# GeoMop/MLMC

Measured on AMD Instinct MI355X. Metric: moment-evals/sec (samples x n_moments), higher is better.
Workload: dtype f64

## Files before the change

### include/mlmc_hip.h

```cpp
#ifndef MLMC_HIP_H
#define MLMC_HIP_H

#include <stdint.h>

#ifdef __cplusplus
extern "C" {
#endif

#define MLMC_ABI_VERSION 8

enum { MLMC_LEGENDRE = 0, MLMC_MONOMIAL = 1, MLMC_FOURIER = 2, MLMC_IDENTITY = 3, MLMC_SPLINE = 4 };
enum {
    MLMC_MODE_MOMENTS = 0,
    MLMC_MODE_COV = 1
};
enum { MLMC_HOST = 0, MLMC_DEVICE = 1 };

typedef struct mlmc_basis mlmc_basis;
typedef struct mlmc_accum mlmc_accum;

typedef struct {
    int32_t kind;
    int32_t size;
    double shift;
    double scale;
    double ref0, ref1;
    int32_t is_log;
    int32_t is_clip;
    int32_t out_size;
    int32_t reserved;
    const double *matrix;
    double x_lo, x_hi;
} mlmc_basis_desc;

int mlmc_init(int device, int flags);
void mlmc_shutdown(void);
int mlmc_set_stream(void *hip_stream);
int mlmc_wait_event(void *hip_event);
int mlmc_synchronize(void);
const char *mlmc_last_error(void);
int mlmc_abi_version(void);
int mlmc_device_info(char *name, int name_len, int *n_cu, int *wave_size, int64_t *hbm_bytes);

int mlmc_basis_create(const mlmc_basis_desc *desc, mlmc_basis **out);
void mlmc_basis_destroy(mlmc_basis *b);
int mlmc_basis_eval(const mlmc_basis *b, const double *x, int64_t n, int32_t size, double *out, int mem_kind);

#define MLMC_MODE_MEAN_ONLY 0x100
int mlmc_accum_create(const mlmc_basis *b, int32_t n_levels, int32_t mode, int32_t n_comp, mlmc_accum **out);
void mlmc_accum_destroy(mlmc_accum *a);
int mlmc_accum_reset(mlmc_accum *a);
int mlmc_accum_push(mlmc_accum *a, int32_t level, const double *fine, const double *coarse, int64_t n, int mem_kind);
int mlmc_accum_finalize(mlmc_accum *a, int64_t *n, int64_t *n_rm, double *s, double *sp, int mem_kind);
int mlmc_accum_estimate(mlmc_accum *a, int32_t n_chunks, const int32_t *levels, const double *const *fine,
                        const double *const *coarse, const int64_t *n_samples, int mem_kind, int64_t *n, int64_t *n_rm,
                        double *s, double *sp);
int mlmc_accum_estimate_packed(mlmc_accum *a, int32_t n_chunks, const int32_t *levels, const double *const *fine,
                               const double *const *coarse, const int64_t *n_samples, int mem_kind, double *packed,
                               int packed_kind);
int mlmc_accum_finalize_packed(mlmc_accum *a, double *packed, int mem_kind);
int mlmc_accum_kernel_time(mlmc_accum *a, double *ms, int64_t *launches, int64_t *alg_bytes);
int mlmc_accum_kernel_flops(mlmc_accum *a, int64_t *mfma_flops);
int mlmc_accum_aux_kernel_time(mlmc_accum *a, double *ms, int64_t *launches, int64_t *alg_bytes);
int mlmc_linearization_table(int32_t kind, int32_t R, int32_t squares, double *out, int64_t out_len);

int mlmc_accum_estimate_multi(int32_t M, const mlmc_basis *const *bases, int32_t K, int32_t n_levels, int32_t n_chunks,
                              const int32_t *levels, const double *const *fine, const double *const *coarse,
                              const int64_t *n_samples, int64_t *n, int64_t *n_rm, double *sums);
int mlmc_accum_estimate_multi_var(int32_t M, const mlmc_basis *const *bases, int32_t K, int32_t n_levels, int32_t n_chunks,
                                  const int32_t *levels, const double *const *fine, const double *const *coarse,
                                  const int64_t *n_samples, int64_t *n, int64_t *n_rm, double *sums, double *sums_sq);

#define MLMC_DIAG_NSTAT 9
int mlmc_level_diagnostics(int32_t M, int32_t n_levels, int32_t n_chunks, const int32_t *levels, const double *const *fine,
                           const double *const *coarse, const int64_t *n_samples, int64_t *n, int64_t *n_rm, double *stats);
int mlmc_diag_merge(const double *a, int64_t na, const double *b, int64_t nb, double *out);

int mlmc_xcov_create(int32_t M, int32_t n_levels, int32_t flags, mlmc_accum **out);
int mlmc_xcov_set_shift(mlmc_accum *a, const double *shift_host);

typedef struct {
    double tol;
    int32_t max_it;
    int32_t n_intervals;
    int32_t gauss_degree;
    int32_t reserved;
    double stab_penalty;
    double penalty_coef;
    int32_t decay_left, decay_right;
} mlmc_maxent_opts;

typedef struct {
    int32_t nit;
    int32_t success;
    double fun;
    double grad_norm;
    double moment0;
    int32_t n_quad;
    int32_t reserved;
} mlmc_maxent_info;

int mlmc_maxent_solve(const mlmc_basis *b, const double *mu, const double *sigma, int32_t R1, double a, double bnd_b,
                      const mlmc_maxent_opts *opts, const double *prev_lambda, int32_t n_prev, double *lambda_io,
                      double *grad_out, double *hess_out, mlmc_maxent_info *info);
int mlmc_density_eval(const mlmc_basis *b, const double *lambda, const double *sigma, int32_t R1, const double *x,
                      int64_t n, double *out, int mem_kind);
int mlmc_density_integrate(const mlmc_basis *b, const double *lambda, const double *sigma, int32_t R1, const double *lo,
                           const double *hi, int64_t n, int32_t degree, double *out);
int mlmc_maxent_solve_batch(int32_t B, const mlmc_basis *const *bases, const int32_t *R1, const double *a, const double *b,
                            const double *mu, const double *sigma, const mlmc_maxent_opts *opts, double *lambda_io,
                            double *grad_out, double *hess_out, mlmc_maxent_info *info);
int mlmc_density_eval_batch(int32_t B, const mlmc_basis *const *bases, const int32_t *R1, const double *lambda, const double *sigma,
                            const double *x, const int64_t *n, double *out);
int mlmc_density_integrate_batch(int32_t B, const mlmc_basis *const *bases, const int32_t *R1, const double *lambda,
                                 const double *sigma, const double *lo, const double *hi, const int64_t *n, int32_t degree,
                                 double *out);
int mlmc_density_cdf_batch(int32_t B, const mlmc_basis *const *bases, const int32_t *R1, const double *lambda, const double *sigma,
                           const double *a, const double *b, int32_t n_intervals, int32_t gauss_degree, const double *x,
                           const int64_t *n, double *out, double *mass_out, int mem_kind);
int mlmc_density_quantiles_batch(int32_t B, const mlmc_basis *const *bases, const int32_t *R1, const double *lambda,
                                 const double *sigma, const double *a, const double *b, int32_t n_intervals, int32_t gauss_degree,
                                 const double *p, const int64_t *n, double *out, double *mass_out, int mem_kind);
int mlmc_density_quantiles_kernel_time(double *ms, int64_t *launches);

int mlmc_percentiles(const double *x, int64_t n, const double *q_percent, int32_t nq, double *out, int64_t *n_valid,
                     int mem_kind);
int mlmc_percentiles_rows(const double *x, int64_t n_rows, int64_t n, int64_t ld, const double *q_percent, int32_t nq,
                          double *out , int64_t *n_valid , int mem_kind);

enum {
    MLMC_X_LOAD = 0,
    MLMC_X_CONST,
    MLMC_X_STORE,
    MLMC_X_SELECT,
    MLMC_X_ADD, MLMC_X_SUB, MLMC_X_MUL, MLMC_X_DIV,
    MLMC_X_MOD,
    MLMC_X_POW, MLMC_X_MAXIMUM, MLMC_X_MINIMUM, MLMC_X_FMAX, MLMC_X_FMIN, MLMC_X_ATAN2, MLMC_X_HYPOT, MLMC_X_FMOD,
    MLMC_X_NEG, MLMC_X_ABS, MLMC_X_SQRT, MLMC_X_SQUARE, MLMC_X_RECIP, MLMC_X_EXP, MLMC_X_EXP2, MLMC_X_EXPM1,
    MLMC_X_LOG, MLMC_X_LOG2, MLMC_X_LOG10, MLMC_X_LOG1P, MLMC_X_SIN, MLMC_X_COS, MLMC_X_TAN, MLMC_X_ASIN, MLMC_X_ACOS,
    MLMC_X_ATAN, MLMC_X_SINH, MLMC_X_COSH, MLMC_X_TANH, MLMC_X_FLOOR, MLMC_X_CEIL, MLMC_X_TRUNC, MLMC_X_RINT,
    MLMC_X_SIGN, MLMC_X_CBRT,
    MLMC_X_LT, MLMC_X_LE, MLMC_X_GT, MLMC_X_GE, MLMC_X_EQ, MLMC_X_NE,
    MLMC_X_AND, MLMC_X_OR, MLMC_X_NOT, MLMC_X_XOR,
    MLMC_X_N_OPS
};
#define MLMC_X_IMM_A 0x4000
#define MLMC_X_IMM_B 0x8000
#define MLMC_X_A_PREV 0x2000
#define MLMC_X_B_PREV 0x1000
#define MLMC_X_NO_WB 0x0800
#define MLMC_X_OP_MASK 0x07ff
typedef struct {
    uint16_t op, dst, a, b;
    double imm;
} mlmc_expr_instr;
#define MLMC_EXPR_MAX_REGS 16
#define MLMC_EXPR_MAX_INSTR 4096
typedef struct mlmc_expr mlmc_expr;
int mlmc_expr_create(const mlmc_expr_instr *prog, int32_t n_instr, int32_t n_regs, int32_t n_in_rows, int32_t n_out_rows,
                     mlmc_expr **out);
void mlmc_expr_destroy(mlmc_expr *e);
int mlmc_expr_eval(mlmc_expr *e, const double *const *rows_in, int32_t has_coarse, int64_t n, int64_t sample_stride,
                   int64_t side_stride, double *fine_out, double *coarse_out, int64_t *n_selected);
int mlmc_expr_state(mlmc_expr *e, int32_t *state, int64_t *compiled_launches);
int mlmc_expr_kernel_time(mlmc_expr *e, double *ms, int64_t *launches, int64_t *alg_bytes);

int mlmc_subsample_gather(const double *fine, const double *coarse, int32_t n_rows, int64_t n, int64_t k, uint64_t seed,
                          double *fine_out, double *coarse_out);

int mlmc_bootstrap_weights(int64_t n, int64_t b0, int64_t nb, const int64_t *sizes, uint64_t seed, uint32_t stream,
                           int32_t *w_out);
typedef struct mlmc_bootstrap mlmc_bootstrap;
int mlmc_bootstrap_create(const mlmc_basis *b, int32_t M, int32_t n_levels, int64_t B, mlmc_bootstrap **out);
void mlmc_bootstrap_destroy(mlmc_bootstrap *bs);
int mlmc_bootstrap_reset(mlmc_bootstrap *bs);
int mlmc_bootstrap_accum(mlmc_bootstrap *bs, int32_t level, const double *fine, const double *coarse, int64_t n,
                         const int64_t *sizes, uint64_t seed, uint32_t stream);
int mlmc_bootstrap_finalize(mlmc_bootstrap *bs, int64_t *n_out, double *s_out, double *sp_out);
int mlmc_bootstrap_kernel_time(mlmc_bootstrap *bs, double *ms_contract, double *ms_rng, int64_t *mfma_flops);

int mlmc_synth_generate(int32_t level_id, int64_t first_sample, int64_t n, double fine_step, double coarse_step,
                        double loc, double scale, int32_t n_rows, const int32_t *rows, double *const *out);
int mlmc_synth_seeds(int32_t level_id, int64_t first_sample, int64_t n, uint32_t *seeds_host);

#ifdef __cplusplus
}
#endif
#endif
```

### mlmc_amd/_lib.py

```python
import ctypes as C
import os
import threading

import numpy as np

_HERE = os.path.dirname(os.path.abspath(__file__))
LIB_PATH = os.environ.get("MLMC_HIP_LIB", os.path.join(_HERE, "libmlmc_hip.so"))

ABI_VERSION = 8
LEGENDRE, MONOMIAL, FOURIER, IDENTITY, SPLINE = 0, 1, 2, 3, 4
MODE_MOMENTS, MODE_COV = 0, 1
MODE_MEAN_ONLY = 0x100
HOST, DEVICE = 0, 1
FLAG_TIMING = 1


class MlmcHipError(RuntimeError):
    pass


class BasisDesc(C.Structure):
    _fields_ = [("kind", C.c_int32), ("size", C.c_int32), ("shift", C.c_double), ("scale", C.c_double),
                ("ref0", C.c_double), ("ref1", C.c_double), ("is_log", C.c_int32), ("is_clip", C.c_int32),
                ("out_size", C.c_int32), ("reserved", C.c_int32), ("matrix", C.POINTER(C.c_double)),
                ("x_lo", C.c_double), ("x_hi", C.c_double)]


class MaxentOpts(C.Structure):
    _fields_ = [("tol", C.c_double), ("max_it", C.c_int32), ("n_intervals", C.c_int32), ("gauss_degree", C.c_int32),
                ("reserved", C.c_int32), ("stab_penalty", C.c_double), ("penalty_coef", C.c_double),
                ("decay_left", C.c_int32), ("decay_right", C.c_int32)]


class MaxentInfo(C.Structure):
    _fields_ = [("nit", C.c_int32), ("success", C.c_int32), ("fun", C.c_double), ("grad_norm", C.c_double),
                ("moment0", C.c_double), ("n_quad", C.c_int32), ("reserved", C.c_int32)]


_dp = C.POINTER(C.c_double)
_ip = C.POINTER(C.c_int64)
_vp = C.c_void_p

SIGNATURES = {
    "mlmc_init": (C.c_int, [C.c_int, C.c_int]),
    "mlmc_shutdown": (None, []),
    "mlmc_set_stream": (C.c_int, [_vp]),
    "mlmc_synchronize": (C.c_int, []),
    "mlmc_wait_event": (C.c_int, [_vp]),
    "mlmc_last_error": (C.c_char_p, []),
    "mlmc_abi_version": (C.c_int, []),
    "mlmc_device_info": (C.c_int, [C.c_char_p, C.c_int, C.POINTER(C.c_int), C.POINTER(C.c_int), _ip]),
    "mlmc_basis_create": (C.c_int, [C.POINTER(BasisDesc), C.POINTER(_vp)]),
    "mlmc_basis_destroy": (None, [_vp]),
    "mlmc_basis_eval": (C.c_int, [_vp, _vp, C.c_int64, C.c_int32, _vp, C.c_int]),
    "mlmc_accum_create": (C.c_int, [_vp, C.c_int32, C.c_int32, C.c_int32, C.POINTER(_vp)]),
    "mlmc_accum_destroy": (None, [_vp]),
    "mlmc_accum_reset": (C.c_int, [_vp]),
    "mlmc_accum_push": (C.c_int, [_vp, C.c_int32, _vp, _vp, C.c_int64, C.c_int]),
    "mlmc_accum_finalize": (C.c_int, [_vp, _vp, _vp, _vp, _vp, C.c_int]),
    "mlmc_accum_finalize_packed": (C.c_int, [_vp, _vp, C.c_int]),
    "mlmc_accum_estimate": (C.c_int, [_vp, C.c_int32, _vp, _vp, _vp, _vp, C.c_int, _vp, _vp, _vp, _vp]),
    "mlmc_accum_estimate_packed": (C.c_int, [_vp, C.c_int32, _vp, _vp, _vp, _vp, C.c_int, _vp, C.c_int]),
    "mlmc_accum_kernel_time": (C.c_int, [_vp, _dp, _ip, _ip]),
    "mlmc_accum_kernel_flops": (C.c_int, [_vp, _ip]),
    "mlmc_accum_aux_kernel_time": (C.c_int, [_vp, _dp, _ip, _ip]),
    "mlmc_linearization_table": (C.c_int, [C.c_int32, C.c_int32, C.c_int32, _vp, C.c_int64]),
    "mlmc_percentiles": (C.c_int, [_vp, C.c_int64, _vp, C.c_int32, _vp, _ip, C.c_int]),
    "mlmc_percentiles_rows": (C.c_int, [_vp, C.c_int64, C.c_int64, C.c_int64, _vp, C.c_int32, _vp, _vp, C.c_int]),
    "mlmc_maxent_solve": (C.c_int, [_vp, _vp, _vp, C.c_int32, C.c_double, C.c_double, C.POINTER(MaxentOpts), _vp,
                                    C.c_int32, _vp, _vp, _vp, C.POINTER(MaxentInfo)]),
    "mlmc_density_eval": (C.c_int, [_vp, _vp, _vp, C.c_int32, _vp, C.c_int64, _vp, C.c_int]),
    "mlmc_density_integrate": (C.c_int, [_vp, _vp, _vp, C.c_int32, _vp, _vp, C.c_int64, C.c_int32, _vp]),
    "mlmc_xcov_create": (C.c_int, [C.c_int32, C.c_int32, C.c_int32, C.POINTER(_vp)]),
    "mlmc_xcov_set_shift": (C.c_int, [_vp, _vp]),
    "mlmc_accum_estimate_multi": (C.c_int, [C.c_int32, _vp, C.c_int32, C.c_int32, C.c_int32, _vp, _vp, _vp, _vp, _vp, _vp,
                                            _vp]),
    "mlmc_accum_estimate_multi_var": (C.c_int, [C.c_int32, _vp, C.c_int32, C.c_int32, C.c_int32, _vp, _vp, _vp, _vp, _vp, _vp,
                                                _vp, _vp]),
    "mlmc_level_diagnostics": (C.c_int, [C.c_int32, C.c_int32, C.c_int32, _vp, _vp, _vp, _vp, _vp, _vp, _vp]),
    "mlmc_diag_merge": (C.c_int, [_vp, C.c_int64, _vp, C.c_int64, _vp]),
    "mlmc_maxent_solve_batch": (C.c_int, [C.c_int32, _vp, _vp, _vp, _vp, _vp, _vp, C.POINTER(MaxentOpts), _vp, _vp, _vp, _vp]),
    "mlmc_density_eval_batch": (C.c_int, [C.c_int32, _vp, _vp, _vp, _vp, _vp, _vp, _vp]),
    "mlmc_density_integrate_batch": (C.c_int, [C.c_int32, _vp, _vp, _vp, _vp, _vp, _vp, _vp, C.c_int32, _vp]),
    "mlmc_density_cdf_batch": (C.c_int, [C.c_int32, _vp, _vp, _vp, _vp, _vp, _vp, C.c_int32, C.c_int32, _vp, _vp, _vp, _vp,
                                         C.c_int]),
    "mlmc_density_quantiles_batch": (C.c_int, [C.c_int32, _vp, _vp, _vp, _vp, _vp, _vp, C.c_int32, C.c_int32, _vp, _vp, _vp, _vp,
                                               C.c_int]),
    "mlmc_density_quantiles_kernel_time": (C.c_int, [_dp, _ip]),
    "mlmc_expr_create": (C.c_int, [_vp, C.c_int32, C.c_int32, C.c_int32, C.c_int32, C.POINTER(_vp)]),
    "mlmc_expr_destroy": (None, [_vp]),
    "mlmc_expr_eval": (C.c_int, [_vp, _vp, C.c_int32, C.c_int64, C.c_int64, C.c_int64, _vp, _vp, _ip]),
    "mlmc_expr_state": (C.c_int, [_vp, C.POINTER(C.c_int32), _ip]),
    "mlmc_expr_kernel_time": (C.c_int, [_vp, _dp, _ip, _ip]),
    "mlmc_synth_generate": (C.c_int, [C.c_int32, C.c_int64, C.c_int64, C.c_double, C.c_double, C.c_double, C.c_double,
                                      C.c_int32, _vp, _vp]),
    "mlmc_synth_seeds": (C.c_int, [C.c_int32, C.c_int64, C.c_int64, _vp]),
    "mlmc_subsample_gather": (C.c_int, [_vp, _vp, C.c_int32, C.c_int64, C.c_int64, C.c_uint64, _vp, _vp]),
    "mlmc_bootstrap_weights": (C.c_int, [C.c_int64, C.c_int64, C.c_int64, _vp, C.c_uint64, C.c_uint32, _vp]),
    "mlmc_bootstrap_create": (C.c_int, [_vp, C.c_int32, C.c_int32, C.c_int64, C.POINTER(_vp)]),
    "mlmc_bootstrap_destroy": (None, [_vp]),
    "mlmc_bootstrap_reset": (C.c_int, [_vp]),
    "mlmc_bootstrap_accum": (C.c_int, [_vp, C.c_int32, _vp, _vp, C.c_int64, _vp, C.c_uint64, C.c_uint32]),
    "mlmc_bootstrap_finalize": (C.c_int, [_vp, _vp, _vp, _vp]),
    "mlmc_bootstrap_kernel_time": (C.c_int, [_vp, _dp, _dp, _ip]),
}

_lock = threading.Lock()
_lib = None
_bound_device = None


def load():
    global _lib
    with _lock:
        if _lib is None:
            if not os.path.exists(LIB_PATH):
                raise MlmcHipError(
                    "libmlmc_hip.so not found at {} -- build it with `python -c 'import __graft_entry__ as g; g.build()'` "
                    "or `make -C mlmc_amd/csrc`; mlmc_amd has no CPU fallback".format(LIB_PATH))
            try:
                import torch
            except ImportError:
                pass
            lib = C.CDLL(LIB_PATH)
            for name, (res, args) in SIGNATURES.items():
                fn = getattr(lib, name)
                fn.restype = res
                fn.argtypes = args
            if lib.mlmc_abi_version() != ABI_VERSION:
                raise MlmcHipError("{} has ABI version {}, this package binds version {}: rebuild it "
                                   "(make -C mlmc_amd/csrc)".format(LIB_PATH, lib.mlmc_abi_version(), ABI_VERSION))
            _lib = lib
    return _lib


def check(rc):
    if rc != 0:
        raise MlmcHipError(load().mlmc_last_error().decode("utf-8", "replace"))


def init(device=None, flags=None):
    global _bound_device
    lib = load()
    if device is None:
        device = _bound_device if _bound_device is not None else int(os.environ.get("LOCAL_RANK", "0"))
    if flags is None:
        flags = FLAG_TIMING if os.environ.get("MLMC_HIP_TIMING") else 0
    check(lib.mlmc_init(int(device), int(flags)))
    _bound_device = int(device)
    return lib


def lib():
    if _bound_device is None:
        return init()
    return _lib


def use_torch_stream():
    import torch
    check(lib().mlmc_set_stream(C.c_void_p(torch.cuda.current_stream().cuda_stream)))


def device_info():
    l = lib()
    name = C.create_string_buffer(256)
    n_cu, wave = C.c_int(), C.c_int()
    hbm = C.c_int64()
    check(l.mlmc_device_info(name, 256, C.byref(n_cu), C.byref(wave), C.byref(hbm)))
    return dict(name=name.value.decode(), n_cu=n_cu.value, wave_size=wave.value, hbm_bytes=hbm.value, device=_bound_device)


def as_f64(a):
    return np.ascontiguousarray(a, dtype=np.float64)


def ptr(a):
    if a is None:
        return None
    if isinstance(a, np.ndarray):
        return a.ctypes.data_as(C.c_void_p)
    if hasattr(a, "data_ptr"):
        return C.c_void_p(a.data_ptr())
    raise TypeError(type(a))


def mem_kind(a):
    if isinstance(a, np.ndarray):
        return HOST
    if hasattr(a, "is_cuda"):
        return DEVICE if a.is_cuda else HOST
    raise TypeError(type(a))
```

### mlmc_amd/csrc/api.hip

```cpp
#include <cmath>
#include <chrono>
#include <cstring>
#include <new>

#include "common.hpp"
#include <algorithm>
#include <map>
#include <tuple>

namespace mlmc {

static thread_local std::string g_err;
void set_error(const std::string &msg) { g_err = msg; }
int fail(const std::string &msg) {
    g_err = msg;
    return 1;
}
Runtime &rt() {
    static Runtime r;
    return r;
}
std::recursive_mutex &api_mutex() {
    static std::recursive_mutex m;
    return m;
// ... 87 lines not shown
    *x_hi = as_double(last);
}

typedef long double ld;
static void legendre_products_ld(int R, std::vector<ld> &out) {
    const int K = 2 * R - 1;
    const size_t RR = (size_t)R * R;
    out.assign((size_t)K * RR, 0.0L);
    for (int i = 0; i < R; ++i)
        for (int j = 0; j < R; ++j) {
            const size_t ij = (size_t)i * R + j;
            const int hi = i > j ? i : j, lo = i > j ? j : i;
            const ld diff = (ld)(hi - lo);
            ld c = (2 * diff + 1) / (2 * (ld)hi + 1);
            for (int t = 1; t <= lo; ++t) {
                const ld tt = (ld)t;
                c = c * ((2 * tt - 1) / tt * (diff + tt) / (2 * (diff + tt) - 1));
            }
            for (int t = 0; t <= lo; ++t) {
                const int k = (hi - lo) + 2 * t;
                out[(size_t)k * RR + ij] = c;
                if (t == lo) break;
                const ld s = (ld)hi + t, kk = (ld)k;
                const ld si = s - hi, sj = s - lo, sk = s - kk;
                ld ratio = ((2 * kk + 5) / (2 * s + 3)) / ((2 * kk + 1) / (2 * s + 1));
                ratio = ratio * ((2 * si + 1) / (si + 1)) * ((2 * sj + 1) / (sj + 1));
                ratio = ratio * (sk / (2 * sk - 1));
                ratio = ratio * ((s + 1) / (2 * s + 1));
                c = c * ratio;
            }
        }
}

bool product_table(int kind, int R, std::vector<double> &out) {
    if (kind != MLMC_LEGENDRE && kind != MLMC_MONOMIAL) return false;
    const int K = 2 * R - 1;
    const size_t RR = (size_t)R * R;
    out.assign((size_t)K * RR, 0.0);
    if (kind == MLMC_MONOMIAL) {
        for (int i = 0; i < R; ++i)
            for (int j = 0; j < R; ++j) out[(size_t)(i + j) * RR + (size_t)i * R + j] = 1.0;
        return true;
    }
    std::vector<ld> c;
    legendre_products_ld(R, c);
    for (size_t q = 0; q < c.size(); ++q) out[q] = (double)c[q];
    return true;
}

static void legendre_square_products_ld(int R, std::vector<ld> &out) {
    const int K = 4 * R - 3;
    const size_t RR = (size_t)R * R;
    out.assign((size_t)K * RR, 0.0L);
    const int Q = 4 * R;
    const ld pi = 3.14159265358979323846264338327950288L;
    std::vector<ld> x(Q), w(Q), P((size_t)K * Q);
    for (int q = 0; q < Q; ++q) {
        ld t = std::cos(pi * ((ld)q + 0.75L) / ((ld)Q + 0.5L)), dp = 1.0L;
        for (int it = 0; it < 100; ++it) {
            ld p0 = 1.0L, p1 = t;
            for (int k = 2; k <= Q; ++k) {
                const ld p2 = ((2 * k - 1) * t * p1 - (k - 1) * p0) / k;
                p0 = p1;
                p1 = p2;
            }
            dp = Q * (t * p1 - p0) / (t * t - 1.0L);
            const ld dt = p1 / dp;
            t -= dt;
            if (std::fabs(dt) < 1e-20L) break;
        }
        {
            ld p0 = 1.0L, p1 = t;
            for (int k = 2; k <= Q; ++k) {
                const ld p2 = ((2 * k - 1) * t * p1 - (k - 1) * p0) / k;
                p0 = p1;
                p1 = p2;
            }
            dp = Q * (t * p1 - p0) / (t * t - 1.0L);
        }
        x[q] = t;
        w[q] = 2.0L / ((1.0L - t * t) * dp * dp);
        ld p0 = 1.0L, p1 = t;
        P[(size_t)0 * Q + q] = 1.0L;
        if (K > 1) P[(size_t)1 * Q + q] = t;
        for (int k = 2; k < K; ++k) {
            const ld p2 = ((2 * k - 1) * t * p1 - (k - 1) * p0) / k;
            p0 = p1;
            p1 = p2;
            P[(size_t)k * Q + q] = p2;
        }
    }
    std::vector<ld> sq(Q);
    for (int i = 0; i < R; ++i)
        for (int j = i; j < R; ++j) {
            for (int q = 0; q < Q; ++q) {
                const ld u = P[(size_t)i * Q + q] * P[(size_t)j * Q + q];
                sq[q] = w[q] * u * u;
            }
            for (int k = 0; k <= 2 * (i + j); k += 2) {
                ld acc = 0.0L;
                const ld *Pk = &P[(size_t)k * Q];
                for (int q = 0; q < Q; ++q) acc += sq[q] * Pk[q];
                const ld c = acc * (2 * k + 1) / 2;
                out[(size_t)k * RR + (size_t)i * R + j] = c;
                out[(size_t)k * RR + (size_t)j * R + i] = c;
            }
        }
    std::vector<ld> t1;
    legendre_products_ld(R, t1);
    for (int j = 0; j < R; ++j)
        for (int k = 0; k < K; ++k) {
            const ld c = k < 2 * R - 1 ? t1[(size_t)k * RR + (size_t)j * R + j] : 0.0L;
            out[(size_t)k * RR + (size_t)j] = c;
            out[(size_t)k * RR + (size_t)j * R] = c;
        }
}

bool square_product_table(int kind, int R, std::vector<double> &out) {
    if (kind != MLMC_LEGENDRE && kind != MLMC_MONOMIAL) return false;
    const int K = 4 * R - 3;
    const size_t RR = (size_t)R * R;
    out.assign((size_t)K * RR, 0.0);
    if (kind == MLMC_MONOMIAL) {
        for (int i = 0; i < R; ++i)
            for (int j = 0; j < R; ++j) out[(size_t)(2 * (i + j)) * RR + (size_t)i * R + j] = 1.0;
        return true;
    }
    std::vector<ld> c;
    legendre_square_products_ld(R, c);
    for (size_t q = 0; q < c.size(); ++q) out[q] = (double)c[q];
    return true;
}

static void chebyshev_compose(const std::vector<ld> &c, int K, int R, std::vector<double> &out) {
    const size_t RR = (size_t)R * R;
    std::vector<ld> g(K), at((size_t)K * K, 0.0L), col(K);
    g[0] = 1.0L;
    for (int j = 1; j < K; ++j) g[j] = g[j - 1] * (ld)(2 * j - 1) / (ld)(2 * j);
    for (int k = 0; k < K; ++k)
        for (int j = 0; j <= k; ++j) at[(size_t)(k - 2 * j < 0 ? 2 * j - k : k - 2 * j) * K + k] += g[j] * g[k - j];
    out.assign((size_t)K * RR, 0.0);
    for (int i = 0; i < R; ++i)
        for (int j = i; j < R; ++j) {
            const size_t ij = (size_t)i * R + j, ji = (size_t)j * R + i;
            for (int k = 0; k < K; ++k) col[k] = c[(size_t)k * RR + ij];
            for (int m = 0; m < K; ++m) {
                ld acc = 0.0L;
                for (int k = m; k < K; k += 2) acc += col[k] * at[(size_t)m * K + k];
                out[(size_t)m * RR + ij] = out[(size_t)m * RR + ji] = (double)acc;
            }
        }
}

bool product_table_chebyshev(int R, std::vector<double> &out) {
    std::vector<ld> c;
    legendre_products_ld(R, c);
    chebyshev_compose(c, 2 * R - 1, R, out);
    return true;
}

bool square_product_table_chebyshev(int R, std::vector<double> &out) {
    std::vector<ld> c;
    legendre_square_products_ld(R, c);
    const int K = 4 * R - 3;
    chebyshev_compose(c, K, R, out);
    std::vector<double> t1;
    product_table_chebyshev(R, t1);
    const size_t RR = (size_t)R * R;
    for (int j = 0; j < R; ++j)
        for (int m = 0; m < K; ++m) {
            const double v = m < 2 * R - 1 ? t1[(size_t)m * RR + (size_t)j * R + j] : 0.0;
            out[(size_t)m * RR + (size_t)j] = v;
            out[(size_t)m * RR + (size_t)j * R] = v;
        }
    return true;
}

static bool linearize_enabled() {
    const char *e = std::getenv("MLMC_HIP_LINEARIZE");
    return !(e && e[0] == '0');
}

static bool linearize_chebyshev_enabled() {
    const char *e = std::getenv("MLMC_HIP_LINEARIZE_CHEB");
    return !(e && e[0] == '0');
}

static int lin_min_size() {
    const char *e = std::getenv("MLMC_HIP_LINEARIZE_MIN");
    return e ? std::atoi(e) : 16;
}

static int need_runtime() {
    if (!rt().ready) return fail("mlmc_init has not been called (no HIP device bound)");
    return 0;
}

}

using namespace mlmc;

extern "C" {

int mlmc_abi_version(void) { return MLMC_ABI_VERSION; }
const char *mlmc_last_error(void) { return g_err.c_str(); }

int mlmc_init(int device, int flags) {
    MLMC_API_GUARD;
    Runtime &r = rt();
    int count = 0;
    hipError_t e = hipGetDeviceCount(&count);
    if (e != hipSuccess || count <= 0) return fail("no HIP device available: libmlmc_hip has no CPU fallback");
    if (device < 0 || device >= count) return fail("mlmc_init: device index out of range");
    if (r.ready && r.device == device) {
        r.flags = flags;
        return 0;
    }
    if (r.ready) return fail("mlmc_init: this process is already bound to another device (one process per GPU)");
    MLMC_HIP_CHECK(hipSetDevice(device));
    MLMC_HIP_CHECK(hipGetDeviceProperties(&r.prop, device));
    if (std::strncmp(r.prop.gcnArchName, "gfx950", 6) != 0)
        return fail(std::string("mlmc_init: kernels are built for gfx950 only, device is ") + r.prop.gcnArchName);
    MLMC_HIP_CHECK(hipStreamCreateWithFlags(&r.stream, hipStreamNonBlocking));
    r.own_stream = true;
    r.device = device;
    r.flags = flags;
    r.n_cu = r.prop.multiProcessorCount;
    r.ready = true;
    return 0;
}

}

namespace mlmc {
hipError_t wait_stream(hipStream_t st) {
    const auto t0 = std::chrono::steady_clock::now();
    for (int spins = 0;; ++spins) {
        const hipError_t e = hipStreamQuery(st);
        if (e != hipErrorNotReady) return e;
        if ((spins & 63) == 63 && std::chrono::steady_clock::now() - t0 > std::chrono::milliseconds(4)) break;
    }
    return hipStreamSynchronize(st);
}
}

extern "C" {

int mlmc_set_stream(void *stream) {
    MLMC_API_GUARD;
    Runtime &r = rt();
    if (!r.ready) return fail("mlmc_init has not been called (no HIP device bound)");
    MLMC_HIP_CHECK(wait_stream(r.stream));
    if (r.own_stream) (void)hipStreamDestroy(r.stream);
    r.stream = (hipStream_t)stream;
    r.own_stream = false;
    return 0;
}

int mlmc_wait_event(void *hip_event) {
    MLMC_API_GUARD;
    Runtime &r = rt();
    if (!r.ready) return fail("mlmc_init has not been called (no HIP device bound)");
    if (!hip_event) return fail("mlmc_wait_event: null event");
    MLMC_HIP_CHECK(hipStreamWaitEvent(r.stream, (hipEvent_t)hip_event, 0));
    return 0;
}

int mlmc_synchronize(void) {
    MLMC_API_GUARD;
    Runtime &r = rt();
    if (!r.ready) return fail("mlmc_init has not been called (no HIP device bound)");
    MLMC_HIP_CHECK(wait_stream(r.stream));
    return 0;
}

void mlmc_shutdown(void) {
    MLMC_API_GUARD;
    Runtime &r = rt();
    if (!r.ready) return;
    (void)wait_stream(r.stream);
    if (r.own_stream) (void)hipStreamDestroy(r.stream);
    r.stream = nullptr;
    r.ready = false;
    r.device = -1;
}

int mlmc_device_info(char *name, int name_len, int *n_cu, int *wave_size, int64_t *hbm_bytes) {
    MLMC_API_GUARD;
    if (need_runtime()) return 1;
    if (name && name_len > 0) {
        std::strncpy(name, rt().prop.name, (size_t)name_len - 1);
        name[name_len - 1] = 0;
    }
    if (n_cu) *n_cu = rt().prop.multiProcessorCount;
    if (wave_size) *wave_size = rt().prop.warpSize;
    if (hbm_bytes) *hbm_bytes = (int64_t)rt().prop.totalGlobalMem;
    return 0;
}

int mlmc_basis_create(const mlmc_basis_desc *d, mlmc_basis **out) {
    MLMC_API_GUARD;
    if (need_runtime()) return 1;
    if (!d || !out) return fail("mlmc_basis_create: null argument");
    if (d->size <= 0) return fail("mlmc_basis_create: size must be > 0");
    if (d->kind < MLMC_LEGENDRE || d->kind > MLMC_SPLINE) return fail("mlmc_basis_create: unknown kind");
    if (d->kind == MLMC_SPLINE && d->size < 4) return fail("mlmc_basis_create: cubic spline moments need size >= 4");
    if (d->kind == MLMC_IDENTITY && d->size != 1) return fail("mlmc_basis_create: IDENTITY has size 1");
    if (d->out_size < 0 || (d->out_size > 0 && !d->matrix)) return fail("mlmc_basis_create: matrix missing");
    if (d->kind == MLMC_LEGENDRE && d->size > 512) return fail("mlmc_basis_create: at most 512 Legendre moments");
    mlmc_basis *b = new (std::nothrow) mlmc_basis();
    if (!b) return fail("out of memory");
    b->p.kind = d->kind;
    b->p.size = d->size;
    b->p.shift = d->shift;
    b->p.scale = d->scale;
    b->p.ref0 = d->ref0;
    b->p.ref1 = d->ref1;
    b->p.is_log = d->is_log;
    b->p.is_clip = d->is_clip;
    b->p.x_lo = d->x_lo;
    b->p.x_hi = d->x_hi;
    if (d->is_log && d->is_clip && d->x_lo == 0.0 && d->x_hi == 0.0) log_keep_interval(b->p, &b->p.x_lo, &b->p.x_hi);
    b->out_size = d->out_size;
    const int R = d->size;
    b->scale_c.assign(R, 1.0);
    if (d->kind == MLMC_LEGENDRE) {
        long double c = 1.0L;
        for (int i = 0; i < R; ++i) {
            if (i >= 1) c = c * (long double)(2 * i - 1) / (long double)(2 * i);
            b->scale_c[i] = (double)c;
        }
    }
    hipError_t e = hipMalloc(&b->d_scale, sizeof(double) * R);
    if (e == hipSuccess) e = hipMemcpy(b->d_scale, b->scale_c.data(), sizeof(double) * R, hipMemcpyHostToDevice);
    if (e == hipSuccess && d->out_size > 0) {
        b->matrix.assign(d->matrix, d->matrix + (size_t)d->out_size * R);
        e = hipMalloc(&b->d_matrix, sizeof(double) * b->matrix.size());
        if (e == hipSuccess)
            e = hipMemcpy(b->d_matrix, b->matrix.data(), sizeof(double) * b->matrix.size(), hipMemcpyHostToDevice);
    }
    if (e != hipSuccess) {
        mlmc_basis_destroy(b);
        return fail(std::string("mlmc_basis_create: ") + hipGetErrorString(e));
    }
    *out = b;
    return 0;
}

void mlmc_basis_destroy(mlmc_basis *b) {
    MLMC_API_GUARD;
    if (!b) return;
    if (b->d_scale) (void)hipFree(b->d_scale);
    if (b->d_matrix) (void)hipFree(b->d_matrix);
    delete b;
}

int mlmc_basis_eval(const mlmc_basis *b, const double *x, int64_t n, int32_t size, double *out, int mem_kind) {
    MLMC_API_GUARD;
    if (need_runtime()) return 1;
    if (!b || (n > 0 && (!x || !out))) return fail("mlmc_basis_eval: null argument");
    const int max_size = b->out_size > 0 ? b->out_size : b->p.size;
    if (size <= 0 || size > max_size) return fail("mlmc_basis_eval: size out of range");
    if (n == 0) return 0;
    hipStream_t st = rt().stream;
    if (mem_kind == MLMC_DEVICE) {
        if (int rc = launch_eval(b, x, n, size, out)) return rc;
        MLMC_HIP_CHECK(wait_stream(st));
        return 0;
    }
    double *d_x = nullptr, *d_o = nullptr;
    hipError_t e0 = hipMalloc(&d_x, sizeof(double) * (size_t)n);
    if (e0 == hipSuccess) e0 = hipMalloc(&d_o, sizeof(double) * (size_t)n * size);
    if (e0 == hipSuccess) e0 = hipMemcpyAsync(d_x, x, sizeof(double) * (size_t)n, hipMemcpyHostToDevice, st);
    int rc = e0 == hipSuccess ? launch_eval(b, d_x, n, size, d_o) : fail(std::string("mlmc_basis_eval: ") + hipGetErrorString(e0));
    if (!rc) {
        hipError_t e = hipMemcpyAsync(out, d_o, sizeof(double) * (size_t)n * size, hipMemcpyDeviceToHost, st);
        if (e == hipSuccess) e = wait_stream(st);
        if (e != hipSuccess) rc = fail(std::string("mlmc_basis_eval copy back: ") + hipGetErrorString(e));
    }
    (void)hipFree(d_x);
    (void)hipFree(d_o);
    return rc;
}

struct LinTables {
    double *d_prod = nullptr, *d_prod2 = nullptr;
};
static int lin_tables(int kind, int R, bool cheb, bool squares, LinTables **out) {
    static std::map<std::tuple<int, int, int>, LinTables> cache;
    LinTables &t = cache[std::make_tuple(cheb ? 1 : 0, kind, R)];
    if (!t.d_prod) {
        std::vector<double> h;
        if (cheb) product_table_chebyshev(R, h);
        else product_table(kind, R, h);
        MLMC_HIP_CHECK(hipMalloc(&t.d_prod, sizeof(double) * h.size()));
        MLMC_HIP_CHECK(hipMemcpy(t.d_prod, h.data(), sizeof(double) * h.size(), hipMemcpyHostToDevice));
    }
    if (squares && !t.d_prod2) {
        std::vector<double> h;
        if (cheb) square_product_table_chebyshev(R, h);
        else square_product_table(kind, R, h);
        MLMC_HIP_CHECK(hipMalloc(&t.d_prod2, sizeof(double) * h.size()));
        MLMC_HIP_CHECK(hipMemcpy(t.d_prod2, h.data(), sizeof(double) * h.size(), hipMemcpyHostToDevice));
    }
    *out = &t;
    return 0;
}

static int inner_basis_create(const mlmc_basis *b, int size, bool cheb, mlmc_basis **out) {
    mlmc_basis_desc d;
    std::memset(&d, 0, sizeof(d));
    d.kind = cheb ? (int)MLMC_MONOMIAL : b->p.kind;
    d.size = size;
    d.shift = b->p.shift; d.scale = b->p.scale; d.ref0 = b->p.ref0; d.ref1 = b->p.ref1;
    d.is_log = b->p.is_log; d.is_clip = b->p.is_clip;
    d.x_lo = b->p.x_lo; d.x_hi = b->p.x_hi;
    if (int rc = mlmc_basis_create(&d, out)) return rc;
    (*out)->p.x_lo = b->p.x_lo;
    (*out)->p.x_hi = b->p.x_hi;
    if (cheb) (*out)->p.kind = KIND_CHEBYSHEV;
    return 0;
}

static int ensure_lin(mlmc_accum *a) {
    if (a->lin) return 0;
    const mlmc_basis *b = a->basis;
    const int K1 = 2 * a->R - 1, K2 = 4 * a->R - 3;
    const bool cheb1 = a->lin_cheb && K1 > 64, cheb2 = a->lin_cheb && K2 > 64;
    LinTables *t1 = nullptr, *t2 = nullptr;
    if (int rc = lin_tables(b->p.kind, a->R, cheb1, false, &t1)) return rc;
    if (a->lin0_eligible)
        if (int rc = lin_tables(b->p.kind, a->R, cheb2, true, &t2)) return rc;
    int rc = inner_basis_create(b, K1, cheb1, &a->lin_basis);
    if (!rc) rc = mlmc_accum_create(a->lin_basis, a->n_levels, MLMC_MODE_MOMENTS | MLMC_MODE_MEAN_ONLY, a->n_comp, &a->lin);
    if (!rc) {
        a->lin->host_outputs = false;
        a->lin_K = K1;
        a->d_lin_prod = t1->d_prod;
    }
    if (!rc && a->lin0_eligible) {
        rc = inner_basis_create(b, K2, cheb2, &a->lin0_basis);
        if (!rc) rc = mlmc_accum_create(a->lin0_basis, a->n_levels, MLMC_MODE_MOMENTS | MLMC_MODE_MEAN_ONLY, a->n_comp, &a->lin0);
        if (!rc) {
            a->lin0->host_outputs = false;
            a->lin0_K = K2;
            a->d_lin0_prod1 = t2->d_prod;
            a->d_lin0_prod = t2->d_prod2;
        }
    }
    if (rc) {
        if (a->lin) mlmc_accum_destroy(a->lin);
        if (a->lin_basis) mlmc_basis_destroy(a->lin_basis);
        if (a->lin0) mlmc_accum_destroy(a->lin0);
        if (a->lin0_basis) mlmc_basis_destroy(a->lin0_basis);
        a->lin = a->lin0 = nullptr;
        a->lin_basis = a->lin0_basis = nullptr;
        a->lin_eligible = a->lin0_eligible = false;
    }
    return rc;
}

int mlmc_accum_create(const mlmc_basis *b, int32_t n_levels, int32_t mode, int32_t n_comp, mlmc_accum **out) {
    MLMC_API_GUARD;
    if (need_runtime()) return 1;
    if (!b || !out) return fail("mlmc_accum_create: null argument");
    if (n_levels <= 0 || n_comp <= 0) return fail("mlmc_accum_create: n_levels and n_comp must be > 0");
    const bool mean_only = (mode & MLMC_MODE_MEAN_ONLY) != 0;
    mode &= ~MLMC_MODE_MEAN_ONLY;
    if (mode != MLMC_MODE_MOMENTS && mode != MLMC_MODE_COV) return fail("mlmc_accum_create: unknown mode");
    mlmc_accum *a = new (std::nothrow) mlmc_accum();
    if (!a) return fail("out of memory");
    a->basis = b;
    a->n_levels = n_levels;
    a->mode = mode;
    const bool spline_band = mode == MLMC_MODE_COV && mean_only && b->out_size == 0 && b->p.kind == MLMC_SPLINE && b->p.size <= SPLINE_BAND_MAX_R;
    a->cov_from_values = mode == MLMC_MODE_COV && (b->out_size > 0 || (b->p.size > 128 && !spline_band));
    a->mean_only = mean_only && ((mode == MLMC_MODE_COV && !a->cov_from_values) || (mode == MLMC_MODE_MOMENTS && b->out_size > 0));
    a->mean_only_plain = mean_only && mode == MLMC_MODE_MOMENTS && b->out_size == 0 &&
                         (b->p.kind == MLMC_LEGENDRE || b->p.kind == MLMC_MONOMIAL || b->p.kind == KIND_CHEBYSHEV) && b->p.size > 64 &&
                         b->p.size <= 256;
    a->n_comp = n_comp;
    a->R = b->p.size;
    a->Rout = b->out_size > 0 ? b->out_size : b->p.size;
    a->RP = (((mode == MLMC_MODE_COV && b->out_size > 0 ? a->Rout : a->R) + 15) / 16) * 16;
    if (mode == MLMC_MODE_MOMENTS) {
        a->K = (int64_t)n_comp * a->Rout;
        a->int_width = 2 * (int64_t)a->R + (b->out_size > 0 ? (int64_t)a->RP * a->RP : 0);
    } else {
        a->K = (int64_t)n_comp * a->Rout * a->Rout;
        a->int_width = 3 * (int64_t)a->RP * a->RP;
    }
    const size_t tot = (size_t)n_levels * n_comp * a->int_width;
    a->state_bytes = sizeof(double) * tot + sizeof(int64_t) * 2 * n_levels;
    a->out_bytes = (sizeof(int64_t) + sizeof(double)) * 2 * n_levels + 2 * sizeof(double) * (size_t)n_levels * a->K;
    if (hipMalloc(&a->d_state, a->state_bytes) != hipSuccess || hipMalloc(&a->d_out, a->out_bytes) != hipSuccess ||
        hipHostMalloc(&a->h_out, a->out_bytes, hipHostMallocDefault) != hipSuccess) {
        mlmc_accum_destroy(a);
        return fail("mlmc_accum_create: device / pinned allocation failed");
    }
    a->d_totals = (double *)a->d_state;
    a->d_counts = (int64_t *)(a->d_totals + tot);
    a->level_flushed.assign(n_levels, 0);
    if (mode == MLMC_MODE_MOMENTS && n_comp == 1 && b->out_size == 0) {
        void *dev_view = nullptr;
        if (hipHostGetDevicePointer(&dev_view, a->h_out, 0) == hipSuccess && dev_view) {
            a->host_outputs = true;
            a->h_out_n = (int64_t *)dev_view;
            a->h_out_s = (double *)(a->h_out_n + 2 * (size_t)n_levels) + 2 * (size_t)n_levels;
            a->h_out_sp = a->h_out_s + (size_t)n_levels * a->K;
        }
    }
    a->d_out_n = (int64_t *)a->d_out;
    a->d_out_nd = (double *)(a->d_out_n + 2 * (size_t)n_levels);
    a->d_out_s = a->d_out_nd + 2 * (size_t)n_levels;
    a->d_out_sp = a->d_out_s + (size_t)n_levels * a->K;
    if (mode == MLMC_MODE_COV && !mean_only && !a->cov_from_values && b->out_size == 0 && b->p.size > lin_min_size() && b->p.size <= 128 &&
        (b->p.kind == MLMC_LEGENDRE || b->p.kind == MLMC_MONOMIAL) && b->p.is_clip &&
        std::fabs(b->p.ref0) <= 1.0 && std::fabs(b->p.ref1) <= 1.0 &&
        linearize_enabled()) {
        a->lin_eligible = true;
        const char *min_n = std::getenv("MLMC_HIP_LINEARIZE_MIN_N");
        a->lin_min_n = min_n ? std::atoll(min_n) : (a->R > 32 ? 100000 : 1500000);
        const char *lin0_env = std::getenv("MLMC_HIP_LINEARIZE_LEVEL0");
        a->lin0_eligible = a->R <= 64 && !(lin0_env && lin0_env[0] == '0');
        a->lin_cheb = b->p.kind == MLMC_LEGENDRE && linearize_chebyshev_enabled() && std::getenv("MLMC_HIP_NO_SPLIT") == nullptr;
    }
    *out = a;
    return mlmc_accum_reset(a);
}

int mlmc_accum_reset(mlmc_accum *a) {
    MLMC_API_GUARD;
    if (need_runtime()) return 1;
    if (!a) return fail("mlmc_accum_reset: null argument");
    hipStream_t st = rt().stream;
    a->pending.clear();
    std::fill(a->level_flushed.begin(), a->level_flushed.end(), 0);
    MLMC_HIP_CHECK(hipMemsetAsync(a->d_state, 0, a->state_bytes, st));
    if (a->xcov) {
        MLMC_HIP_CHECK(hipMemcpyAsync(a->d_shift, a->shift_host.data(), sizeof(double) * a->shift_host.size(), hipMemcpyHostToDevice, st));
        a->xcov_pushes = 0;
    }
    a->lin_used = a->lin0_used = false;
    a->lin_levels.assign(a->n_levels, 0);
    a->lin0_levels.assign(a->n_levels, 0);
    if (a->lin0)
        if (int rc = mlmc_accum_reset(a->lin0)) return rc;
    if (a->lin) return mlmc_accum_reset(a->lin);
    return 0;
}

void mlmc_accum_destroy(mlmc_accum *a) {
    MLMC_API_GUARD;
    if (!a) return;
    if (rt().ready) (void)wait_stream(rt().stream);
    if (a->lin) mlmc_accum_destroy(a->lin);
    if (a->lin_basis) mlmc_basis_destroy(a->lin_basis);
    if (a->lin0) mlmc_accum_destroy(a->lin0);
    if (a->lin0_basis) mlmc_basis_destroy(a->lin0_basis);
    void *ptrs[] = {a->d_state, a->d_partials, a->d_pcounts, a->d_stage_f, a->d_stage_c, a->d_mask, a->d_out, a->d_vals_f, a->d_vals_c, a->d_vals_tmp,
                    a->d_shift};
    for (void *p : ptrs)
        if (p) (void)hipFree(p);
    if (a->h_out) (void)hipHostFree(a->h_out);
    for (hipEvent_t e : a->ev) (void)hipEventDestroy(e);
    delete a;
}

int mlmc_accum_push(mlmc_accum *a, int32_t level, const double *fine, const double *coarse, int64_t n, int mem_kind) {
    MLMC_API_GUARD;
    if (need_runtime()) return 1;
    if (!a) return fail("mlmc_accum_push: null argument");
    if (level < 0 || level >= a->n_levels) return fail("mlmc_accum_push: level out of range");
    if (n < 0) return fail("mlmc_accum_push: negative n");
    if (n == 0) return 0;
    if (!fine) return fail("mlmc_accum_push: fine is NULL");
    if (n > ((int64_t)1 << 40)) return fail("mlmc_accum_push: chunk too large, split it");
    hipStream_t st = rt().stream;
    const size_t bytes = sizeof(double) * (size_t)n * a->n_comp;
    const double *d_f = fine, *d_c = coarse;
    if (mem_kind == MLMC_HOST) {
        if (bytes > a->stage_cap) {
            MLMC_HIP_CHECK(wait_stream(st));
            if (a->d_stage_f) (void)hipFree(a->d_stage_f);
            if (a->d_stage_c) (void)hipFree(a->d_stage_c);
            a->d_stage_f = a->d_stage_c = nullptr;
            a->stage_cap = 0;
            MLMC_HIP_CHECK(hipMalloc(&a->d_stage_f, bytes));
            MLMC_HIP_CHECK(hipMalloc(&a->d_stage_c, bytes));
            a->stage_cap = bytes;
        } else {
            MLMC_HIP_CHECK(wait_stream(st));
        }
        MLMC_HIP_CHECK(hipMemcpyAsync(a->d_stage_f, fine, bytes, hipMemcpyHostToDevice, st));
        d_f = a->d_stage_f;
        if (coarse) {
            MLMC_HIP_CHECK(hipMemcpyAsync(a->d_stage_c, coarse, bytes, hipMemcpyHostToDevice, st));
            d_c = a->d_stage_c;
        }
        MLMC_HIP_CHECK(wait_stream(st));
    } else if (mem_kind != MLMC_DEVICE) {
        return fail("mlmc_accum_push: bad mem_kind");
    }
    if (a->xcov) {
        ++a->xcov_pushes;
        return launch_xcov_push(a, level, d_f, d_c, n);
    }
    const uint8_t *d_mask = nullptr;
    bool count_in_kernel = true;
    if (a->n_comp > 1) {
        if (int rc = ensure((void **)&a->d_mask, &a->mask_cap, (size_t)n)) return rc;
        if (int rc = launch_mask(a, d_f, d_c, n, a->d_mask, a->d_counts + 2 * (int64_t)level)) return rc;
        d_mask = a->d_mask;
        count_in_kernel = false;
    }
    for (int m = 0; m < a->n_comp; ++m) {
        const double *f_m = d_f + (int64_t)m * n;
        const double *c_m = d_c ? d_c + (int64_t)m * n : nullptr;
        const bool count = count_in_kernel && m == 0;
        int rc;
        if (a->mode == MLMC_MODE_MOMENTS) {
            const bool defer = mem_kind == MLMC_DEVICE || a->n_comp > 1;
            rc = launch_moments_accum(a, level, m, f_m, c_m, d_mask, n, count, defer);
            if (!rc && a->basis->out_size > 0 && !a->mean_only) {
                if (a->R <= 128) {
                    rc = launch_cov_accum(a, level, m, f_m, c_m, d_mask, n, false, 1);
                } else {
                    int64_t chunk = 1 << 22;
                    while (chunk > 4096 && chunk * a->R > ((int64_t)1 << 28)) chunk >>= 1;
                    const size_t need = sizeof(double) * (size_t)(n < chunk ? n : chunk) * a->R;
                    if (need > a->vals_cap) {
                        MLMC_HIP_CHECK(wait_stream(st));
                        if (a->d_vals_f) (void)hipFree(a->d_vals_f);
                        if (a->d_vals_c) (void)hipFree(a->d_vals_c);
                        a->d_vals_f = a->d_vals_c = nullptr;
                        a->vals_cap = 0;
                        MLMC_HIP_CHECK(hipMalloc(&a->d_vals_f, need));
                        MLMC_HIP_CHECK(hipMalloc(&a->d_vals_c, need));
                        a->vals_cap = need;
                    }
                    for (int64_t off = 0; off < n && !rc; off += chunk) {
                        const int64_t m_n = (n - off < chunk) ? n - off : chunk;
                        rc = launch_eval_scaled_base(a->basis, f_m + off, m_n, a->d_vals_f);
                        if (!rc && c_m) rc = launch_eval_scaled_base(a->basis, c_m + off, m_n, a->d_vals_c);
                        if (!rc) rc = launch_cov_from_values(a, level, m, a->d_vals_f, c_m ? a->d_vals_c : nullptr,
                                                             d_mask ? d_mask + off : nullptr, m_n, false, 1);
                    }
                }
            }
        } else if (a->cov_from_values) {
            const int R1 = a->Rout;
            int64_t chunk = 1 << 22;
            while (chunk > 4096 && chunk * R1 > ((int64_t)1 << 28)) chunk >>= 1;
            const size_t need = sizeof(double) * (size_t)(n < chunk ? n : chunk) * R1;
            if (need > a->vals_cap) {
                MLMC_HIP_CHECK(wait_stream(st));
                if (a->d_vals_f) (void)hipFree(a->d_vals_f);
                if (a->d_vals_c) (void)hipFree(a->d_vals_c);
                a->d_vals_f = a->d_vals_c = nullptr;
                a->vals_cap = 0;
                MLMC_HIP_CHECK(hipMalloc(&a->d_vals_f, need));
                MLMC_HIP_CHECK(hipMalloc(&a->d_vals_c, need));
                a->vals_cap = need;
            }
            if (a->basis->out_size > 0) {
                const size_t need_tmp = sizeof(double) * (size_t)(n < chunk ? n : chunk) * a->R;
                if (need_tmp > a->vals_tmp_cap) {
                    MLMC_HIP_CHECK(wait_stream(st));
                    if (a->d_vals_tmp) (void)hipFree(a->d_vals_tmp);
                    a->d_vals_tmp = nullptr;
                    a->vals_tmp_cap = 0;
                    MLMC_HIP_CHECK(hipMalloc(&a->d_vals_tmp, need_tmp));
                    a->vals_tmp_cap = need_tmp;
                }
            }
            rc = 0;
            for (int64_t off = 0; off < n && !rc; off += chunk) {
                const int64_t m_n = (n - off < chunk) ? n - off : chunk;
                rc = launch_eval(a->basis, f_m + off, m_n, R1, a->d_vals_f, a->d_vals_tmp);
                if (!rc && c_m) rc = launch_eval(a->basis, c_m + off, m_n, R1, a->d_vals_c, a->d_vals_tmp);
                if (!rc) rc = launch_cov_from_values(a, level, m, a->d_vals_f, c_m ? a->d_vals_c : nullptr,
                                                     d_mask ? d_mask + off : nullptr, m_n, count);
            }
        } else {
            if (a->lin_eligible && !a->lin && n >= a->lin_min_n)
                if (int rcl = ensure_lin(a)) return rcl;
            const bool use_lin0 = a->lin0 && !d_c && n >= a->lin_min_n;
            if (use_lin0) {
                a->lin0_used = true;
                a->lin0_levels[level] = 1;
                rc = launch_moments_accum(a->lin0, level, m, f_m, nullptr, d_mask, n, count_in_kernel && m == 0,
                                          mem_kind == MLMC_DEVICE || a->n_comp > 1);
                if (rc) return rc;
                continue;
            }
            const bool use_lin = a->lin && n >= a->lin_min_n;
            rc = m == 0 ? launch_cov_accum(a, level, 0, d_f, d_c, d_mask, n, count_in_kernel, a->mean_only ? 2 : (use_lin ? 3 : 0), a->n_comp) : 0;
            if (!rc && use_lin) { a->lin_used = true; a->lin_levels[level] = 1; }
            if (!rc && use_lin)
                rc = launch_moments_accum(a->lin, level, m, f_m, c_m, d_mask, n, false, mem_kind == MLMC_DEVICE || a->n_comp > 1);
        }
        if (rc) return rc;
    }
    if (a->mode == MLMC_MODE_MOMENTS && (mem_kind == MLMC_HOST || a->n_comp > 1))
        if (int rc = flush_moments(a)) return rc;
    if (a->lin && (mem_kind == MLMC_HOST || a->n_comp > 1))
        if (int rc = flush_moments(a->lin)) return rc;
    if (a->lin0 && (mem_kind == MLMC_HOST || a->n_comp > 1))
        if (int rc = flush_moments(a->lin0)) return rc;
    return 0;
}

int mlmc_accum_finalize(mlmc_accum *a, int64_t *n, int64_t *n_rm, double *s, double *sp, int mem_kind) {
    MLMC_API_GUARD;
    if (need_runtime()) return 1;
    if (!a || !n || !n_rm || !s || !sp) return fail("mlmc_accum_finalize: null argument");
    hipStream_t st = rt().stream;
    if (a->mode == MLMC_MODE_MOMENTS)
        if (int rcf = flush_moments(a)) return rcf;
    const int L = a->n_levels;
    const size_t nk = (size_t)L * a->K;
    if (a->host_outputs && mem_kind == MLMC_HOST) {
        MLMC_HIP_CHECK(wait_stream(st));
        const int64_t *hn = (const int64_t *)a->h_out;
        const double *hs = (const double *)(hn + 2 * (size_t)L) + 2 * (size_t)L;
        const size_t K = (size_t)a->K;
        for (int l = 0; l < L; ++l) {
            if (a->level_flushed[l]) {
                n[l] = hn[l];
                n_rm[l] = hn[L + l];
                std::memcpy(s + l * K, hs + l * K, sizeof(double) * K);
                std::memcpy(sp + l * K, hs + nk + l * K, sizeof(double) * K);
            } else {
                n[l] = n_rm[l] = 0;
                std::fill(s + l * K, s + (l + 1) * K, 0.0);
                std::fill(sp + l * K, sp + (l + 1) * K, 0.0);
            }
        }
        return 0;
    }
    int rc = a->xcov ? launch_xcov_finalize(a) : (a->mode == MLMC_MODE_MOMENTS) ? launch_moments_finalize(a) : launch_cov_finalize(a);
    if (rc) return rc;
    if (mem_kind == MLMC_DEVICE) {
        MLMC_HIP_CHECK(hipMemcpyAsync(n, a->d_out_n, sizeof(int64_t) * L, hipMemcpyDeviceToDevice, st));
        MLMC_HIP_CHECK(hipMemcpyAsync(n_rm, a->d_out_n + L, sizeof(int64_t) * L, hipMemcpyDeviceToDevice, st));
        MLMC_HIP_CHECK(hipMemcpyAsync(s, a->d_out_s, sizeof(double) * nk, hipMemcpyDeviceToDevice, st));
        MLMC_HIP_CHECK(hipMemcpyAsync(sp, a->d_out_sp, sizeof(double) * nk, hipMemcpyDeviceToDevice, st));
        MLMC_HIP_CHECK(wait_stream(st));
    } else {
        MLMC_HIP_CHECK(hipMemcpyAsync(a->h_out, a->d_out, a->out_bytes, hipMemcpyDeviceToHost, st));
        MLMC_HIP_CHECK(wait_stream(st));
        const int64_t *hn = (const int64_t *)a->h_out;
        const double *hs = (const double *)(hn + 2 * (size_t)L) + 2 * (size_t)L;
        std::memcpy(n, hn, sizeof(int64_t) * L);
        std::memcpy(n_rm, hn + L, sizeof(int64_t) * L);
        std::memcpy(s, hs, sizeof(double) * nk);
        std::memcpy(sp, hs + nk, sizeof(double) * nk);
    }
    return 0;
}

int mlmc_accum_estimate(mlmc_accum *a, int32_t n_chunks, const int32_t *levels, const double *const *fine,
                        const double *const *coarse, const int64_t *n_samples, int mem_kind, int64_t *n, int64_t *n_rm,
                        double *s, double *sp) {
    MLMC_API_GUARD;
    if (!a || n_chunks < 0 || (n_chunks > 0 && (!levels || !fine || !n_samples))) return fail("mlmc_accum_estimate: null argument");
    if (int rc = mlmc_accum_reset(a)) return rc;
    for (int k = 0; k < n_chunks; ++k)
        if (int rc = mlmc_accum_push(a, levels[k], fine[k], coarse ? coarse[k] : nullptr, n_samples[k], mem_kind)) return rc;
    return mlmc_accum_finalize(a, n, n_rm, s, sp, MLMC_HOST);
}

int mlmc_accum_finalize_packed(mlmc_accum *a, double *packed, int mem_kind) {
    MLMC_API_GUARD;
    if (need_runtime()) return 1;
    if (!a || !packed) return fail("mlmc_accum_finalize_packed: null argument");
    hipStream_t st = rt().stream;
    if (a->mode == MLMC_MODE_MOMENTS && a->host_outputs && mem_kind == MLMC_DEVICE && a->R <= MAX_TERMS_PER_PASS &&
        (int)a->pending.size() == a->n_levels &&
        std::none_of(a->level_flushed.begin(), a->level_flushed.end(), [](char f) { return f != 0; })) {
        a->packed_target = packed;
        const int rcf = flush_moments(a);
        a->packed_target = nullptr;
        return rcf;
    }
    if (a->mode == MLMC_MODE_MOMENTS)
        if (int rcf = flush_moments(a)) return rcf;
    int rc = a->xcov ? launch_xcov_finalize(a) : (a->mode == MLMC_MODE_MOMENTS) ? launch_moments_finalize(a) : launch_cov_finalize(a);
    if (rc) return rc;
    const size_t bytes = sizeof(double) * (2 * (size_t)a->n_levels + 2 * (size_t)a->n_levels * a->K);
    MLMC_HIP_CHECK(hipMemcpyAsync(packed, a->d_out_nd, bytes, mem_kind == MLMC_DEVICE ? hipMemcpyDeviceToDevice : hipMemcpyDeviceToHost, st));
    if (mem_kind == MLMC_DEVICE) return 0;
    MLMC_HIP_CHECK(wait_stream(st));
    return 0;
}

int mlmc_accum_estimate_packed(mlmc_accum *a, int32_t n_chunks, const int32_t *levels, const double *const *fine,
                               const double *const *coarse, const int64_t *n_samples, int mem_kind, double *packed,
                               int packed_kind) {
    MLMC_API_GUARD;
    if (!a || n_chunks < 0 || (n_chunks > 0 && (!levels || !fine || !n_samples))) return fail("mlmc_accum_estimate_packed: null argument");
    if (int rc = mlmc_accum_reset(a)) return rc;
    for (int k = 0; k < n_chunks; ++k)
        if (int rc = mlmc_accum_push(a, levels[k], fine[k], coarse ? coarse[k] : nullptr, n_samples[k], mem_kind)) return rc;
    return mlmc_accum_finalize_packed(a, packed, packed_kind);
}

int mlmc_accum_kernel_time(mlmc_accum *a, double *ms, int64_t *launches, int64_t *alg_bytes) {
    MLMC_API_GUARD;
    if (!a) return fail("mlmc_accum_kernel_time: null argument");
    if (a->ev_used) {
        MLMC_HIP_CHECK(hipEventSynchronize(a->ev[a->ev_used - 1]));
        if (int rc = timing_collect(a)) return rc;
    }
    if (ms) *ms = a->ms_total;
    if (launches) *launches = a->launches;
    if (alg_bytes) *alg_bytes = a->alg_bytes;
    a->ms_total = 0;
    a->launches = 0;
    a->alg_bytes = 0;
    return 0;
}

int mlmc_accum_aux_kernel_time(mlmc_accum *a, double *ms, int64_t *launches, int64_t *alg_bytes) {
    MLMC_API_GUARD;
    if (!a) return fail("mlmc_accum_aux_kernel_time: null argument");
    double t = 0.0, t0 = 0.0;
    int64_t l = 0, l0 = 0, b = 0, b0 = 0;
    if (a->lin)
        if (int rc = mlmc_accum_kernel_time(a->lin, &t, &l, &b)) return rc;
    if (a->lin0)
        if (int rc = mlmc_accum_kernel_time(a->lin0, &t0, &l0, &b0)) return rc;
    if (ms) *ms = t + t0;
    if (launches) *launches = l + l0;
    if (alg_bytes) *alg_bytes = b + b0;
    return 0;
}

int mlmc_linearization_table(int32_t kind, int32_t R, int32_t squares, double *out, int64_t out_len) {
    if (!out) return fail("mlmc_linearization_table: null argument");
    if (kind != MLMC_LEGENDRE && kind != MLMC_MONOMIAL) return fail("mlmc_linearization_table: Legendre or monomial moments");
    if (squares < 0 || squares > 3) return fail("mlmc_linearization_table: squares is 0 .. 3");
    const bool cheb = squares >= 2, sq = squares == 1 || squares == 3;
    if (cheb && kind != MLMC_LEGENDRE) return fail("mlmc_linearization_table: the tables for Chebyshev sums belong to Legendre moments");
    if (R < 1 || R > (sq ? 64 : 128)) return fail("mlmc_linearization_table: size out of range");
    const int64_t K = sq ? 4 * (int64_t)R - 3 : 2 * (int64_t)R - 1;
    if (out_len < K * R * R) return fail("mlmc_linearization_table: output too small");
    std::vector<double> t;
    if (cheb) {
        if (sq) square_product_table_chebyshev(R, t);
        else product_table_chebyshev(R, t);
    } else if (sq) {
        square_product_table(kind, R, t);
    } else {
        product_table(kind, R, t);
    }
    std::memcpy(out, t.data(), sizeof(double) * t.size());
    return 0;
}

int mlmc_xcov_create(int32_t M, int32_t n_levels, int32_t flags, mlmc_accum **out) {
    MLMC_API_GUARD;
    if (need_runtime()) return 1;
    if (!out) return fail("mlmc_xcov_create: null argument");
    if (M < 1 || M > XCOV_MAX_M)
        return fail("mlmc_xcov_create: M = " + std::to_string(M) + " components, supported are 1 .. " + std::to_string(XCOV_MAX_M));
    if (n_levels <= 0) return fail("mlmc_xcov_create: n_levels must be > 0");
    if (flags & ~MLMC_MODE_MEAN_ONLY) return fail("mlmc_xcov_create: unknown flags (only MLMC_MODE_MEAN_ONLY)");
    mlmc_accum *a = new (std::nothrow) mlmc_accum();
    if (!a) return fail("out of memory");
    a->xcov = true;
    a->mode = MODE_XCOV;
    a->n_levels = n_levels;
    a->n_comp = M;
    a->mean_only = (flags & MLMC_MODE_MEAN_ONLY) != 0;
    a->K = (int64_t)M * M;
    a->int_width = 2 * a->K;
    const size_t tot = (size_t)n_levels * a->int_width;
    a->state_bytes = sizeof(double) * tot + sizeof(int64_t) * 2 * n_levels;
    a->out_bytes = (sizeof(int64_t) + sizeof(double)) * 2 * n_levels + 2 * sizeof(double) * (size_t)n_levels * a->K;
    a->shift_host.assign(M, 0.0);
    if (hipMalloc(&a->d_state, a->state_bytes) != hipSuccess || hipMalloc(&a->d_out, a->out_bytes) != hipSuccess ||
        hipMalloc(&a->d_shift, sizeof(double) * M) != hipSuccess ||
        hipHostMalloc(&a->h_out, a->out_bytes, hipHostMallocDefault) != hipSuccess) {
        mlmc_accum_destroy(a);
        return fail("mlmc_xcov_create: device / pinned allocation failed");
    }
    a->d_totals = (double *)a->d_state;
    a->d_counts = (int64_t *)(a->d_totals + tot);
    a->level_flushed.assign(n_levels, 0);
    a->d_out_n = (int64_t *)a->d_out;
    a->d_out_nd = (double *)(a->d_out_n + 2 * (size_t)n_levels);
    a->d_out_s = a->d_out_nd + 2 * (size_t)n_levels;
    a->d_out_sp = a->d_out_s + (size_t)n_levels * a->K;
    *out = a;
    return mlmc_accum_reset(a);
}

int mlmc_xcov_set_shift(mlmc_accum *a, const double *shift_host) {
    MLMC_API_GUARD;
    if (need_runtime()) return 1;
    if (!a) return fail("mlmc_xcov_set_shift: null argument");
    if (!a->xcov) return fail("mlmc_xcov_set_shift: not a component-covariance accumulator (mlmc_xcov_create)");
    if (a->xcov_pushes > 0) return fail("mlmc_xcov_set_shift: pushes are pending; reset the accumulator first");
    const int M = a->n_comp;
    if (shift_host)
        for (int m = 0; m < M; ++m)
            if (!std::isfinite(shift_host[m])) return fail("mlmc_xcov_set_shift: shift[" + std::to_string(m) + "] is not finite");
    MLMC_HIP_CHECK(wait_stream(rt().stream));
    if (shift_host) std::memcpy(a->shift_host.data(), shift_host, sizeof(double) * M);
    else std::fill(a->shift_host.begin(), a->shift_host.end(), 0.0);
    return 0;
}

int mlmc_accum_kernel_flops(mlmc_accum *a, int64_t *mfma_flops) {
    MLMC_API_GUARD;
    if (!a) return fail("mlmc_accum_kernel_flops: null argument");
    if (mfma_flops) *mfma_flops = a->mfma_flops;
    a->mfma_flops = 0;
    return 0;
}

}
```

### mlmc_amd/csrc/common.hpp

```cpp
#pragma once
#include <hip/hip_runtime.h>
#include <stdint.h>
#include <mutex>
#include <string>
#include <vector>

#include "../../include/mlmc_hip.h"

namespace mlmc {

constexpr int WAVE = 64;
constexpr int ACC_THREADS = 256;
#ifndef MLMC_TERMS_PER_PASS
#define MLMC_TERMS_PER_PASS 64
#endif
constexpr int MAX_TERMS_PER_PASS = MLMC_TERMS_PER_PASS;
constexpr int KIND_CHEBYSHEV = 16;
static_assert(KIND_CHEBYSHEV > MLMC_SPLINE && KIND_CHEBYSHEV > MLMC_IDENTITY && KIND_CHEBYSHEV > MLMC_FOURIER && KIND_CHEBYSHEV > MLMC_MONOMIAL &&
                  KIND_CHEBYSHEV > MLMC_LEGENDRE && KIND_CHEBYSHEV > 7,
              "KIND_CHEBYSHEV must not collide with a public basis kind of mlmc_hip.h");
constexpr int SPLINE_BAND_MAX_R = 256;

void set_error(const std::string &msg);
int fail(const std::string &msg);
#define MLMC_HIP_CHECK(expr)                                                                   \
    do {                                                                                       \
        hipError_t _e = (expr);                                                                \
        if (_e != hipSuccess)                                                                  \
            return ::mlmc::fail(std::string(#expr) + ": " + hipGetErrorString(_e));            \
    } while (0)

std::recursive_mutex &api_mutex();
void bind_thread_to_device();
struct ApiGuard {
    std::lock_guard<std::recursive_mutex> lock;
    ApiGuard() : lock(api_mutex()) { bind_thread_to_device(); }
};
#define MLMC_API_GUARD ::mlmc::ApiGuard mlmc_api_guard_

struct Runtime {
    bool ready = false;
    int device = -1;
    int flags = 0;
    int n_cu = 0;
    hipStream_t stream = nullptr;
    bool own_stream = false;
    hipDeviceProp_t prop;
};
Runtime &rt();
hipError_t wait_stream(hipStream_t st);

struct MultiWorkspace {
    char *dev = nullptr;
    size_t cap = 0;
    int reserve(size_t bytes) {
        if (bytes <= cap) return 0;
        MLMC_HIP_CHECK(wait_stream(rt().stream));
        if (dev) (void)hipFree(dev);
        dev = nullptr;
        cap = 0;
        MLMC_HIP_CHECK(hipMalloc((void **)&dev, bytes));
        cap = bytes;
        return 0;
    }
};

inline size_t mm_align(size_t bytes) { return (bytes + 255) / 256 * 256; }

__device__ __forceinline__ unsigned long long order_key(double x) {
    unsigned long long u = (unsigned long long)__double_as_longlong(x);
    return (u >> 63) ? ~u : (u | 0x8000000000000000ull);
}

__device__ __forceinline__ void philox_round(uint32_t (&c)[4], uint32_t k0, uint32_t k1) {
    const uint64_t p0 = (uint64_t)0xD2511F53u * c[0], p1 = (uint64_t)0xCD9E8D57u * c[2];
    const uint32_t n0 = (uint32_t)(p1 >> 32) ^ c[1] ^ k0, n1 = (uint32_t)p1;
    const uint32_t n2 = (uint32_t)(p0 >> 32) ^ c[3] ^ k1, n3 = (uint32_t)p0;
    c[0] = n0; c[1] = n1; c[2] = n2; c[3] = n3;
}

struct BasisParams {
    int kind;
    int size;
    double shift, scale, ref0, ref1;
    int is_log, is_clip;
    double x_lo, x_hi;
};

}

struct mlmc_basis {
    mlmc::BasisParams p;
    int out_size = 0;
    std::vector<double> matrix;
    std::vector<double> scale_c;
    double *d_scale = nullptr;
    double *d_matrix = nullptr;
};

struct PendingSeg {
    const double *fine, *coarse;
    const uint8_t *mask;
    int64_t n;
    int level, comp;
    bool count;
};

struct mlmc_accum {
    const mlmc_basis *basis = nullptr;
    int n_levels = 0, mode = 0, n_comp = 1;
    bool mean_only = false;
    bool cov_from_values = false;
    bool mean_only_plain = false;
    int R = 0;
    int Rout = 0;
    int64_t K = 0;
    int64_t int_width = 0;
    void *d_state = nullptr;
    size_t state_bytes = 0;
    double *d_totals = nullptr;
    int64_t *d_counts = nullptr;
    double *d_partials = nullptr; size_t partials_cap = 0;
    int64_t *d_pcounts = nullptr; size_t pcounts_cap = 0;
    double *d_stage_f = nullptr, *d_stage_c = nullptr; size_t stage_cap = 0;
    uint8_t *d_mask = nullptr; size_t mask_cap = 0;
    double *d_vals_f = nullptr, *d_vals_c = nullptr; size_t vals_cap = 0;
    double *d_vals_tmp = nullptr; size_t vals_tmp_cap = 0;
    void *d_out = nullptr;
    size_t out_bytes = 0;
    void *h_out = nullptr;
    bool host_outputs = false;
    double *packed_target = nullptr;
    double *h_out_s = nullptr, *h_out_sp = nullptr; int64_t *h_out_n = nullptr;
    std::vector<char> level_flushed;
    double *d_out_s = nullptr, *d_out_sp = nullptr, *d_out_nd = nullptr; int64_t *d_out_n = nullptr;
    std::vector<hipEvent_t> ev;
    size_t ev_used = 0;
    double ms_total = 0;
    int64_t launches = 0, alg_bytes = 0;
    int64_t mfma_flops = 0;
    int RP = 0;
    bool lin_eligible = false, lin0_eligible = false;
    mlmc_accum *lin = nullptr;
    mlmc_basis *lin_basis = nullptr;
    double *d_lin_prod = nullptr;
    int lin_K = 0;
    mlmc_accum *lin0 = nullptr;
    mlmc_basis *lin0_basis = nullptr;
    double *d_lin0_prod = nullptr;
    double *d_lin0_prod1 = nullptr;
    bool lin_cheb = false;
    std::vector<char> lin_levels, lin0_levels;
    int lin0_K = 0;
    bool lin0_used = false;
    int64_t lin_min_n = 0;
    bool lin_used = false;
    std::vector<PendingSeg> pending;
    bool xcov = false;
    double *d_shift = nullptr;
    std::vector<double> shift_host;
    int64_t xcov_pushes = 0;
};

namespace mlmc {
int launch_eval(const mlmc_basis *b, const double *d_x, int64_t n, int size, double *d_out, double *scratch = nullptr);
int launch_eval_scaled_base(const mlmc_basis *b, const double *d_x, int64_t n, double *d_out);
int launch_mask(const mlmc_accum *a, const double *d_f, const double *d_c, int64_t n, uint8_t *d_mask, int64_t *d_counts_level);
int launch_moments_accum(mlmc_accum *a, int level, int comp, const double *d_f, const double *d_c, const uint8_t *d_mask,
                         int64_t n, bool count, bool defer);
int flush_moments(mlmc_accum *a);
int launch_moments_finalize(mlmc_accum *a);
int launch_cov_accum(mlmc_accum *a, int level, int comp, const double *d_f, const double *d_c, const uint8_t *d_mask,
                     int64_t n, bool count, int gram_mode, int ncomp = 1);
int launch_cov_finalize(mlmc_accum *a);
constexpr int XCOV_MAX_M = 1024;
constexpr int MODE_XCOV = 2;
int launch_xcov_push(mlmc_accum *a, int level, const double *d_f, const double *d_c, int64_t n);
int launch_xcov_finalize(mlmc_accum *a);
bool product_table(int kind, int R, std::vector<double> &out);
bool square_product_table(int kind, int R, std::vector<double> &out);
bool product_table_chebyshev(int R, std::vector<double> &out);
bool square_product_table_chebyshev(int R, std::vector<double> &out);
int launch_cov_from_values(mlmc_accum *a, int level, int comp, const double *d_vf, const double *d_vc, const uint8_t *d_mask,
                           int64_t n, bool count, int gram_mode = 0);
int ensure(void **p, size_t *cap, size_t bytes);
void gauss_legendre(int n, std::vector<double> &x, std::vector<double> &w);
std::vector<double> effective_coeffs(const mlmc_basis *b, const double *lambda, const double *sigma, int R1);
int timing_begin(mlmc_accum *a);
int timing_end(mlmc_accum *a);
}
```

### mlmc_amd/csrc/cov.hip

```cpp
#include <cstring>

#include "device_basis.hpp"

namespace mlmc {

typedef double v4f64 __attribute__((ext_vector_type(4)));
#ifdef MLMC_PROF_COV
__device__ unsigned long long *g_prof_cov;
#define MLMC_COV_STAMP(slot)                                      \
    {                                                             \
        const unsigned long long now_ = __builtin_amdgcn_s_memtime(); \
        prof_acc[slot] += now_ - prof_t;                          \
        prof_t = now_;                                            \
    }
#else
#define MLMC_COV_STAMP(slot)
#endif
#ifndef MLMC_COV_PRIO_MFMA
#define MLMC_COV_PRIO_MFMA 0
#define MLMC_COV_PRIO_EVAL 2
#endif
#ifndef MLMC_COV_SLICE_BITS
#define MLMC_COV_SLICE_BITS 17
#endif
// ... 212 lines not shown
            const int rowl = lane & 15;
#pragma unroll
            for (int kk = 0; kk < BATCH / 16; ++kk) {
                const int col = 4 * (wave + 4 * kk) + (lane >> 4);
                double d[T], sv[T], dd[T], ss[T], ds[T];
#pragma unroll
                for (int i = 0; i < T; ++i) {
                    const double f = lds_f[(16 * i + rowl) * STRIDE + col];
                    d[i] = sv[i] = f;
                    if (PAIR) {
                        const double c = lds_c[(16 * i + rowl) * STRIDE + col];
                        d[i] = f - c;
                        sv[i] = f + c;
                    }
                    if (M0) {
                        dd[i] = d[i] * d[i];
                        ss[i] = sv[i] * sv[i];
                        ds[i] = d[i] * sv[i];
                    }
                }
#pragma unroll
                for (int i = 0; i < T; ++i)
#pragma unroll
                    for (int j = 0; j < T; ++j) {
                        const bool upper = j >= i;
                        if (M0) {
                            if (DO_G0 && (PAIR || upper)) acc[0][i][j] = __builtin_amdgcn_mfma_f64_16x16x4f64(d[i], sv[j], acc[0][i][j], 0, 0, 0);
                            if (PAIR || upper) acc[1][i][j] = __builtin_amdgcn_mfma_f64_16x16x4f64(dd[i], ss[j], acc[1][i][j], 0, 0, 0);
                            if (PAIR && upper) acc[NG - 1][i][j] = __builtin_amdgcn_mfma_f64_16x16x4f64(ds[i], ds[j], acc[NG - 1][i][j], 0, 0, 0);
                        } else if (MODE == 1 || !PAIR) {
                            if (upper) acc[0][i][j] = __builtin_amdgcn_mfma_f64_16x16x4f64(d[i], d[j], acc[0][i][j], 0, 0, 0);
                        } else {
                            acc[0][i][j] = __builtin_amdgcn_mfma_f64_16x16x4f64(d[i], sv[j], acc[0][i][j], 0, 0, 0);
                        }
                    }
            }
            __builtin_amdgcn_s_setprio(MLMC_COV_PRIO_EVAL);
            MLMC_COV_STAMP(2)
            __syncthreads();
            MLMC_COV_STAMP(3)
            continue;
        }
        const int arow = 16 * I + (lane & 15);
#pragma unroll
        for (int kk = 0; kk < BATCH / 4 / NSL; ++kk) {
            const int ks = kslice + kk * NSL;
            const int col = 4 * ks + (lane >> 4);
            double fa = lds_f[arow * STRIDE + col];
            double da = fa, sa = fa;
            if (PAIR) {
                double ca = lds_c[arow * STRIDE + col];
                da = fa - ca;
                sa = fa + ca;
            }
            const double a1 = da * da, a2 = da * sa;
#pragma unroll
            for (int J = 0; J < T; ++J) {
                const int brow = 16 * J + (lane & 15);
                double fb = (WIDE ? lds_fb : lds_f)[brow * STRIDE + col];
                double db = fb, sb = fb;
                if (PAIR) {
                    double cb = (WIDE ? lds_cb : lds_c)[brow * STRIDE + col];
                    db = fb - cb;
                    sb = fb + cb;
                }
                if (M0) {
                    if (DO_G0) acc[0][0][J] = __builtin_amdgcn_mfma_f64_16x16x4f64(da, sb, acc[0][0][J], 0, 0, 0);
                    if (PAIR) {
                        acc[1][0][J] = __builtin_amdgcn_mfma_f64_16x16x4f64(a1, sb * sb, acc[1][0][J], 0, 0, 0);
                        acc[2][0][J] = __builtin_amdgcn_mfma_f64_16x16x4f64(a2, db * sb, acc[2][0][J], 0, 0, 0);
                    } else {
                        acc[1][0][J] = __builtin_amdgcn_mfma_f64_16x16x4f64(a1, fb * fb, acc[1][0][J], 0, 0, 0);
                    }
                } else {
                    acc[0][0][J] = __builtin_amdgcn_mfma_f64_16x16x4f64(da, MODE == 2 ? sb : db, acc[0][0][J], 0, 0, 0);
                }
            }
        }
        __builtin_amdgcn_s_setprio(MLMC_COV_PRIO_EVAL);
        __syncthreads();
    }

#ifdef MLMC_PROF_COV
    if (lane == 0 && blockIdx.y == 0) {
        unsigned long long *q = g_prof_cov + ((size_t)blockIdx.x * 4 + wave) * 6;
        q[0] = prof_acc[0]; q[1] = prof_acc[1]; q[2] = prof_acc[2]; q[3] = prof_acc[3];
        q[4] = __builtin_amdgcn_s_memtime() - prof_t0;
        q[5] = ((unsigned long long)__builtin_amdgcn_s_getreg((4 << 0) | (0 << 6) | (31 << 11)) & 0xffffu) |
               ((unsigned long long)__builtin_amdgcn_s_getreg((20 << 0) | (0 << 6) | (3 << 11)) << 16) |
               ((__builtin_amdgcn_s_memrealtime() - prof_r0) << 24);
    }
#endif
    constexpr int NGOUT = M0 ? 3 : 1;
    double *__restrict__ prow = partials + (SLICED ? ((int64_t)blockIdx.x * 4 + wave) : ((int64_t)blockIdx.x * NSL + kslice)) * (NGOUT * NT * NT);
#pragma unroll
    for (int Iw = 0; Iw < TI; ++Iw) {
        const int It = SLICED ? Iw : I;
#pragma unroll
        for (int J = 0; J < T; ++J) {
#pragma unroll
            for (int r = 0; r < 4; ++r) {
                const int row = 16 * It + (lane >> 4) + 4 * r;
                const int col = 16 * J + (lane & 15);
                const bool low = SLICED && J < It;
                const int mirror = (16 * It + (lane & 15)) * NT + (16 * J + (lane >> 4) + 4 * r);
                if (M0) {
                    if (PAIR) {
                        prow[0 * NT * NT + row * NT + col] = acc[0][Iw][J][r];
                        prow[1 * NT * NT + row * NT + col] = acc[1][Iw][J][r];
                        if (!low) prow[2 * NT * NT + row * NT + col] = acc[NG - 1][Iw][J][r];
                        else prow[2 * NT * NT + mirror] = acc[NG - 1][SLICED ? J : 0][It][r];
                    } else if (!low) {
                        prow[0 * NT * NT + row * NT + col] = acc[0][Iw][J][r];
                        prow[1 * NT * NT + row * NT + col] = acc[1][Iw][J][r];
                        prow[2 * NT * NT + row * NT + col] = acc[1][Iw][J][r];
                    } else {
                        prow[0 * NT * NT + mirror] = acc[0][SLICED ? J : 0][It][r];
                        prow[1 * NT * NT + mirror] = acc[1][SLICED ? J : 0][It][r];
                        prow[2 * NT * NT + mirror] = acc[1][SLICED ? J : 0][It][r];
                    }
                } else if (low && (MODE == 1 || !PAIR)) {
                    prow[mirror] = acc[0][SLICED ? J : 0][It][r];
                } else {
                    prow[row * NT + col] = acc[0][Iw][J][r];
                }
            }
        }
    }
    if (pcounts) {
        n_keep = wave_sum_i(n_keep);
        n_rm = wave_sum_i(n_rm);
        if (lane == 0) { ldc[wave][0] = n_keep; ldc[wave][1] = n_rm; }
        __syncthreads();
        if (threadIdx.x < 2) {
            const int v = ldc[0][threadIdx.x] + ldc[1][threadIdx.x] + ldc[2][threadIdx.x] + ldc[3][threadIdx.x];
            pcounts[(int64_t)blockIdx.x * 2 + threadIdx.x] = v;
        }
    }
}

__host__ __device__ constexpr int sym_n(int w) { return w < 2 ? 2 : 3; }
__host__ __device__ constexpr int sym_i(int w, int t) { return t == 0 ? w : (w < 2 ? w : (w == 2 ? (t == 1 ? 2 : 0) : (t == 1 ? 0 : 1))); }
__host__ __device__ constexpr int sym_j(int w, int t) { return t == 0 ? w : (w < 2 ? w + 1 : (w == 2 ? (t == 1 ? 3 : 2) : 3)); }
__host__ __device__ constexpr int psym_n(int w) { return w == 0 ? 1 : 3; }
__host__ __device__ constexpr int psym_i(int w, int t) { return t == 0 ? w : (w == 1 ? (t == 1 ? 1 : 0) : (w == 2 ? (t == 1 ? 2 : 0) : (t == 1 ? 0 : 1))); }
__host__ __device__ constexpr int psym_j(int w, int t) { return t == 0 ? w : (w == 1 ? (t == 1 ? 2 : 1) : (w == 2 ? (t == 1 ? 3 : 2) : 3)); }
__host__ __device__ constexpr int bsym_n(int w) { return (w == 0 || w == 3) ? 3 : 2; }
__host__ __device__ constexpr int bsym_i(int w, int t) { return w == 0 ? (t == 2 ? 1 : 0) : (w == 1 ? 0 : (w == 2 ? 1 : (t == 2 ? 3 : 2))); }
__host__ __device__ constexpr int bsym_j(int w, int t) { return w == 0 ? (t == 0 ? 0 : 1) : (w == 1 ? 2 + t : (w == 2 ? 2 + t : (t == 0 ? 2 : 3))); }
__host__ __device__ constexpr int xsym_n(int kind, int w) { return kind == 2 ? bsym_n(w) : (kind == 1 ? psym_n(w) : sym_n(w)); }
__host__ __device__ constexpr int xsym_i(int kind, int w, int t) { return kind == 2 ? bsym_i(w, t) : (kind == 1 ? psym_i(w, t) : sym_i(w, t)); }
__host__ __device__ constexpr int xsym_j(int kind, int w, int t) { return kind == 2 ? bsym_j(w, t) : (kind == 1 ? psym_j(w, t) : sym_j(w, t)); }

template <int KIND, bool PAIR, int MODE, int BD, int W>
__device__ __forceinline__ void cov_t4_body(const BasisParams &bp, 
                                            const double *__restrict__ fine, const double *__restrict__ coarse,
                                            const uint8_t *__restrict__ mask, int64_t n, double *__restrict__ partials,
                                            int64_t *__restrict__ pcounts, double *__restrict__ lds_f,
                                            double *__restrict__ lds_c, int (*ldc)[2]) {
    constexpr int NT = 64;
    constexpr int TA = 64 * BD;
    constexpr int N_EVAL = TA + NT;
    constexpr bool BLK = PAIR && (MODE == 0 || MODE == 3) && MLMC_COV_BLK22 && COV_T4_BATCH == 32;
    constexpr bool BLK2 = PAIR && MODE == 2 && MLMC_COV_BLK22 && COV_T4_BATCH == 32;
    constexpr int ONE = BLK ? 2 : ((PAIR && MLMC_COV_T4_ONE_LIST && COV_T4_BATCH == 32) ? 1 : 0);
    constexpr int NS = xsym_n(ONE, W);
    constexpr int W1 = (MODE == 0 && !PAIR) ? (W + 2) % 4 : W;
    constexpr int NS1 = sym_n(W1);
    constexpr int NFULL = (MODE == 0 && PAIR) ? 2 : (((MODE == 2 || MODE == 3) && PAIR) ? 1 : 0);
    constexpr int GV = MODE == 3 ? 0 : 1;
    constexpr int NSYMM = (MODE == 0 && !PAIR) ? 2 : 1;
    const int lane = threadIdx.x & 63;

    v4f64 accf[NFULL > 0 ? NFULL : 1][4];
    v4f64 accs[NSYMM][3];
#pragma unroll
    for (int g = 0; g < (NFULL > 0 ? NFULL : 1); ++g)
#pragma unroll
        for (int j = 0; j < 4; ++j) accf[g][j] = (v4f64){0.0, 0.0, 0.0, 0.0};
#pragma unroll
    for (int g = 0; g < NSYMM; ++g)
#pragma unroll
        for (int t = 0; t < 3; ++t) accs[g][t] = (v4f64){0.0, 0.0, 0.0, 0.0};

    constexpr int BATCH = PAIR ? COV_T4_BATCH : 2 * COV_T4_BATCH;
    constexpr int STRIDE = BATCH + MLMC_COV_B128_PAD;
    constexpr bool evaluator = BLK ? (W == 1) : (W < COV_T4_BATCH / 32);
    constexpr int EW = BLK ? 0 : W;
    const int samp = PAIR ? (EW * 32 + (lane & 31)) : (EW * 64 + lane);
    const int psamp = cov_t4_pos(samp);
    const bool is_coarse = PAIR && (lane >> 5);
    const double *__restrict__ src = is_coarse ? coarse : fine;
    double *__restrict__ dst = is_coarse ? lds_c : lds_f;
    int n_keep = 0, n_rm = 0;

    const int64_t n_batches = (n + BATCH - 1) / BATCH;
    int64_t batch = blockIdx.x;
    double xv = 0.0;
    uint8_t mv = 1;
    if (evaluator && batch < n_batches) {
        int64_t idx = batch * BATCH + samp;
        if (idx < n) { xv = src[idx]; if (mask) mv = mask[idx]; }
    }
#ifdef MLMC_PROF_COV
    unsigned long long prof_acc[4] = {0, 0, 0, 0}, prof_t = __builtin_amdgcn_s_memtime();
    const unsigned long long prof_t0 = prof_t, prof_r0 = __builtin_amdgcn_s_memrealtime();
#endif
    constexpr bool RANKS = (MODE == 0 || (MODE == 3 && MLMC_COV_VAR_RANKS)) && PAIR;
    const unsigned per_round = gridDim.x >= (unsigned)COV_T4_WGS ? gridDim.x / (unsigned)COV_T4_WGS : 1u;
    const unsigned prio_slot = (blockIdx.x / per_round) % (unsigned)COV_T4_WGS;
    MLMC_COV_EVAL_PRIO(RANKS);
    for (; batch < n_batches; batch += gridDim.x) {
        if (evaluator) {
            const int64_t idx = batch * BATCH + samp;
            const bool valid = idx < n;
            bool keep;
            double t = transform_value(bp, xv, keep);
            keep = keep && valid && (mv != 0);
            if (PAIR) {
                const int other = __shfl_xor((int)keep, 32, 64);
                keep = keep && (other != 0);
            }
            if (!is_coarse) { n_keep += (int)keep; n_rm += (int)(valid && !keep); }
            const int64_t nidx = (batch + gridDim.x) * BATCH + samp;
            if (nidx < n) { xv = src[nidx]; if (mask) mv = mask[nidx]; }
            TermGen<KIND> g;
            g.init(keep ? t : 0.0, keep ? 1.0 : 0.0, bp);
            if constexpr (KIND == MLMC_SPLINE) {
                cov_spline_store<NT, STRIDE, TA>(g, dst, psamp);
            } else {
#pragma unroll
                for (int i = 0; i < N_EVAL; ++i) {
                    const double q = g.next(i);
                    if (i >= TA) dst[(i - TA) * STRIDE + psamp] = q;
                }
            }
        }
        MLMC_COV_STAMP(0)
        const unsigned long long prio_clock = __builtin_amdgcn_s_memtime();
        __syncthreads();
        MLMC_COV_STAMP(1)
        MLMC_COV_MFMA_PRIO(RANKS, prio_slot, (unsigned)COV_T4_WGS, prio_clock);
        typedef double v2f64 __attribute__((ext_vector_type(2)));
        v2f64 f2[4], c2[4];
#pragma unroll
        for (int ks = 0; ks < BATCH / 4; ++ks) {
            const int col = 4 * ks + (lane >> 4);
            double d[4], sm[4];
#pragma unroll
            for (int J = 0; J < 4; ++J) {
                const int row = 16 * J + (lane & 15);
                double f, c = 0.0;
                if (MLMC_COV_B128) {
                    if ((ks & 1) == 0) {
                        const int base = row * STRIDE + 8 * (ks >> 1) + 2 * (lane >> 4);
                        f2[J] = *reinterpret_cast<const v2f64 *>(lds_f + base);
                        if (PAIR) c2[J] = *reinterpret_cast<const v2f64 *>(lds_c + base);
                    }
                    f = (ks & 1) ? f2[J].y : f2[J].x;
                    if (PAIR) c = (ks & 1) ? c2[J].y : c2[J].x;
                } else {
                    f = lds_f[row * STRIDE + col];
                    if (PAIR) c = lds_c[row * STRIDE + col];
                }
                d[J] = f;
                sm[J] = f;
                if (PAIR) {
                    d[J] = f - c;
                    sm[J] = f + c;
                }
            }
            if (BLK) {
                constexpr int RA = 2 * (W >> 1), CA = 2 * (W & 1);
                double ds[4];
#pragma unroll
                for (int J = 0; J < 4; ++J) ds[J] = d[J] * sm[J];
#pragma unroll
                for (int r = 0; r < 2; ++r) {
                    const double dr2 = d[RA + r] * d[RA + r];
#pragma unroll
                    for (int c = 0; c < 2; ++c) {
                        if (MODE == 0)
                            accf[0][2 * r + c] = __builtin_amdgcn_mfma_f64_16x16x4f64(d[RA + r], sm[CA + c], accf[0][2 * r + c], 0, 0, 0);
                        accf[GV][2 * r + c] = __builtin_amdgcn_mfma_f64_16x16x4f64(dr2, sm[CA + c] * sm[CA + c], accf[GV][2 * r + c], 0, 0, 0);
                    }
                }
#pragma unroll
                for (int t = 0; t < NS; ++t)
                    accs[0][t] = __builtin_amdgcn_mfma_f64_16x16x4f64(ds[xsym_i(ONE, W, t)], ds[xsym_j(ONE, W, t)], accs[0][t], 0, 0, 0);
            } else if ((MODE == 0 || MODE == 3) && PAIR) {
                const double dw2 = d[W] * d[W];
                double ds[4];
#pragma unroll
                for (int J = 0; J < 4; ++J) {
                    if (MODE == 0) accf[0][J] = __builtin_amdgcn_mfma_f64_16x16x4f64(d[W], sm[J], accf[0][J], 0, 0, 0);
                    accf[GV][J] = __builtin_amdgcn_mfma_f64_16x16x4f64(dw2, sm[J] * sm[J], accf[GV][J], 0, 0, 0);
                    ds[J] = d[J] * sm[J];
                }
#pragma unroll
                for (int t = 0; t < NS; ++t)
                    accs[0][t] = __builtin_amdgcn_mfma_f64_16x16x4f64(ds[xsym_i(ONE, W, t)], ds[xsym_j(ONE, W, t)], accs[0][t], 0, 0, 0);
            } else if (MODE == 0) {
                double f2[4];
#pragma unroll
                for (int J = 0; J < 4; ++J) f2[J] = d[J] * d[J];
#pragma unroll
                for (int t = 0; t < NS; ++t)
                    accs[0][t] = __builtin_amdgcn_mfma_f64_16x16x4f64(d[xsym_i(ONE, W, t)], d[xsym_j(ONE, W, t)], accs[0][t], 0, 0, 0);
#pragma unroll
                for (int t = 0; t < NS1; ++t)
                    accs[1][t] = __builtin_amdgcn_mfma_f64_16x16x4f64(f2[sym_i(W1, t)], f2[sym_j(W1, t)], accs[1][t], 0, 0, 0);
            } else if (MODE == 3) {
                double f2[4];
#pragma unroll
                for (int J = 0; J < 4; ++J) f2[J] = d[J] * d[J];
#pragma unroll
                for (int t = 0; t < NS; ++t)
                    accs[0][t] = __builtin_amdgcn_mfma_f64_16x16x4f64(f2[xsym_i(ONE, W, t)], f2[xsym_j(ONE, W, t)], accs[0][t], 0, 0, 0);
            } else if (MODE == 2 && PAIR && BLK2) {
                constexpr int RA = 2 * (W >> 1), CA = 2 * (W & 1);
#pragma unroll
                for (int r = 0; r < 2; ++r)
#pragma unroll
                    for (int c = 0; c < 2; ++c)
                        accf[0][2 * r + c] = __builtin_amdgcn_mfma_f64_16x16x4f64(d[RA + r], sm[CA + c], accf[0][2 * r + c], 0, 0, 0);
            } else if (MODE == 2 && PAIR) {
#pragma unroll
                for (int J = 0; J < 4; ++J)
                    accf[0][J] = __builtin_amdgcn_mfma_f64_16x16x4f64(d[W], sm[J], accf[0][J], 0, 0, 0);
            } else {
#pragma unroll
                for (int t = 0; t < NS; ++t)
                    accs[0][t] = __builtin_amdgcn_mfma_f64_16x16x4f64(d[xsym_i(ONE, W, t)], d[xsym_j(ONE, W, t)], accs[0][t], 0, 0, 0);
            }
        }
        MLMC_COV_EVAL_PRIO(RANKS);
        MLMC_COV_STAMP(2)
        __syncthreads();
        MLMC_COV_STAMP(3)
    }
#ifdef MLMC_PROF_COV
    if (lane == 0 && blockIdx.y == 0) {
        unsigned long long *q = g_prof_cov + ((size_t)blockIdx.x * 4 + W) * 6;
        q[0] = prof_acc[0]; q[1] = prof_acc[1]; q[2] = prof_acc[2]; q[3] = prof_acc[3];
        q[4] = __builtin_amdgcn_s_memtime() - prof_t0;
        q[5] = ((unsigned long long)__builtin_amdgcn_s_getreg((4 << 0) | (0 << 6) | (31 << 11)) & 0xffffu) |
               ((unsigned long long)__builtin_amdgcn_s_getreg((20 << 0) | (0 << 6) | (3 << 11)) << 16) |
               ((__builtin_amdgcn_s_memrealtime() - prof_r0) << 24);
    }
#endif

    constexpr int NGOUT = cov_ng(MODE);
    double *__restrict__ prow = partials + (int64_t)blockIdx.x * (NGOUT * NT * NT);
    const int r0 = lane >> 4, c0 = lane & 15;
    if (MODE == 3 && PAIR) {
#pragma unroll
        for (int J = 0; J < 4; ++J)
#pragma unroll
            for (int r = 0; r < 4; ++r) {
                const int tr = BLK ? 2 * (W >> 1) + (J >> 1) : W, tc = BLK ? 2 * (W & 1) + (J & 1) : J;
                prow[(16 * tr + r0 + 4 * r) * NT + 16 * tc + c0] = accf[0][J][r];
            }
    }
    if (MODE == 0 && PAIR) {
#pragma unroll
        for (int J = 0; J < 4; ++J)
#pragma unroll
            for (int r = 0; r < 4; ++r) {
                const int tr = BLK ? 2 * (W >> 1) + (J >> 1) : W, tc = BLK ? 2 * (W & 1) + (J & 1) : J;
                const int row = 16 * tr + r0 + 4 * r, col = 16 * tc + c0;
                prow[0 * NT * NT + row * NT + col] = accf[0][J][r];
                prow[1 * NT * NT + row * NT + col] = accf[1][J][r];
            }
    }
    if (MODE == 2 && PAIR) {
#pragma unroll
        for (int J = 0; J < 4; ++J)
#pragma unroll
            for (int r = 0; r < 4; ++r) {
                const int tr = BLK2 ? 2 * (W >> 1) + (J >> 1) : W, tc = BLK2 ? 2 * (W & 1) + (J & 1) : J;
                prow[(16 * tr + r0 + 4 * r) * NT + 16 * tc + c0] = accf[0][J][r];
            }
    }
#pragma unroll
    for (int t = 0; t < ((MODE == 2 && PAIR) ? 0 : NS); ++t)
#pragma unroll
        for (int r = 0; r < 4; ++r) {
            const int row = 16 * xsym_i(ONE, W, t) + r0 + 4 * r, col = 16 * xsym_j(ONE, W, t) + c0;
            if (MODE == 0 && PAIR) {
                prow[2 * NT * NT + row * NT + col] = accs[0][t][r];
                if (xsym_i(ONE, W, t) != xsym_j(ONE, W, t)) prow[2 * NT * NT + col * NT + row] = accs[0][t][r];
            } else if (MODE == 3) {
                const bool off = xsym_i(ONE, W, t) != xsym_j(ONE, W, t);
                prow[NT * NT + row * NT + col] = accs[0][t][r];
                if (off) prow[NT * NT + col * NT + row] = accs[0][t][r];
                if (!PAIR) {
                    prow[row * NT + col] = accs[0][t][r];
                    if (off) prow[col * NT + row] = accs[0][t][r];
                }
            } else if (MODE == 0) {
                prow[0 * NT * NT + row * NT + col] = accs[0][t][r];
                if (xsym_i(ONE, W, t) != xsym_j(ONE, W, t)) prow[0 * NT * NT + col * NT + row] = accs[0][t][r];
            } else {
                prow[row * NT + col] = accs[0][t][r];
                if (xsym_i(ONE, W, t) != xsym_j(ONE, W, t)) prow[col * NT + row] = accs[0][t][r];
            }
        }
    if (MODE == 0 && !PAIR) {
#pragma unroll
        for (int t = 0; t < NS1; ++t)
#pragma unroll
            for (int r = 0; r < 4; ++r) {
                const int row = 16 * sym_i(W1, t) + r0 + 4 * r, col = 16 * sym_j(W1, t) + c0;
                prow[1 * NT * NT + row * NT + col] = accs[1][t][r];
                prow[2 * NT * NT + row * NT + col] = accs[1][t][r];
                if (sym_i(W1, t) != sym_j(W1, t)) {
                    prow[1 * NT * NT + col * NT + row] = accs[1][t][r];
                    prow[2 * NT * NT + col * NT + row] = accs[1][t][r];
                }
            }
    }
    if (pcounts) {
        n_keep = wave_sum_i(n_keep);
        n_rm = wave_sum_i(n_rm);
        if (lane == 0 && W < 2) { ldc[W][0] = n_keep; ldc[W][1] = n_rm; }
        __syncthreads();
        if (threadIdx.x < 2) pcounts[(int64_t)blockIdx.x * 2 + threadIdx.x] = ldc[0][threadIdx.x] + ldc[1][threadIdx.x];
    }
}

template <int KIND, bool PAIR, int MODE, int BD>
__global__ __launch_bounds__(256, COV_T4_WGS) void k_cov_accum_t4(BasisParams bp, 
                                                         const double *__restrict__ fine, const double *__restrict__ coarse,
                                                         const uint8_t *__restrict__ mask, int64_t n, int R,
                                                         double *__restrict__ partials, int64_t *__restrict__ pcounts) {
    __shared__ __attribute__((aligned(16))) double lds_f[64 * ((PAIR ? COV_T4_BATCH : 2 * COV_T4_BATCH) + MLMC_COV_B128_PAD)];
    __shared__ __attribute__((aligned(16))) double lds_c[PAIR ? 64 * (COV_T4_BATCH + MLMC_COV_B128_PAD) : 1];
    __shared__ int ldc[2][2];
    (void)R;
    fine += (int64_t)blockIdx.y * n;
    if (PAIR) coarse += (int64_t)blockIdx.y * n;
    partials += (int64_t)blockIdx.y * gridDim.x * (cov_ng(MODE) * 64 * 64);
    if (blockIdx.y) pcounts = nullptr;
    switch (__builtin_amdgcn_readfirstlane((int)(threadIdx.x >> 6))) {
        case 0: cov_t4_body<KIND, PAIR, MODE, BD, 0>(bp, fine, coarse, mask, n, partials, pcounts, lds_f, lds_c, ldc); break;
        case 1: cov_t4_body<KIND, PAIR, MODE, BD, 1>(bp, fine, coarse, mask, n, partials, pcounts, lds_f, lds_c, ldc); break;
        case 2: cov_t4_body<KIND, PAIR, MODE, BD, 2>(bp, fine, coarse, mask, n, partials, pcounts, lds_f, lds_c, ldc); break;
        default: cov_t4_body<KIND, PAIR, MODE, BD, 3>(bp, fine, coarse, mask, n, partials, pcounts, lds_f, lds_c, ldc); break;
    }
}

__global__ __launch_bounds__(1024) void k_reduce_cov(const double *__restrict__ partials, int nrows, int NT, int NG, int RP,
                                                    int roff, int coff, double *__restrict__ totals, int64_t comp_stride,
                                                    int mirror, const int64_t *__restrict__ pcounts, int nblocks,
                                                    int64_t *__restrict__ counts) {
    __shared__ double lds[64][17];
    const int c = threadIdx.x & 15, g = threadIdx.x >> 4;
    const int width = NG * NT * NT;
    if (pcounts && blockIdx.x == gridDim.x - 1) {
        if (blockIdx.y == 0 && threadIdx.x < 64) {
            int64_t a = 0, b = 0;
            for (int i = threadIdx.x; i < nblocks; i += 64) { a += pcounts[2 * i]; b += pcounts[2 * i + 1]; }
            for (int off = 32; off >= 1; off >>= 1) { a += __shfl_xor(a, off, 64); b += __shfl_xor(b, off, 64); }
            if (threadIdx.x == 0) { counts[0] += a; counts[1] += b; }
        }
        return;
    }
    partials += (int64_t)blockIdx.y * nrows * width;
    totals += (int64_t)blockIdx.y * comp_stride;
    const int col = blockIdx.x * 16 + c;
    double acc = 0.0;
    if (col < width)
        for (int b = g; b < nrows; b += 64) acc += partials[(int64_t)b * width + col];
    lds[g][c] = acc;
    __syncthreads();
    if (g == 0 && col < width) {
        double v = 0.0;
#pragma unroll
        for (int k = 0; k < 64; ++k) v += lds[k][c];
        const int gi = col / (NT * NT), rem = col % (NT * NT);
        const int row = roff + rem / NT, cc = coff + rem % NT;
        if (row < RP && cc < RP) {
            totals[(int64_t)gi * RP * RP + (int64_t)row * RP + cc] += v;
            if (mirror) totals[(int64_t)gi * RP * RP + (int64_t)cc * RP + row] += v;
        }
    }
}

template <int KIND, int T, int MODE, int BI, int BJ>
static int launch_cov_t(const BasisParams &bp, bool pair, int blocks, int ncomp, const double *d_f, const double *d_c,
                        const uint8_t *d_mask, int64_t n, int R, double *partials, int64_t *pcounts) {
    hipStream_t st = rt().stream;
    if constexpr (T == 4 && BI == BJ) {
        if (pair)
            hipLaunchKernelGGL((k_cov_accum_t4<KIND, true, MODE, BI>), dim3(blocks, ncomp), dim3(256), 0, st, bp, d_f, d_c, d_mask, n, R, partials, pcounts);
        else
            hipLaunchKernelGGL((k_cov_accum_t4<KIND, false, MODE, BI>), dim3(blocks, ncomp), dim3(256), 0, st, bp, d_f, d_c, d_mask, n, R, partials, pcounts);
    } else {
        if (pair)
            hipLaunchKernelGGL((k_cov_accum<KIND, T, true, MODE, BI, BJ>), dim3(blocks, ncomp), dim3(256), 0, st, bp, d_f, d_c, d_mask, n, R, partials, pcounts, 0, 0);
        else
            hipLaunchKernelGGL((k_cov_accum<KIND, T, false, MODE, BI, BJ>), dim3(blocks, ncomp), dim3(256), 0, st, bp, d_f, d_c, d_mask, n, R, partials, pcounts, 0, 0);
    }
    MLMC_HIP_CHECK(hipGetLastError());
    return 0;
}

template <int KIND, int MODE>
static int launch_cov_kind(const BasisParams &bp, int T, int bi, int bj, bool pair, int blocks, int ncomp, const double *d_f,
                           const double *d_c, const uint8_t *d_mask, int64_t n, int R, double *partials, int64_t *pcounts) {
#define MLMC_COV_ARGS bp, pair, blocks, ncomp, d_f, d_c, d_mask, n, R, partials, pcounts
    if (T == 1) return launch_cov_t<KIND, 1, MODE, 0, 0>(MLMC_COV_ARGS);
    if (T == 2) return launch_cov_t<KIND, 2, MODE, 0, 0>(MLMC_COV_ARGS);
    if (bi == 0 && bj == 0) return launch_cov_t<KIND, 4, MODE, 0, 0>(MLMC_COV_ARGS);
    if (bi == 0 && bj == 1) return launch_cov_t<KIND, 4, MODE, 0, 1>(MLMC_COV_ARGS);
    if (bi == 1 && bj == 0) return launch_cov_t<KIND, 4, MODE, 1, 0>(MLMC_COV_ARGS);
    if (bi == 1 && bj == 1) return launch_cov_t<KIND, 4, MODE, 1, 1>(MLMC_COV_ARGS);
#undef MLMC_COV_ARGS
    return fail("covariance: at most 128 moments");
}

int launch_cov_from_values(mlmc_accum *a, int level, int comp, const double *d_vf, const double *d_vc, const uint8_t *d_mask,
                           int64_t n, bool count, int gram_mode) {
    if (n == 0) return 0;
    const bool diff_gram = gram_mode == 1;
    const int R = diff_gram ? a->R : a->Rout;
    hipStream_t st = rt().stream;
    const int T = (R <= 16) ? 1 : (R <= 32 ? 2 : 4);
    const int NT = 16 * T, NSL = 4 / T;
    const bool pair = d_vc != nullptr;
    const int NB = (R + 63) / 64;
    const int64_t n_batches = (n + COV_BATCH - 1) / COV_BATCH;
    const int NG = diff_gram ? 1 : 3;
    const size_t width = (size_t)NG * NT * NT;
    const BasisParams &bp = a->basis->p;
    double *totals = a->d_totals + ((int64_t)level * a->n_comp + comp) * a->int_width + (diff_gram ? 2 * (int64_t)R : 0);
    const bool symmetric = !pair || diff_gram;
    for (int bi = 0; bi < NB; ++bi)
        for (int bj = 0; bj < NB; ++bj) {
            if (symmetric && bj < bi) continue;
            const bool wide = bi != bj;
            int blocks = rt().n_cu * (wide ? 1 : 2);
            if (n_batches < blocks) blocks = (int)n_batches;
            const int n_slices = T <= 2 ? 4 : NSL;
            if (int rc = ensure((void **)&a->d_partials, &a->partials_cap, sizeof(double) * (size_t)blocks * n_slices * width)) return rc;
            if (int rc = ensure((void **)&a->d_pcounts, &a->pcounts_cap, sizeof(int64_t) * (size_t)blocks * 2)) return rc;
            const bool do_count = count && bi == 0 && bj == 0 && !diff_gram;
            int64_t *pc = do_count ? a->d_pcounts : nullptr;
            if (int rc = timing_begin(a)) return rc;
#define MLMC_COV_VALS1(TT, BJJ, MODE)                                                                                           \
    do {                                                                                                                        \
        if (pair)                                                                                                               \
            hipLaunchKernelGGL((k_cov_accum<MLMC_IDENTITY, TT, true, MODE, 0, BJJ, true>), dim3(blocks), dim3(256), 0, st, bp,      \
                               d_vf, d_vc, d_mask, n, R, a->d_partials, pc, 64 * bi, 64 * bj);                                  \
        else                                                                                                                    \
            hipLaunchKernelGGL((k_cov_accum<MLMC_IDENTITY, TT, false, MODE, 0, BJJ, true>), dim3(blocks), dim3(256), 0, st, bp,     \
                               d_vf, d_vc, d_mask, n, R, a->d_partials, pc, 64 * bi, 64 * bj);                                  \
    } while (0)
#define MLMC_COV_VALS(TT, BJJ)                                                                                                  \
    do {                                                                                                                        \
        if (diff_gram) MLMC_COV_VALS1(TT, BJJ, 1); else MLMC_COV_VALS1(TT, BJJ, 0);                                             \
    } while (0)
            if (T == 1) MLMC_COV_VALS(1, 0);
            else if (T == 2) MLMC_COV_VALS(2, 0);
            else if (!wide) MLMC_COV_VALS(4, 0);
            else MLMC_COV_VALS(4, 1);
#undef MLMC_COV_VALS
#undef MLMC_COV_VALS1
            MLMC_HIP_CHECK(hipGetLastError());
            if (int rc = timing_end(a)) return rc;
            if (!diff_gram) {
                a->launches += 1;
                a->alg_bytes += (int64_t)n * (pair ? 16 : 8);
                a->mfma_flops += (int64_t)512 * n * (T <= 2 ? (pair ? 2 * T * T + T * (T + 1) / 2 : T * (T + 1)) : (pair ? 3 : 2) * 16);
            }
            hipLaunchKernelGGL(k_reduce_cov, dim3((unsigned)((width + 15) / 16) + (do_count ? 1u : 0u)), dim3(1024), 0, st, a->d_partials,
                               blocks * n_slices, NT, NG, a->RP, 64 * bi, 64 * bj, totals, (int64_t)0, (symmetric && wide) ? 1 : 0,
                               do_count ? a->d_pcounts : (const int64_t *)nullptr, blocks, a->d_counts + 2 * (int64_t)level);
            MLMC_HIP_CHECK(hipGetLastError());
        }
    return 0;
}

constexpr int BAND_W = 5;
template <bool PAIR>
__global__ __launch_bounds__(256) void k_spline_band_accum(BasisParams bp, const double *__restrict__ fine,
                                                          const double *__restrict__ coarse, const uint8_t *__restrict__ mask,
                                                          int64_t n, int R, double *__restrict__ partials,
                                                          int64_t *__restrict__ pcounts) {
    extern __shared__ double band_tab[];
    __shared__ int ldc[4][2];
    const int RP8 = R + 8;
    fine += (int64_t)blockIdx.y * n;
    if (PAIR) coarse += (int64_t)blockIdx.y * n;
    partials += (int64_t)blockIdx.y * gridDim.x * (BAND_W * R);
    if (blockIdx.y) pcounts = nullptr;
    const int lane = threadIdx.x & 63, wave = threadIdx.x >> 6;
    for (int i = threadIdx.x; i < 4 * RP8 * BAND_W; i += 256) band_tab[i] = 0.0;
    __syncthreads();
    double *__restrict__ tab = band_tab + (size_t)wave * RP8 * BAND_W;
    int n_keep = 0, n_rm = 0;
    const int64_t T = (int64_t)gridDim.x * 256;
    for (int64_t i = (int64_t)blockIdx.x * 256 + threadIdx.x; i < n; i += T) {
        bool kf, kc = true;
        const double tf = transform_value(bp, fine[i], kf);
        double tc = 0.0;
        if (PAIR) tc = transform_value(bp, coarse[i], kc);
        const bool keep = kf && kc && (!mask || mask[i] != 0);
        n_keep += (int)keep;
        n_rm += (int)!keep;
        if (!keep) continue;
        TermGen<MLMC_SPLINE> gf, gc;
        gf.init(tf, 1.0, bp);
        const double nf[4] = {gf.n0, gf.n1, gf.n2, gf.n3};
        double nc[4] = {0.0, 0.0, 0.0, 0.0};
        bool same = false;
        if (PAIR) {
            gc.init(tc, 1.0, bp);
            nc[0] = gc.n0; nc[1] = gc.n1; nc[2] = gc.n2; nc[3] = gc.n3;
            same = gc.k == gf.k;
        }
#pragma unroll
        for (int j = 0; j < 4; ++j) {
            const int r = gf.k + j;
            if (r < 1) continue;
            double *__restrict__ row = tab + (size_t)r * BAND_W;
            atomicAdd(&row[4], same ? nf[j] - nc[j] : nf[j]);
#pragma unroll
            for (int j2 = j; j2 < 4; ++j2)
                atomicAdd(&row[j2 - j], same ? __builtin_fma(nf[j], nf[j2], -(nc[j] * nc[j2])) : nf[j] * nf[j2]);
        }
        if (PAIR && !same) {
#pragma unroll
            for (int j = 0; j < 4; ++j) {
                const int r = gc.k + j;
                if (r < 1) continue;
                double *__restrict__ row = tab + (size_t)r * BAND_W;
                atomicAdd(&row[4], -nc[j]);
#pragma unroll
                for (int j2 = j; j2 < 4; ++j2) atomicAdd(&row[j2 - j], -(nc[j] * nc[j2]));
            }
        }
    }
    n_keep = wave_sum_i(n_keep);
    n_rm = wave_sum_i(n_rm);
    if (lane == 0) { ldc[wave][0] = n_keep; ldc[wave][1] = n_rm; }
    __syncthreads();
    for (int j = threadIdx.x; j < BAND_W * R; j += 256) {
        const int o = j;
        partials[(int64_t)blockIdx.x * (BAND_W * R) + j] =
            ((band_tab[o] + band_tab[(size_t)RP8 * BAND_W + o]) + band_tab[(size_t)2 * RP8 * BAND_W + o]) + band_tab[(size_t)3 * RP8 * BAND_W + o];
    }
    if (pcounts && threadIdx.x < 2)
        pcounts[(int64_t)blockIdx.x * 2 + threadIdx.x] = ldc[0][threadIdx.x] + ldc[1][threadIdx.x] + ldc[2][threadIdx.x] + ldc[3][threadIdx.x];
}

__global__ __launch_bounds__(1024) void k_reduce_band(const double *__restrict__ partials, const int64_t *__restrict__ pcounts, int nblocks,
                                                     int R, int RP, double *__restrict__ totals, int64_t comp_stride,
                                                     int64_t *__restrict__ counts, int corner) {
    __shared__ double lds[64][17];
    __shared__ long long lc[16][2];
    const int width = BAND_W * R;
    const int n_col_groups = (width + 15) / 16;
    totals += (int64_t)blockIdx.y * comp_stride;
    if ((int)blockIdx.x == n_col_groups) {
        long long a = 0, b = 0;
        for (int i = threadIdx.x; i < nblocks; i += 1024) { a += pcounts[2 * i]; b += pcounts[2 * i + 1]; }
        for (int off = 32; off >= 1; off >>= 1) { a += __shfl_xor(a, off, 64); b += __shfl_xor(b, off, 64); }
        if ((threadIdx.x & 63) == 0) { lc[threadIdx.x >> 6][0] = a; lc[threadIdx.x >> 6][1] = b; }
        __syncthreads();
        if (threadIdx.x == 0) {
            a = 0; b = 0;
            for (int w = 0; w < 16; ++w) { a += lc[w][0]; b += lc[w][1]; }
            if (counts && blockIdx.y == 0) { counts[0] += a; counts[1] += b; }
            if (corner) totals[0] += (double)a;
        }
        return;
    }
    partials += (int64_t)blockIdx.y * nblocks * width;
    const int c = threadIdx.x & 15, g = threadIdx.x >> 4;
    const int col = blockIdx.x * 16 + c;
    double acc = 0.0;
    if (col < width)
        for (int b = g; b < nblocks; b += 64) acc += partials[(int64_t)b * width + col];
    lds[g][c] = acc;
    __syncthreads();
    if (g == 0 && col < width) {
        double v = 0.0;
#pragma unroll
        for (int k = 0; k < 64; ++k) v += lds[k][c];
        const int r = col / BAND_W, w = col % BAND_W;
        if (r >= 1) {
            if (w == 4) {
                totals[r] += v;
                totals[(int64_t)r * RP] += v;
            } else if (r + w < R) {
                totals[(int64_t)r * RP + r + w] += v;
                if (w) totals[(int64_t)(r + w) * RP + r] += v;
            }
        }
    }
}

static int launch_spline_band(mlmc_accum *a, int level, int comp, const double *d_f, const double *d_c, const uint8_t *d_mask, int64_t n,
                              bool count, int ncomp) {
    hipStream_t st = rt().stream;
    const int R = a->R;
    const bool pair = d_c != nullptr;
    int blocks = rt().n_cu * 4;
    const int64_t want = (n + 255) / 256;
    if (want < blocks) blocks = (int)want;
    if (int rc = ensure((void **)&a->d_partials, &a->partials_cap, sizeof(double) * (size_t)blocks * BAND_W * R * ncomp)) return rc;
    if (int rc = ensure((void **)&a->d_pcounts, &a->pcounts_cap, sizeof(int64_t) * (size_t)blocks * 2)) return rc;
    const size_t lds = sizeof(double) * 4 * (size_t)(R + 8) * BAND_W;
    const BasisParams &bp = a->basis->p;
    double *totals = a->d_totals + ((int64_t)level * a->n_comp + comp) * a->int_width;
    if (int rc = timing_begin(a)) return rc;
    if (pair)
        hipLaunchKernelGGL(k_spline_band_accum<true>, dim3(blocks, ncomp), dim3(256), lds, st, bp, d_f, d_c, d_mask, n, R, a->d_partials, a->d_pcounts);
    else
        hipLaunchKernelGGL(k_spline_band_accum<false>, dim3(blocks, ncomp), dim3(256), lds, st, bp, d_f, d_c, d_mask, n, R, a->d_partials, a->d_pcounts);
    MLMC_HIP_CHECK(hipGetLastError());
    if (int rc = timing_end(a)) return rc;
    a->launches += 1;
    a->alg_bytes += (int64_t)n * (pair ? 16 : 8) * ncomp;
    hipLaunchKernelGGL(k_reduce_band, dim3((BAND_W * R + 15) / 16 + 1, ncomp), dim3(1024), 0, st, a->d_partials, a->d_pcounts, blocks, R, a->RP,
                       totals, a->int_width, count ? a->d_counts + 2 * (int64_t)level : (int64_t *)nullptr, pair ? 0 : 1);
    MLMC_HIP_CHECK(hipGetLastError());
    return 0;
}

static int cov_tiles_per_sample(int T, bool diagonal, bool pair, int gram_mode) {
    const int full = T * T, upper = T * (T + 1) / 2;
    if (!diagonal) return (gram_mode == 0 ? (pair ? 3 : 2) : (gram_mode == 3 ? (pair ? 2 : 1) : 1)) * full;
    if (gram_mode == 0) return pair ? 2 * full + upper : 2 * upper;
    if (gram_mode == 3) return pair ? full + upper : upper;
    if (gram_mode == 1 || !pair) return upper;
    return full;
}

int launch_cov_accum(mlmc_accum *a, int level, int comp, const double *d_f, const double *d_c, const uint8_t *d_mask,
                     int64_t n, bool count, int gram_mode, int ncomp) {
    const bool diff_gram_only = gram_mode == 1;
    if (n == 0) return 0;
    const int R = a->R;
    if (a->basis->p.kind == MLMC_SPLINE && gram_mode == 2 && R <= SPLINE_BAND_MAX_R)
        return launch_spline_band(a, level, comp, d_f, d_c, d_mask, n, count, ncomp);
    if (R > 128) return fail("covariance accumulation in registers covers 128 moments; larger bases go through launch_cov_from_values");
    hipStream_t st = rt().stream;
    const int T = (R <= 16) ? 1 : (R <= 32 ? 2 : 4);
    const int NT = 16 * T, NSL = 4 / T;
    const int NB = (R + 63) / 64;
    const bool pair = d_c != nullptr;
    const int64_t bsz = T == 4 ? (pair ? COV_T4_BATCH : 2 * COV_T4_BATCH) : cov_batch(T, false, false, pair);
    const int64_t n_batches = (n + bsz - 1) / bsz;
    const BasisParams &bp = a->basis->p;
    double *totals0 = a->d_totals + ((int64_t)level * a->n_comp + comp) * a->int_width + (diff_gram_only ? 2 * (int64_t)R : 0);
    for (int bi = 0; bi < NB; ++bi)
        for (int bj = 0; bj < NB; ++bj) {
            if (!pair && bj < bi) continue;
            const bool two_slots = gram_mode == 3 && T == 4 && bi == bj;
            const int NG = gram_mode == 3 ? (two_slots ? 2 : 3) : cov_ng(gram_mode);
            const size_t width = (size_t)NG * NT * NT;
            double *totals = totals0 + (two_slots ? (int64_t)a->RP * a->RP : 0);
            int blocks = rt().n_cu * ((bi != bj) ? ((pair && MLMC_COV_WIDE_BATCH < 64) ? 2 : 1) : (T == 1 ? 4 : (T == 4 ? COV_T4_WGS : 2)));
            if ((n_batches + 3) / 4 < blocks) blocks = (int)((n_batches + 3) / 4);
            const int n_slices = T <= 2 ? 4 : NSL;
            if (int rc = ensure((void **)&a->d_partials, &a->partials_cap, sizeof(double) * (size_t)blocks * n_slices * width * ncomp)) return rc;
            if (int rc = ensure((void **)&a->d_pcounts, &a->pcounts_cap, sizeof(int64_t) * (size_t)blocks * 2)) return rc;
            const bool do_count = count && bi == 0 && bj == 0;
            int64_t *pc = do_count ? a->d_pcounts : nullptr;
            const bool timed = !diff_gram_only;
            if (timed) if (int rc = timing_begin(a)) return rc;
            int rc;
#define MLMC_COV_DISPATCH(KIND)                                                                                               \
    rc = gram_mode == 3 ? launch_cov_kind<KIND, 3>(bp, T, bi, bj, pair, blocks, ncomp, d_f, d_c, d_mask, n, R, a->d_partials, pc) \
       : gram_mode == 2 ? launch_cov_kind<KIND, 2>(bp, T, bi, bj, pair, blocks, ncomp, d_f, d_c, d_mask, n, R, a->d_partials, pc) \
       : diff_gram_only ? launch_cov_kind<KIND, 1>(bp, T, bi, bj, pair, blocks, ncomp, d_f, d_c, d_mask, n, R, a->d_partials, pc) \
                        : launch_cov_kind<KIND, 0>(bp, T, bi, bj, pair, blocks, ncomp, d_f, d_c, d_mask, n, R, a->d_partials, pc)
#define MLMC_COV_DISPATCH012(KIND)                                                                                            \
    rc = gram_mode == 2 ? launch_cov_kind<KIND, 2>(bp, T, bi, bj, pair, blocks, ncomp, d_f, d_c, d_mask, n, R, a->d_partials, pc) \
       : diff_gram_only ? launch_cov_kind<KIND, 1>(bp, T, bi, bj, pair, blocks, ncomp, d_f, d_c, d_mask, n, R, a->d_partials, pc) \
                        : launch_cov_kind<KIND, 0>(bp, T, bi, bj, pair, blocks, ncomp, d_f, d_c, d_mask, n, R, a->d_partials, pc)
            if (gram_mode == 3 && bp.kind != MLMC_LEGENDRE && bp.kind != MLMC_MONOMIAL)
                return fail("covariance: the variance-only pass exists for the polynomial families");
            switch (bp.kind) {
                case MLMC_LEGENDRE: MLMC_COV_DISPATCH(MLMC_LEGENDRE); break;
                case MLMC_MONOMIAL: MLMC_COV_DISPATCH(MLMC_MONOMIAL); break;
                case MLMC_FOURIER: MLMC_COV_DISPATCH012(MLMC_FOURIER); break;
                case MLMC_SPLINE: MLMC_COV_DISPATCH012(MLMC_SPLINE); break;
                default: return fail("covariance: unsupported basis kind");
            }
#undef MLMC_COV_DISPATCH
#undef MLMC_COV_DISPATCH012
            if (rc) return rc;
            if (timed) {
                if (int rc2 = timing_end(a)) return rc2;
                a->launches += 1;
                a->alg_bytes += (int64_t)n * (pair ? 16 : 8) * ncomp;
                a->mfma_flops += (int64_t)512 * cov_tiles_per_sample(T, bi == bj, pair, gram_mode) * n * ncomp;
            }
            hipLaunchKernelGGL(k_reduce_cov, dim3((unsigned)((width + 15) / 16) + (do_count ? 1u : 0u), ncomp), dim3(1024), 0, st, a->d_partials,
                               blocks * n_slices, NT, NG, a->RP, 64 * bi, 64 * bj, totals, a->int_width, (!pair && bi != bj) ? 1 : 0,
                               do_count ? a->d_pcounts : (const int64_t *)nullptr, blocks, a->d_counts + 2 * (int64_t)level);
            MLMC_HIP_CHECK(hipGetLastError());
        }
    return 0;
}

__global__ void k_cov_finalize(const double *__restrict__ totals, const double *__restrict__ scale_c, int R, int RP,
                               int64_t int_width, double *__restrict__ out_s, double *__restrict__ out_sp,
                               const int64_t *__restrict__ counts, int n_levels, int64_t *__restrict__ out_n,
                               double *__restrict__ out_nd, int mean_only, const int64_t *__restrict__ counts2) {
    const int lc = blockIdx.y;
    if (lc == 0 && blockIdx.x == 0)
        for (int l = threadIdx.x; l < n_levels; l += blockDim.x) {
            const int64_t kept = counts[2 * l] + (counts2 ? counts2[2 * l] : 0), removed = counts[2 * l + 1] + (counts2 ? counts2[2 * l + 1] : 0);
            out_n[l] = kept;
            out_n[n_levels + l] = removed;
            out_nd[l] = (double)kept;
            out_nd[n_levels + l] = (double)removed;
        }
    const double *G0 = totals + (int64_t)lc * int_width;
    const double *G1 = G0 + (int64_t)RP * RP;
    const double *G2 = G1 + (int64_t)RP * RP;
    const int idx = blockIdx.x * blockDim.x + threadIdx.x;
    if (idx >= R * R) return;
    const int i = idx / R, j = idx % R;
    const double ci = scale_c ? scale_c[i] : 1.0, cj = scale_c ? scale_c[j] : 1.0;
    const double cc = ci * cj;
    out_s[(int64_t)lc * R * R + idx] = 0.5 * cc * (G0[i * RP + j] + G0[j * RP + i]);
    out_sp[(int64_t)lc * R * R + idx] = mean_only ? __builtin_nan("")
                                                  : 0.25 * (cc * cc) * ((G1[i * RP + j] + G1[j * RP + i]) + 2.0 * G2[i * RP + j]);
}

constexpr int LIN_LC = 8;
constexpr int LIN_MAX_JOBS = 12;
struct LinSrc {
    const double *prod;
    const double *totals;
    const double *scale;
    int64_t width;
    int K, squares;
};
struct LinJob {
    double *out;
    int n_rows;
    int row[LIN_LC];
    LinSrc src[2];
};
struct LinJobs {
    LinJob job[LIN_MAX_JOBS];
};
__global__ void k_cov_lin_mean(LinJobs jobs, int R, int parity_step) {
    extern __shared__ double m_s[];
    const LinJob &jb = jobs.job[blockIdx.y];
    const int idx = blockIdx.x * blockDim.x + threadIdx.x;
    const int RR = R * R;
    for (int e = 0; e < 2; ++e) {
        const LinSrc &sr = jb.src[e];
        if (!sr.prod) continue;
        const int K = sr.K;
        __syncthreads();
        for (int q = threadIdx.x; q < LIN_LC * K; q += blockDim.x) {
            const int l = q / K, k = q % K;
            m_s[q] = l < jb.n_rows ? sr.scale[k] * sr.totals[(int64_t)jb.row[l] * sr.width + k] : 0.0;
        }
        __syncthreads();
        if (idx < RR) {
            double acc[LIN_LC];
#pragma unroll
            for (int l = 0; l < LIN_LC; ++l) acc[l] = 0.0;
            const int k0 = (parity_step == 2 && !sr.squares) ? ((idx / R + idx % R) & 1) : 0;
            for (int k = k0; k < K; k += parity_step) {
                const double c = sr.prod[(int64_t)k * RR + idx];
#pragma unroll
                for (int l = 0; l < LIN_LC; ++l) acc[l] = __builtin_fma(c, m_s[l * K + k], acc[l]);
            }
#pragma unroll
            for (int l = 0; l < LIN_LC; ++l)
                if (l < jb.n_rows) jb.out[(int64_t)jb.row[l] * RR + idx] += acc[l];
        }
    }
}

int launch_cov_finalize(mlmc_accum *a) {
    if (a->lin && a->lin_used) {
        if (int rc = flush_moments(a->lin)) return rc;
    }
    const bool lin0 = a->lin0 && a->lin0_used;
    if (lin0) {
        if (int rc = flush_moments(a->lin0)) return rc;
    }
    const int pstep = a->basis->p.kind == MLMC_LEGENDRE ? 2 : 1;
    const int n_lc = a->n_levels * a->n_comp;
    const bool vals = a->cov_from_values;
    const int R = vals ? a->Rout : a->R;
    hipLaunchKernelGGL(k_cov_finalize, dim3((R * R + 255) / 256, n_lc), dim3(256), 0, rt().stream, a->d_totals,
                       vals ? (const double *)nullptr : a->basis->d_scale, R,
                       a->RP, a->int_width, a->d_out_s, a->d_out_sp, a->d_counts, a->n_levels, a->d_out_n, a->d_out_nd,
                       a->mean_only ? 1 : 0, lin0 ? a->lin0->d_counts : (const int64_t *)nullptr);
    MLMC_HIP_CHECK(hipGetLastError());
    const bool lin = a->lin && a->lin_used;
    if (!lin && !lin0) return 0;
    LinSrc src0, src02, src1;
    std::memset(&src0, 0, sizeof(src0));
    std::memset(&src02, 0, sizeof(src02));
    std::memset(&src1, 0, sizeof(src1));
    int max_K = 0;
    if (lin0) {
        src0.prod = a->d_lin0_prod1; src0.totals = a->lin0->d_totals; src0.scale = a->lin0_basis->d_scale;
        src0.width = a->lin0->int_width; src0.K = a->lin_K; src0.squares = 0;
        src02 = src0;
        src02.prod = a->d_lin0_prod; src02.K = a->lin0_K; src02.squares = 1;
        max_K = a->lin0_K;
    }
    if (lin) {
        src1.prod = a->d_lin_prod; src1.totals = a->lin->d_totals; src1.scale = a->lin_basis->d_scale;
        src1.width = a->lin->int_width; src1.K = a->lin_K; src1.squares = 0;
        if (a->lin_K > max_K) max_K = a->lin_K;
    }
    LinJobs jobs;
    std::memset(&jobs, 0, sizeof(jobs));
    int n_jobs = 0;
    const dim3 block(256);
    auto launch = [&]() -> int {
        if (n_jobs == 0) return 0;
        hipLaunchKernelGGL(k_cov_lin_mean, dim3((R * R + 255) / 256, n_jobs), block, sizeof(double) * LIN_LC * max_K, rt().stream, jobs, R, pstep);
        MLMC_HIP_CHECK(hipGetLastError());
        std::memset(&jobs, 0, sizeof(jobs));
        n_jobs = 0;
        return 0;
    };
    for (int cls = 1; cls <= 4; ++cls) {
        LinJob *jb = nullptr;
        for (int lc = 0; lc < n_lc; ++lc) {
            const int level = lc / a->n_comp;
            const int fed = ((lin0 && a->lin0_levels[level]) ? 1 : 0) | ((lin && a->lin_levels[level]) ? 2 : 0);
            if (cls <= 3 ? fed != cls : !(fed & 1)) continue;
            if (!jb || jb->n_rows == LIN_LC) {
                if (n_jobs == LIN_MAX_JOBS)
                    if (int rc = launch()) return rc;
                jb = &jobs.job[n_jobs++];
                jb->out = cls == 4 ? a->d_out_sp : a->d_out_s;
                jb->src[0] = cls == 4 ? src02 : (cls == 2 ? src1 : src0);
                if (cls == 3) jb->src[1] = src1;
            }
            jb->row[jb->n_rows++] = lc;
        }
    }
    return launch();
}

}
```

### mlmc_amd/csrc/device_basis.hpp

```cpp
#pragma once
#include "common.hpp"

namespace mlmc {

__device__ __forceinline__ double transform_value(const BasisParams &bp, double x, bool &keep) {
    if (bp.kind == MLMC_IDENTITY) {
        keep = !(x != x);
        return x;
    }
    if (bp.is_log) {
        const double tl = (log(x) - bp.shift) * bp.scale + bp.ref0;
        if (bp.is_clip)
            keep = (x >= bp.x_lo) && (x <= bp.x_hi);
        else
            keep = (x > 0.0) && (x < __builtin_inf()) && !(tl != tl) && !(fabs(tl) == __builtin_inf());
        return tl;
    }
    double t = (x - bp.shift) * bp.scale + bp.ref0;
    if (bp.is_clip)
        keep = (t >= bp.ref0) && (t <= bp.ref1);
    else
        keep = !(t != t) && !(fabs(t) == __builtin_inf());
    return t;
}

__device__ __forceinline__ double transform_plain(const BasisParams &bp, double x, bool &keep) {
    const double t = (x - bp.shift) * bp.scale + bp.ref0;
    keep = (t >= bp.ref0) && (t <= bp.ref1);
    return t;
}

constexpr int LEGENDRE_MAX_TERMS = 512;
struct LegendreG {
    double v[LEGENDRE_MAX_TERMS];
    constexpr LegendreG() : v() {
        for (int i = 0; i < LEGENDRE_MAX_TERMS; ++i)
            v[i] = i < 2 ? 0.0 : 4.0 * ((double)((long long)(i - 1) * (i - 1)) / (double)((long long)(2 * i - 1) * (2 * i - 3)));
    }
};
__device__ constexpr LegendreG kLegendreG = LegendreG();

template <int KIND>
struct TermGen {
    double x, p1, p2, c1, s1;
    __device__ __forceinline__ void init(double x_, double w, const BasisParams &) {
        x = (KIND == MLMC_LEGENDRE || KIND == KIND_CHEBYSHEV) ? 2.0 * x_ : x_;
        p1 = w;
        p2 = 0.0;
        if (KIND == MLMC_FOURIER) {
            sincos(x_, &s1, &c1);
            p1 = w;
            p2 = 0.0;
        }
    }
    __device__ __forceinline__ double skip(int j, double g) {
        if (KIND == MLMC_LEGENDRE) {
            const double q = __builtin_fma(x, p1, -(g * p2));
            p2 = p1;
            p1 = q;
            return q;
        } else if (KIND == KIND_CHEBYSHEV) {
            const double q = __builtin_fma(x, p1, -p2);
            p2 = p1;
            p1 = q;
            return q;
        } else {
            return next(2 + (j & 1));
        }
    }
    __device__ __forceinline__ void jump128() {
        const double w = p1, t = 0.5 * x;
        double a = t, b = __builtin_fma(x, t, -1.0);
#pragma unroll
        for (int k = 0; k < 7; ++k) {
            const double a2 = 2.0 * a;
            b = __builtin_fma(a2, b, -t);
            a = __builtin_fma(a2, a, -1.0);
        }
        const double c = __builtin_fma(x, a, -b);
        p2 = __builtin_fma(x, c, -a) * w;
        p1 = c * w;
    }
    __device__ __forceinline__ double next(int i) {
        if (i == 0) return p1;
        if (KIND == MLMC_LEGENDRE) {
            double q;
            if (i == 1) q = x * p1;
            else q = __builtin_fma(x, p1, -(kLegendreG.v[i] * p2));
            p2 = p1;
            p1 = q;
            return q;
        } else if (KIND == KIND_CHEBYSHEV) {
            double q;
            if (i == 1) q = (0.5 * x) * p1;
            else q = __builtin_fma(x, p1, -p2);
            p2 = p1;
            p1 = q;
            return q;
        } else if (KIND == MLMC_MONOMIAL) {
            p1 = p1 * x;
            return p1;
        } else if (KIND == MLMC_FOURIER) {
            if (i & 1) {
                double c = __builtin_fma(p1, c1, -(p2 * s1));
                double s = __builtin_fma(p2, c1, p1 * s1);
                p1 = c;
                p2 = s;
                return c;
            }
            return p2;
        } else {
            return 0.0;
        }
    }
};

template <>
struct TermGen<MLMC_IDENTITY> {
    double v;
    __device__ __forceinline__ void init(double x_, double w, const BasisParams &) { v = x_ * w; }
    __device__ __forceinline__ double next(int) { return v; }
};

template <>
struct TermGen<MLMC_SPLINE> {
    double n0, n1, n2, n3, w;
    int k;
    static __device__ __forceinline__ double knot(int j, int ns, double inv_ns) {
        int c = j - 3;
        c = c < 0 ? 0 : (c > ns ? ns : c);
        return (double)c * inv_ns;
    }
    __device__ __forceinline__ void init(double t, double w_, const BasisParams &bp) {
        w = w_;
        const int ns = bp.size - 3;
        const double inv_ns = 1.0 / (double)ns;
        const double u = (t - bp.ref0) / (bp.ref1 - bp.ref0);
        int s = (int)(u * (double)ns);
        s = s < 0 ? 0 : (s > ns - 1 ? ns - 1 : s);
        k = s;
        if (s >= 2 && s <= ns - 3) {
            const double v = u * (double)ns - (double)s;
            const double v2 = v * v, v3 = v2 * v, om = 1.0 - v;
            constexpr double sixth = 1.0 / 6.0;
            n0 = (om * om * om * sixth) * w;
            n1 = (__builtin_fma(3.0, v3, __builtin_fma(-6.0, v2, 4.0)) * sixth) * w;
            n2 = (__builtin_fma(-3.0, v3, __builtin_fma(3.0, v2, __builtin_fma(3.0, v, 1.0))) * sixth) * w;
            n3 = (v3 * sixth) * w;
            return;
        }
        const int mu = s + 3;
        double N[4], left[4], right[4];
        N[0] = 1.0;
#pragma unroll
        for (int j = 1; j <= 3; ++j) {
            left[j] = u - knot(mu + 1 - j, ns, inv_ns);
            right[j] = knot(mu + j, ns, inv_ns) - u;
            double saved = 0.0;
#pragma unroll
            for (int r = 0; r < j; ++r) {
                const double temp = N[r] / (right[r + 1] + left[j - r]);
                N[r] = saved + right[r + 1] * temp;
                saved = left[j - r] * temp;
            }
            N[j] = saved;
        }
        n0 = N[0] * w; n1 = N[1] * w; n2 = N[2] * w; n3 = N[3] * w;
    }
    __device__ __forceinline__ double next(int i) {
        if (i == 0) return w;
        const int j = i - k;
        return j == 0 ? n0 : (j == 1 ? n1 : (j == 2 ? n2 : (j == 3 ? n3 : 0.0)));
    }
};

__device__ __forceinline__ double wave_sum(double v) {
#pragma unroll
    for (int off = 32; off >= 1; off >>= 1) v += __shfl_xor(v, off, 64);
    return v;
}
__device__ __forceinline__ int wave_sum_i(int v) {
#pragma unroll
    for (int off = 32; off >= 1; off >>= 1) v += __shfl_xor(v, off, 64);
    return v;
}

}
```

### mlmc_amd/csrc/moments.hip

```cpp
#include <cstdlib>
#include <cstring>

#include "device_basis.hpp"

namespace mlmc {

template <int KIND>
__global__ void k_eval(BasisParams bp, const double *__restrict__ scale_c,
                       const double *__restrict__ x, int64_t n, int size, double *__restrict__ out) {
    int64_t i = (int64_t)blockIdx.x * blockDim.x + threadIdx.x;
    if (i >= n) return;
    bool keep;
    double t = transform_value(bp, x[i], keep);
    TermGen<KIND> g;
    g.init(keep ? t : 0.0, 1.0, bp);
    const double nan = __builtin_nan("");
    for (int r = 0; r < size; ++r) {
        double q = g.next(r);
        if (KIND == MLMC_LEGENDRE && scale_c) q *= scale_c[r];
        out[i * size + r] = keep ? q : nan;
    }
}

__global__ void k_apply_matrix(const double *__restrict__ phi, const double *__restrict__ T, int64_t n, int R0, int size,
// ... 345 lines not shown

    double s[RT], sp[RT];
#pragma unroll
    for (int i = 0; i < RT; ++i) { s[i] = 0.0; sp[i] = 0.0; }
    int n_keep = 0, n_rm = 0;
    const unsigned prio_mod = tab.prio_mod > 0 ? (unsigned)tab.prio_mod : 1u;
    constexpr bool WIDE = RT <= 16 && T0C == 0;
    if (PLAIN && WIDE) {
        if (sg.coarse) accum_samples_wide<KIND, RT, true>(bp, sg.fine, sg.coarse, sg.n, bid, sg.nblocks, s, sp, n_keep, n_rm);
        else accum_samples_wide<KIND, RT, false>(bp, sg.fine, sg.coarse, sg.n, bid, sg.nblocks, s, sp, n_keep, n_rm);
    } else if (sg.coarse) {
        accum_samples<KIND, RT, true, T0C, PLAIN>(bp, sg.fine, sg.coarse, sg.mask, sg.n, t0, bid, sg.nblocks, prio_mod, s, sp, n_keep, n_rm);
    } else {
        accum_samples<KIND, RT, false, T0C, PLAIN>(bp, sg.fine, sg.coarse, sg.mask, sg.n, t0, bid, sg.nblocks, prio_mod, s, sp, n_keep, n_rm);
    }
#ifdef MLMC_PROF
    const unsigned long long prof_r1 = __builtin_amdgcn_s_memrealtime(), prof_c1 = __builtin_amdgcn_s_memtime();
#endif
    __shared__ double red[2 * RT][WAVE + 1];
    __shared__ int ldc[4][2];
    const int lane = threadIdx.x & 63, wave = threadIdx.x >> 6;
    for (int w = 0; w < 4; ++w) {
        if (wave == w) {
            if (w == 0) {
#pragma unroll
                for (int i = 0; i < RT; ++i) { red[i][lane] = s[i]; red[RT + i][lane] = sp[i]; }
            } else {
#pragma unroll
                for (int i = 0; i < RT; ++i) { red[i][lane] += s[i]; red[RT + i][lane] += sp[i]; }
            }
        }
        __syncthreads();
    }
    n_keep = wave_sum_i(n_keep);
    n_rm = wave_sum_i(n_rm);
    if (lane == 0) { ldc[wave][0] = n_keep; ldc[wave][1] = n_rm; }
    __syncthreads();
    for (int j = threadIdx.x; j < 2 * RT; j += ACC_THREADS) {
        double v = 0.0;
#pragma unroll 8
        for (int l = 0; l < WAVE; ++l) v += red[j][l];
        partials[(int64_t)blockIdx.x * (2 * RT) + j] = v;
    }
    if (threadIdx.x < 2) {
        int v = ldc[0][threadIdx.x] + ldc[1][threadIdx.x] + ldc[2][threadIdx.x] + ldc[3][threadIdx.x];
        pcounts[(int64_t)blockIdx.x * 2 + threadIdx.x] = v;
    }
#ifdef MLMC_PROF
    if ((threadIdx.x & 63) == 0) {
        unsigned long long *p = g_prof + ((size_t)blockIdx.x * 4 + (threadIdx.x >> 6)) * 5;
        p[0] = prof_r0; p[1] = prof_r1; p[2] = __builtin_amdgcn_s_memrealtime(); p[3] = prof_c1 - prof_c0;
        p[4] = (unsigned long long)__builtin_amdgcn_s_getreg((4 << 0) | (0 << 6) | (31 << 11)) |
               ((unsigned long long)__builtin_amdgcn_s_getreg((20 << 0) | (0 << 6) | (31 << 11)) << 32);
    }
#endif
}

constexpr int SPLIT_LANES = 128;
#ifndef MLMC_SPLIT_HEAD
#define MLMC_SPLIT_HEAD 30
#endif
constexpr int SPLIT_HEAD = MLMC_SPLIT_HEAD;
__host__ __device__ constexpr int split_max(int ht, int tt) { return ht > tt ? ht : tt; }
#ifndef MLMC_SPLIT_WPS
#define MLMC_SPLIT_WPS 2
#endif
#ifdef MLMC_SPLIT_NO_PRIO
#define MLMC_SPLIT_PRIO_INIT
#define MLMC_SPLIT_PRIO_TRIP
#else
#ifndef MLMC_SPLIT_PRIO_BITS
#define MLMC_SPLIT_PRIO_BITS 16
#endif
#define MLMC_SPLIT_PRIO_INIT                                                                                              \
    const unsigned prio_phase = (__builtin_amdgcn_s_getreg((3 << 11) | (0 << 6) | 4) & 15u) % MLMC_SPLIT_WPS;  \
    unsigned long long prio_clock = __builtin_amdgcn_s_memtime();
#define MLMC_SPLIT_PRIO_TRIP                                                                                              \
    if ((((unsigned)(prio_clock >> MLMC_SPLIT_PRIO_BITS)) % MLMC_SPLIT_WPS) == prio_phase) __builtin_amdgcn_s_setprio(2); \
    else __builtin_amdgcn_s_setprio(0);                                                                                   \
    prio_clock = __builtin_amdgcn_s_memtime();
#endif

template <int KIND>
__device__ __forceinline__ void split_export(const TermGen<KIND> &g, double *__restrict__ slot) {
    slot[0 * SPLIT_LANES] = g.x;
    slot[1 * SPLIT_LANES] = g.p1;
    if (KIND == MLMC_LEGENDRE || KIND == KIND_CHEBYSHEV) slot[2 * SPLIT_LANES] = g.p2;
}
template <int KIND>
__device__ __forceinline__ void split_import(TermGen<KIND> &g, const double *__restrict__ slot) {
    g.x = slot[0 * SPLIT_LANES];
    g.p1 = slot[1 * SPLIT_LANES];
    g.p2 = (KIND == MLMC_LEGENDRE || KIND == KIND_CHEBYSHEV) ? slot[2 * SPLIT_LANES] : 0.0;
    g.c1 = g.s1 = 0.0;
}

#ifndef MLMC_SPLIT_NS
#define MLMC_SPLIT_NS 2
#endif
template <int KIND, bool PAIR, bool PLAIN, int HT, int TT, bool SQ, int NS, int T0 = 0>
__device__ __forceinline__ void split_head(const BasisParams &bp, const double *__restrict__ fine, const double *__restrict__ coarse,
                                           const uint8_t *__restrict__ mask, int64_t n, int bid, int nb, int n_trips,
                                           double *__restrict__ hand, double (&s)[split_max(HT, TT)], double (&sp)[split_max(HT, TT)],
                                           int &n_keep, int &n_rm) {
    const int64_t T = (int64_t)nb * SPLIT_LANES;
    const int l128 = threadIdx.x & (SPLIT_LANES - 1);
    int64_t idx[NS];
    double f[NS], c[NS];
    uint8_t m[NS];
#pragma unroll
    for (int q = 0; q < NS; ++q) {
        idx[q] = (int64_t)bid * SPLIT_LANES + l128 + q * T;
        const int64_t j = idx[q] < n ? idx[q] : n - 1;
        f[q] = fine[j];
        c[q] = PAIR ? coarse[j] : 0.0;
        m[q] = (!PLAIN && mask) ? mask[j] : (uint8_t)1;
    }
    MLMC_SPLIT_PRIO_INIT
    for (int k = 0; k < n_trips; ++k) {
        MLMC_SPLIT_PRIO_TRIP
        bool valid[NS];
        double xf[NS], xc[NS];
        uint8_t mm[NS];
#pragma unroll
        for (int q = 0; q < NS; ++q) {
            valid[q] = idx[q] < n;
            xf[q] = f[q]; xc[q] = c[q]; mm[q] = m[q];
            idx[q] += (int64_t)NS * T;
            const int64_t j = idx[q] < n ? idx[q] : n - 1;
            f[q] = fine[j];
            if (PAIR) c[q] = coarse[j];
            if (!PLAIN && mask) m[q] = mask[j];
        }
        TermGen<KIND> gf[NS], gc[NS];
#pragma unroll
        for (int q = 0; q < NS; ++q) {
            bool kf, kc = true;
            const double tf = PLAIN ? transform_plain(bp, xf[q], kf) : transform_value(bp, xf[q], kf);
            double tc = 0;
            if (PAIR) tc = PLAIN ? transform_plain(bp, xc[q], kc) : transform_value(bp, xc[q], kc);
            const bool keep = valid[q] && kf && kc && (PLAIN || mm[q] != 0);
            n_keep += (int)keep;
            n_rm += (int)(valid[q] && !keep);
            const double w = keep ? 1.0 : 0.0;
            gf[q].init(keep ? tf : 0.0, w, bp);
            if (PAIR) gc[q].init(keep ? tc : 0.0, w, bp);
        }
        if constexpr (KIND == KIND_CHEBYSHEV && T0 == 128) {
#pragma unroll
            for (int q = 0; q < NS; ++q) {
                gf[q].jump128();
                if (PAIR) gc[q].jump128();
            }
        } else if (T0 > 0) {
#pragma unroll
            for (int i = 0; i < T0; ++i) {
#pragma unroll
                for (int q = 0; q < NS; ++q) {
                    gf[q].next(i);
                    if (PAIR) gc[q].next(i);
                }
            }
        }
#pragma unroll
        for (int i = 0; i < HT; ++i) {
#pragma unroll
            for (int q = 0; q < NS; ++q) {
                double d = gf[q].next(T0 + i);
                if (PAIR) d -= gc[q].next(T0 + i);
                s[i] += d;
                if (SQ) sp[i] = __builtin_fma(d, d, sp[i]);
            }
        }
        double *__restrict__ slot = hand + (size_t)(k & 1) * (6 * NS * SPLIT_LANES) + l128;
#pragma unroll
        for (int q = 0; q < NS; ++q) {
            split_export<KIND>(gf[q], slot + (3 * q) * SPLIT_LANES);
            if (PAIR) split_export<KIND>(gc[q], slot + (3 * (NS + q)) * SPLIT_LANES);
        }
        __syncthreads();
    }
    __syncthreads();
}

template <int KIND, bool PAIR, int HT, int TT, bool SQ, int NS, int T0 = 0>
__device__ __forceinline__ void split_tail(const BasisParams &bp, int n_trips, const double *__restrict__ hand,
                                           double (&s)[split_max(HT, TT)], double (&sp)[split_max(HT, TT)]) {
    const int l128 = threadIdx.x & (SPLIT_LANES - 1);
    __syncthreads();
    MLMC_SPLIT_PRIO_INIT
    for (int k = 0; k < n_trips; ++k) {
        MLMC_SPLIT_PRIO_TRIP
        const double *__restrict__ slot = hand + (size_t)(k & 1) * (6 * NS * SPLIT_LANES) + l128;
        TermGen<KIND> gf[NS], gc[NS];
#pragma unroll
        for (int q = 0; q < NS; ++q) {
            split_import<KIND>(gf[q], slot + (3 * q) * SPLIT_LANES);
            if (PAIR) split_import<KIND>(gc[q], slot + (3 * (NS + q)) * SPLIT_LANES);
        }
#pragma unroll
        for (int i = 0; i < TT; ++i) {
#pragma unroll
            for (int q = 0; q < NS; ++q) {
                double d = gf[q].next(T0 + HT + i);
                if (PAIR) d -= gc[q].next(T0 + HT + i);
                s[i] += d;
                if (SQ) sp[i] = __builtin_fma(d, d, sp[i]);
            }
        }
        __syncthreads();
    }
}

template <int KIND, bool PLAIN, int HT, int TT, int WPS, bool SQ = true, int NS = MLMC_SPLIT_NS, int T0 = 0>
__global__ __launch_bounds__(ACC_THREADS, WPS) void k_moments_accum_split(BasisParams bp, SegTable tab,
                                                                        double *__restrict__ partials,
                                                                        int64_t *__restrict__ pcounts) {
    __shared__ double hand[2 * 6 * NS * SPLIT_LANES];
    constexpr int MAXT = split_max(HT, TT), NTOT = HT + TT;
    __shared__ double wsum[4][2 * MAXT];
    __shared__ int ldc[2][2];
    Seg sg = tab.seg[0];
#pragma unroll
    for (int k = 1; k < MAX_SEG; ++k)
        if (k < tab.nseg && (int)blockIdx.x >= tab.seg[k].block0) sg = tab.seg[k];
    const int bid = (int)blockIdx.x - sg.block0;
    const int lane = threadIdx.x & 63;
    const int wave = __builtin_amdgcn_readfirstlane((int)(threadIdx.x >> 6));
    const int64_t T2 = NS * (int64_t)sg.nblocks * SPLIT_LANES;
    const int64_t first = (int64_t)bid * SPLIT_LANES;
    const int n_trips = first < sg.n ? (int)((sg.n - first + T2 - 1) / T2) : 0;

    double s[MAXT], sp[MAXT];
#pragma unroll
    for (int i = 0; i < MAXT; ++i) { s[i] = 0.0; sp[i] = 0.0; }
    int n_keep = 0, n_rm = 0;
    if (wave < 2) {
        if (sg.coarse) split_head<KIND, true, PLAIN, HT, TT, SQ, NS, T0>(bp, sg.fine, sg.coarse, sg.mask, sg.n, bid, sg.nblocks, n_trips, hand, s, sp, n_keep, n_rm);
        else split_head<KIND, false, PLAIN, HT, TT, SQ, NS, T0>(bp, sg.fine, sg.coarse, sg.mask, sg.n, bid, sg.nblocks, n_trips, hand, s, sp, n_keep, n_rm);
    } else {
        if (sg.coarse) split_tail<KIND, true, HT, TT, SQ, NS, T0>(bp, n_trips, hand, s, sp);
        else split_tail<KIND, false, HT, TT, SQ, NS, T0>(bp, n_trips, hand, s, sp);
    }
#pragma unroll
    for (int i = 0; i < MAXT; ++i) {
        const double a = wave_sum(s[i]), b = SQ ? wave_sum(sp[i]) : __builtin_nan("");
        if (lane == 0) { wsum[wave][i] = a; wsum[wave][MAXT + i] = b; }
    }
    n_keep = wave_sum_i(n_keep);
    n_rm = wave_sum_i(n_rm);
    if (lane == 0 && wave < 2) { ldc[wave][0] = n_keep; ldc[wave][1] = n_rm; }
    __syncthreads();
    if (threadIdx.x < 2 * NTOT) {
        const int which = threadIdx.x / NTOT, term = threadIdx.x % NTOT;
        const int half = term < HT ? 0 : 1, i = half ? term - HT : term;
        partials[(int64_t)blockIdx.x * (2 * NTOT) + threadIdx.x] = wsum[2 * half][which * MAXT + i] + wsum[2 * half + 1][which * MAXT + i];
    }
    if (threadIdx.x < 2) pcounts[(int64_t)blockIdx.x * 2 + threadIdx.x] = ldc[0][threadIdx.x] + ldc[1][threadIdx.x];
}

__global__ __launch_bounds__(1024) void k_reduce_partials(const double *__restrict__ partials,
                                                         const int64_t *__restrict__ pcounts, SegTable tab, ReduceTable rtab,
                                                         int width, int RT, int t0, int int_R) {
    __shared__ double lds[16][64];
    Seg sg = tab.seg[0];
    ReduceTarget tg = rtab.t[0];
#pragma unroll
    for (int k = 1; k < MAX_SEG; ++k)
        if ((int)blockIdx.x == k) { sg = tab.seg[k]; tg = rtab.t[k]; }
    const int row0 = sg.block0, nblocks = sg.nblocks;
    const int c = threadIdx.x & 63, g = threadIdx.x >> 6;
    for (int c0 = 0; c0 < width; c0 += 64) {
        const int col = c0 + c;
        double acc = 0.0;
        if (col < width) {
            const double *__restrict__ pc = partials + (int64_t)row0 * width + col;
#pragma unroll 8
            for (int b = g; b < nblocks; b += 16) acc += pc[(int64_t)b * width];
        }
        __syncthreads();
        lds[g][c] = acc;
        __syncthreads();
        if (g == 0 && col < width) {
            double v = 0.0;
#pragma unroll
            for (int k = 0; k < 16; ++k) v += lds[k][c];
            const int which = col / RT, term = t0 + col % RT;
            if (term < int_R) {
                const double t = tg.totals[(int64_t)which * int_R + term] + v;
                tg.totals[(int64_t)which * int_R + term] = t;
                if (tg.h_s) {
                    const double c = tg.scale[term];
                    if (which == 0) tg.h_s[term] = c * t;
                    else tg.h_sp[term] = (c * c) * t;
                    if (tg.p_s) {
                        if (which == 0) tg.p_s[term] = c * t;
                        else tg.p_sp[term] = (c * c) * t;
                    }
                }
            }
        }
    }
    if (tg.counts && g == 15) {
        int64_t a = 0, b = 0;
        for (int i = c; i < nblocks; i += 64) { a += pcounts[2 * (int64_t)(row0 + i)]; b += pcounts[2 * (int64_t)(row0 + i) + 1]; }
        for (int off = 32; off >= 1; off >>= 1) { a += __shfl_xor(a, off, 64); b += __shfl_xor(b, off, 64); }
// ... 43 lines not shown
        const double nf[4] = {gf.n0, gf.n1, gf.n2, gf.n3};
        if (!pair) {
#pragma unroll
            for (int j = 0; j < 4; ++j) {
                const int r = gf.k + j;
                if (r > 0) { atomicAdd(&ws[r], nf[j]); if (NEED_SQ) atomicAdd(&wsp[r], nf[j] * nf[j]); }
            }
            continue;
        }
        gc.init(tc, 1.0, bp);
        const double nc[4] = {gc.n0, gc.n1, gc.n2, gc.n3};
        const int delta = gc.k - gf.k;
        if (delta == 0) {
#pragma unroll
            for (int j = 0; j < 4; ++j) {
                const int r = gf.k + j;
                const double d = nf[j] - nc[j];
                if (r > 0) { atomicAdd(&ws[r], d); if (NEED_SQ) atomicAdd(&wsp[r], d * d); }
            }
        } else {
#pragma unroll
            for (int j = 0; j < 4; ++j) {
                const int r = gf.k + j, jc = j - delta;
                const double c = jc == 0 ? nc[0] : (jc == 1 ? nc[1] : (jc == 2 ? nc[2] : (jc == 3 ? nc[3] : 0.0)));
                const double d = nf[j] - c;
                if (r > 0) { atomicAdd(&ws[r], d); if (NEED_SQ) atomicAdd(&wsp[r], d * d); }
            }
#pragma unroll
            for (int j = 0; j < 4; ++j) {
                const int r = gc.k + j, jf = j + delta;
                if ((jf < 0 || jf > 3) && r > 0) { atomicAdd(&ws[r], -nc[j]); if (NEED_SQ) atomicAdd(&wsp[r], nc[j] * nc[j]); }
            }
        }
    }
    n_keep = wave_sum_i(n_keep);
    n_rm = wave_sum_i(n_rm);
    if (lane == 0) { ldc[wave][0] = n_keep; ldc[wave][1] = n_rm; }
    __syncthreads();
    const int keep_block = ldc[0][0] + ldc[1][0] + ldc[2][0] + ldc[3][0];
    for (int j = threadIdx.x; j < 2 * R; j += ACC_THREADS) {
        const int which = j / R, r = j % R;
        const int o = which * RP + r;
        double v = ((sacc[o] + sacc[2 * RP + o]) + sacc[4 * RP + o]) + sacc[6 * RP + o];
        if (r == 0) v = pair ? 0.0 : (double)keep_block;
        partials[(int64_t)blockIdx.x * (2 * R) + j] = v;
    }
    if (threadIdx.x < 2) {
        int v = ldc[0][threadIdx.x] + ldc[1][threadIdx.x] + ldc[2][threadIdx.x] + ldc[3][threadIdx.x];
        pcounts[(int64_t)blockIdx.x * 2 + threadIdx.x] = v;
    }
}

template <int KIND, int RT, int T0C, bool PLAIN>
static int launch_accum_rt(const BasisParams &bp, const SegTable &tab, int total_blocks, int t0,
                           double *partials, int64_t *pcounts) {
    hipLaunchKernelGGL((k_moments_accum<KIND, RT, T0C, PLAIN>), dim3(total_blocks), dim3(ACC_THREADS), 0, rt().stream, bp, tab, t0, partials,
                       pcounts);
    MLMC_HIP_CHECK(hipGetLastError());
    return 0;
}

template <int KIND, int RT, int T0C, bool PLAIN>
static int occupancy_rt(int *per_cu) {
    MLMC_HIP_CHECK(hipOccupancyMaxActiveBlocksPerMultiprocessor(per_cu, (const void *)k_moments_accum<KIND, RT, T0C, PLAIN>, ACC_THREADS, 0));
    return 0;
}

static int pick_rt(int kind, int n_terms, int t0) {
    if (kind == MLMC_IDENTITY) return 4;
    if (t0 == 32) return n_terms <= 16 ? 16 : 32;
    if (t0 == 64) return n_terms <= 16 ? 16 : (n_terms <= 32 ? 32 : (n_terms <= 48 ? 48 : 64));
    if (t0 > 0) return 64;
    if (kind == MLMC_LEGENDRE) {
        const int opts[] = {4, 6, 8, 10, 12, 16, 20, 24, 28, 32, 40, 48, 56, 64};
        for (int o : opts)
            if (n_terms <= o) return o;
        return 64;
    }
    const int opts[] = {8, 16, 24, 32, 48, 64};
    for (int o : opts)
        if (n_terms <= o) return o;
    return 64;
}

static int accum_dispatch(int op, bool plain, const BasisParams &bp, int rt_sel, const SegTable *tab, int total_blocks,
                          int t0, double *partials, int64_t *pcounts, int *out) {
#define MLMC_RT_GO1(KIND, N, T0C, P) \
    (op == 0 ? occupancy_rt<KIND, N, T0C, P>(out) : launch_accum_rt<KIND, N, T0C, P>(bp, *tab, total_blocks, t0, partials, pcounts))
#define MLMC_RT_GO(KIND, N, T0C) (plain ? MLMC_RT_GO1(KIND, N, T0C, true) : MLMC_RT_GO1(KIND, N, T0C, false))
#define MLMC_RT_CASE(KIND, N) case N: return MLMC_RT_GO(KIND, N, 0)
#define MLMC_RT_LATER(KIND)                                                                                  \
    if (t0 == 32) return rt_sel == 16 ? MLMC_RT_GO(KIND, 16, 32) : MLMC_RT_GO(KIND, 32, 32);                 \
    if (t0 == 64) {                                                                                          \
        switch (rt_sel) {                                                                                    \
            case 16: return MLMC_RT_GO(KIND, 16, 64);                                                        \
            case 32: return MLMC_RT_GO(KIND, 32, 64);                                                        \
            case 48: return MLMC_RT_GO(KIND, 48, 64);                                                        \
            default: return MLMC_RT_GO(KIND, 64, 64);                                                        \
        }                                                                                                    \
    }                                                                                                        \
    return MLMC_RT_GO(KIND, 64, -1)
    if (t0 > 0) {
        switch (bp.kind) {
            case MLMC_LEGENDRE: MLMC_RT_LATER(MLMC_LEGENDRE);
            case MLMC_MONOMIAL: MLMC_RT_LATER(MLMC_MONOMIAL);
            case MLMC_FOURIER: MLMC_RT_LATER(MLMC_FOURIER);
            default: return fail("moments: a later pass needs a polynomial / Fourier basis");
        }
    }
    switch (bp.kind) {
        case MLMC_LEGENDRE:
            switch (rt_sel) {
                MLMC_RT_CASE(MLMC_LEGENDRE, 4); MLMC_RT_CASE(MLMC_LEGENDRE, 6); MLMC_RT_CASE(MLMC_LEGENDRE, 8);
                MLMC_RT_CASE(MLMC_LEGENDRE, 10); MLMC_RT_CASE(MLMC_LEGENDRE, 12);
                MLMC_RT_CASE(MLMC_LEGENDRE, 16); MLMC_RT_CASE(MLMC_LEGENDRE, 20); MLMC_RT_CASE(MLMC_LEGENDRE, 24);
                MLMC_RT_CASE(MLMC_LEGENDRE, 28); MLMC_RT_CASE(MLMC_LEGENDRE, 32); MLMC_RT_CASE(MLMC_LEGENDRE, 40);
                MLMC_RT_CASE(MLMC_LEGENDRE, 48); MLMC_RT_CASE(MLMC_LEGENDRE, 56);
                default: return MLMC_RT_GO(MLMC_LEGENDRE, 64, 0);
            }
        case MLMC_MONOMIAL:
            switch (rt_sel) {
                MLMC_RT_CASE(MLMC_MONOMIAL, 8); MLMC_RT_CASE(MLMC_MONOMIAL, 16); MLMC_RT_CASE(MLMC_MONOMIAL, 24);
                MLMC_RT_CASE(MLMC_MONOMIAL, 32); MLMC_RT_CASE(MLMC_MONOMIAL, 48);
                default: return MLMC_RT_GO(MLMC_MONOMIAL, 64, 0);
            }
        case MLMC_FOURIER:
            switch (rt_sel) {
                MLMC_RT_CASE(MLMC_FOURIER, 8); MLMC_RT_CASE(MLMC_FOURIER, 16); MLMC_RT_CASE(MLMC_FOURIER, 24);
                MLMC_RT_CASE(MLMC_FOURIER, 32); MLMC_RT_CASE(MLMC_FOURIER, 48);
                default: return MLMC_RT_GO(MLMC_FOURIER, 64, 0);
            }
        case MLMC_IDENTITY: return MLMC_RT_GO1(MLMC_IDENTITY, 4, 0, false);
        default: return fail("unknown basis kind");
    }
#undef MLMC_RT_LATER
#undef MLMC_RT_CASE
#undef MLMC_RT_GO
#undef MLMC_RT_GO1
}

template <int KIND, bool PLAIN, int HT, int TT, int WPS, bool SQ, int T0 = 0>
static int split_go(int op, const BasisParams &bp, const SegTable *tab, int total_blocks, double *partials, int64_t *pcounts, int *out) {
    if (op == 0) {
        MLMC_HIP_CHECK(hipOccupancyMaxActiveBlocksPerMultiprocessor(out, (const void *)k_moments_accum_split<KIND, PLAIN, HT, TT, WPS, SQ, MLMC_SPLIT_NS, T0>, ACC_THREADS, 0));
        return 0;
    }
    hipLaunchKernelGGL((k_moments_accum_split<KIND, PLAIN, HT, TT, WPS, SQ, MLMC_SPLIT_NS, T0>), dim3(total_blocks), dim3(ACC_THREADS), 0, rt().stream, bp, *tab, partials, pcounts);
    MLMC_HIP_CHECK(hipGetLastError());
    return 0;
}
constexpr int SPLIT_MEAN_HEAD_96 = 46, SPLIT_MEAN_HEAD_128 = 62;
constexpr int SPLIT_MEAN_HEAD_W2 = 40;
constexpr int SPLIT_CHEB_HEAD_96 = 45, SPLIT_CHEB_HEAD_128 = 61, SPLIT_CHEB_HEAD_W2 = 51;
static int split_dispatch(int op, bool plain, const BasisParams &bp, int n_split, int t0, const SegTable *tab, int total_blocks, double *partials,
                          int64_t *pcounts, int *out) {
#define MLMC_SPLIT_GO(KIND, P)                                                                                                          \
    (t0 == 128 ? split_go<KIND, P, SPLIT_MEAN_HEAD_W2, 128 - SPLIT_MEAN_HEAD_W2, 2, false, 128>(op, bp, tab, total_blocks, partials, pcounts, out) \
     : n_split == 64 ? split_go<KIND, P, SPLIT_HEAD, 64 - SPLIT_HEAD, MLMC_SPLIT_WPS, true>(op, bp, tab, total_blocks, partials, pcounts, out)   \
     : n_split == 96 ? split_go<KIND, P, SPLIT_MEAN_HEAD_96, 96 - SPLIT_MEAN_HEAD_96, 2, false>(op, bp, tab, total_blocks, partials, pcounts, out) \
                     : split_go<KIND, P, SPLIT_MEAN_HEAD_128, 128 - SPLIT_MEAN_HEAD_128, 2, false>(op, bp, tab, total_blocks, partials, pcounts, out))
#define MLMC_SPLIT_GO_CHEB(P)                                                                                                           \
    (t0 == 128 ? split_go<KIND_CHEBYSHEV, P, SPLIT_CHEB_HEAD_W2, 128 - SPLIT_CHEB_HEAD_W2, 2, false, 128>(op, bp, tab, total_blocks, partials, pcounts, out) \
     : n_split == 96 ? split_go<KIND_CHEBYSHEV, P, SPLIT_CHEB_HEAD_96, 96 - SPLIT_CHEB_HEAD_96, 2, false>(op, bp, tab, total_blocks, partials, pcounts, out) \
                     : split_go<KIND_CHEBYSHEV, P, SPLIT_CHEB_HEAD_128, 128 - SPLIT_CHEB_HEAD_128, 2, false>(op, bp, tab, total_blocks, partials, pcounts, out))
    if (bp.kind == KIND_CHEBYSHEV) {
        if (n_split == 64 && t0 == 0) return fail("moments: Chebyshev sums exist for the mean-only term-split kernels (65..256 terms)");
        return plain ? MLMC_SPLIT_GO_CHEB(true) : MLMC_SPLIT_GO_CHEB(false);
    }
    if (bp.kind == MLMC_LEGENDRE) return plain ? MLMC_SPLIT_GO(MLMC_LEGENDRE, true) : MLMC_SPLIT_GO(MLMC_LEGENDRE, false);
    return plain ? MLMC_SPLIT_GO(MLMC_MONOMIAL, true) : MLMC_SPLIT_GO(MLMC_MONOMIAL, false);
#undef MLMC_SPLIT_GO_CHEB
#undef MLMC_SPLIT_GO
}

int flush_moments(mlmc_accum *a) {
    const int nseg = (int)a->pending.size();
    if (nseg == 0) return 0;
    hipStream_t st = rt().stream;
    const int R = a->R;
    const BasisParams &bp = a->basis->p;
    const bool sparse_spline = bp.kind == MLMC_SPLINE;
    if (sparse_spline && R > SPLINE_MAX_R) return fail("spline moments: at most 512 basis functions");
    static const bool no_split = std::getenv("MLMC_HIP_NO_SPLIT") != nullptr;
    const bool cheb = bp.kind == KIND_CHEBYSHEV;
    const bool poly = bp.kind == MLMC_LEGENDRE || bp.kind == MLMC_MONOMIAL || cheb;
    const bool poly64 = poly && R > 48 && R <= 64;
    const bool split_mean = poly && a->mean_only_plain && R > 64 && R <= 256 && (!no_split || cheb);
    const bool split = (poly64 && !no_split) || split_mean;
    if (cheb && !split_mean) return fail("moments: Chebyshev sums exist for the mean-only term-split kernels (65..256 terms)");
    const int pass_terms = split_mean ? 128 : ((poly64 && !split) ? 32 : MAX_TERMS_PER_PASS);
    for (int t0 = 0; t0 < (sparse_spline ? 1 : R); t0 += pass_terms) {
        const int n_terms = (R - t0 < pass_terms) ? R - t0 : pass_terms;
        const int n_split = split_mean ? ((t0 == 0 && R <= 96) ? 96 : 128) : 64;
        const int rt_sel = sparse_spline ? R : (split ? n_split : pick_rt(bp.kind, n_terms, t0));
        const int width = 2 * rt_sel;
        int per_cu = 4;
        bool plain = bp.kind != MLMC_IDENTITY && !bp.is_log && bp.is_clip;
        for (const PendingSeg &p : a->pending) plain = plain && p.mask == nullptr;
        if (split) {
            static int occ_split[3][2][4];
            int &cached = occ_split[bp.kind == MLMC_LEGENDRE ? 0 : (cheb ? 2 : 1)][plain ? 1 : 0][t0 ? 3 : (n_split == 64 ? 0 : (n_split == 96 ? 1 : 2))];
            if (cached == 0)
                if (int rc = split_dispatch(0, plain, bp, n_split, t0, nullptr, 0, nullptr, nullptr, &cached)) return rc;
            per_cu = cached;
        } else if (!sparse_spline) {
            static int occ_cache[8][4][2][65];
            int &cached = occ_cache[bp.kind & 7][t0 == 0 ? 0 : (t0 == 64 ? 1 : (t0 == 32 ? 2 : 3))][plain ? 1 : 0][rt_sel];
            if (cached == 0)
                if (int rc = accum_dispatch(0, plain, bp, rt_sel, nullptr, 0, t0, nullptr, nullptr, &cached)) return rc;
            per_cu = cached;
        }
        if (cheb && per_cu > 2) per_cu = 2;
        if (per_cu < 1) per_cu = 1;
        if (per_cu > 8) per_cu = 8;
        const int resident = rt().n_cu * per_cu;
        constexpr double W_PAIR = 7.0, W_SINGLE = 4.3;
        double wsum = 0.0;
        for (const PendingSeg &p : a->pending) wsum += (double)p.n * (p.coarse ? W_PAIR : W_SINGLE);
        SegTable tab;
        ReduceTable rtab;
        std::memset(&tab, 0, sizeof(tab));
        std::memset(&rtab, 0, sizeof(rtab));
        tab.nseg = nseg;
        tab.prio_mod = per_cu < 1 ? 1 : (per_cu > 8 ? 8 : per_cu);
        int total = 0;
        int64_t bytes = 0;
        for (int k = 0; k < nseg; ++k) {
            const PendingSeg &p = a->pending[k];
            int nb = (int)((double)resident * ((double)p.n * (p.coarse ? W_PAIR : W_SINGLE)) / wsum);
            const int64_t per_trip = split ? (int64_t)MLMC_SPLIT_NS * SPLIT_LANES : 2 * ACC_THREADS;
            const int64_t want = (p.n + per_trip - 1) / per_trip;
            if (nb > want) nb = (int)want;
            if (nb < 1) nb = 1;
            tab.seg[k].fine = p.fine;
            tab.seg[k].coarse = p.coarse;
            tab.seg[k].mask = p.mask;
            tab.seg[k].n = p.n;
            tab.seg[k].block0 = total;
            tab.seg[k].nblocks = nb;
            total += nb;
            rtab.t[k].totals = a->d_totals + ((int64_t)p.level * a->n_comp + p.comp) * a->int_width;
            rtab.t[k].counts = (p.count && t0 == 0) ? a->d_counts + (int64_t)p.level * 2 : nullptr;
            if (a->host_outputs) {
                rtab.t[k].h_s = a->h_out_s + (int64_t)p.level * R;
                rtab.t[k].h_sp = a->h_out_sp + (int64_t)p.level * R;
                rtab.t[k].h_n = a->h_out_n + p.level;
                rtab.t[k].h_n_stride = a->n_levels;
                if (a->packed_target) {
                    double *pk = a->packed_target;
                    rtab.t[k].p_nd = pk + p.level;
                    rtab.t[k].p_s = pk + 2 * (int64_t)a->n_levels + (int64_t)p.level * R;
                    rtab.t[k].p_sp = rtab.t[k].p_s + (int64_t)a->n_levels * R;
                }
                rtab.t[k].scale = a->basis->d_scale;
                a->level_flushed[p.level] = 1;
            }
            bytes += p.n * (p.coarse ? 16 : 8);
        }
        if (int rc = ensure((void **)&a->d_partials, &a->partials_cap, sizeof(double) * (size_t)total * width)) return rc;
        if (int rc = ensure((void **)&a->d_pcounts, &a->pcounts_cap, sizeof(int64_t) * (size_t)total * 2)) return rc;
        if (int rc = timing_begin(a)) return rc;
        if (sparse_spline) {
            const size_t lds = sizeof(double) * 4 * 2 * (size_t)(R + 8);
            if (a->mean_only)
                hipLaunchKernelGGL(k_spline_accum<false>, dim3(total), dim3(ACC_THREADS), lds, st, bp, tab, R, a->d_partials, a->d_pcounts);
            else
                hipLaunchKernelGGL(k_spline_accum<true>, dim3(total), dim3(ACC_THREADS), lds, st, bp, tab, R, a->d_partials, a->d_pcounts);
            MLMC_HIP_CHECK(hipGetLastError());
        } else if (split) {
            if (int rc = split_dispatch(1, plain, bp, n_split, t0, &tab, total, a->d_partials, a->d_pcounts, nullptr)) return rc;
        } else if (int rc = accum_dispatch(1, plain, bp, rt_sel, &tab, total, t0, a->d_partials, a->d_pcounts, nullptr)) {
            return rc;
        }
        if (int rc = timing_end(a)) return rc;
        a->launches += 1;
        a->alg_bytes += bytes;
        hipLaunchKernelGGL(k_reduce_partials, dim3(nseg), dim3(1024), 0, st, a->d_partials, a->d_pcounts, tab, rtab, width, rt_sel, t0, R);
        MLMC_HIP_CHECK(hipGetLastError());
    }
    a->pending.clear();
    return 0;
}

int launch_moments_accum(mlmc_accum *a, int level, int comp, const double *d_f, const double *d_c, const uint8_t *d_mask,
                         int64_t n, bool count, bool defer) {
    if (n == 0) return 0;
    for (const PendingSeg &p : a->pending)
        if (p.level == level && p.comp == comp) {
            if (int rc = flush_moments(a)) return rc;
            break;
        }
    if ((int)a->pending.size() >= MAX_SEG)
        if (int rc = flush_moments(a)) return rc;
    a->pending.push_back(PendingSeg{d_f, d_c, d_mask, n, level, comp, count});
    if (!defer) return flush_moments(a);
    return 0;
}

__global__ void k_moments_finalize(const double *__restrict__ totals, const double *__restrict__ scale_c,
                                   const double *__restrict__ T, int R, int RP, int Rout, int has_T, int64_t int_width,
                                   int n_lc, double *__restrict__ out_s, double *__restrict__ out_sp,
                                   const int64_t *__restrict__ counts, int n_levels, int64_t *__restrict__ out_n,
                               double *__restrict__ out_nd, int mean_only) {
    const int lc = blockIdx.x;
    if (lc >= n_lc) return;
    if (lc == 0)
        for (int l = threadIdx.x; l < n_levels; l += blockDim.x) {
            out_n[l] = counts[2 * l];
            out_n[n_levels + l] = counts[2 * l + 1];
            out_nd[l] = (double)counts[2 * l];
            out_nd[n_levels + l] = (double)counts[2 * l + 1];
        }
    const double *tot = totals + (int64_t)lc * int_width;
    for (int j = threadIdx.x; j < Rout; j += blockDim.x) {
        double s, sp;
        if (!has_T) {
            const double c = scale_c[j];
            s = c * tot[j];
            sp = (c * c) * tot[R + j];
        } else {
            const double *G = tot + 2 * R;
            s = 0.0;
            sp = 0.0;
            for (int i = 0; i < R; ++i) {
                const double ti = T[(int64_t)j * R + i] * scale_c[i];
                s = __builtin_fma(ti, tot[i], s);
                if (mean_only) continue;
                double row = 0.0;
                for (int k = 0; k < R; ++k) row = __builtin_fma(T[(int64_t)j * R + k] * scale_c[k], G[(int64_t)i * RP + k], row);
                sp = __builtin_fma(ti, row, sp);
            }
            if (mean_only) sp = __builtin_nan("");
        }
        out_s[(int64_t)lc * Rout + j] = s;
        out_sp[(int64_t)lc * Rout + j] = sp;
    }
}

int launch_moments_finalize(mlmc_accum *a) {
    const int n_lc = a->n_levels * a->n_comp;
    hipLaunchKernelGGL(k_moments_finalize, dim3(n_lc), dim3(128), 0, rt().stream, a->d_totals, a->basis->d_scale,
                       a->basis->d_matrix, a->R, a->RP, a->Rout, a->basis->out_size > 0 ? 1 : 0, a->int_width, n_lc,
                       a->d_out_s, a->d_out_sp, a->d_counts, a->n_levels, a->d_out_n, a->d_out_nd, a->mean_only ? 1 : 0);
    MLMC_HIP_CHECK(hipGetLastError());
    return 0;
}

}
```

Measured before the change: 308.3 billion.

## Derive low Chebyshev moments from covariance-kernel row sums via connection table

In the linearized covariance path for 49..64-term Legendre bases, the matrix kernel now also accumulates per-row sums of the basis values, reduces them in extra reduce-kernel blocks, and rebuilds the first 64 Chebyshev moments through a Legendre-to-Chebyshev connection matrix. The separate Chebyshev moment pass can then start at term 64, using a new jump64 recurrence and a 63-term split kernel. This removes the redundant evaluation of the low Chebyshev terms. The cost is extra register use and shuffles in the covariance kernel, more reduce blocks, and possible loss of accuracy from the connection-coefficient recombination.

```diff
diff --git a/include/mlmc_hip.h b/include/mlmc_hip.h
--- a/include/mlmc_hip.h
+++ b/include/mlmc_hip.h
@@ -63,6 +63,8 @@
 int mlmc_accum_kernel_flops(mlmc_accum *a, int64_t *mfma_flops);
 int mlmc_accum_aux_kernel_time(mlmc_accum *a, double *ms, int64_t *launches, int64_t *alg_bytes);
 int mlmc_linearization_table(int32_t kind, int32_t R, int32_t squares, double *out, int64_t out_len);
+
+int mlmc_chebyshev_connection_table(int32_t M, double *out, int64_t out_len);
 
 int mlmc_accum_estimate_multi(int32_t M, const mlmc_basis *const *bases, int32_t K, int32_t n_levels, int32_t n_chunks,
                               const int32_t *levels, const double *const *fine, const double *const *coarse,
diff --git a/mlmc_amd/_lib.py b/mlmc_amd/_lib.py
--- a/mlmc_amd/_lib.py
+++ b/mlmc_amd/_lib.py
@@ -65,6 +65,7 @@
     "mlmc_accum_kernel_flops": (C.c_int, [_vp, _ip]),
     "mlmc_accum_aux_kernel_time": (C.c_int, [_vp, _dp, _ip, _ip]),
     "mlmc_linearization_table": (C.c_int, [C.c_int32, C.c_int32, C.c_int32, _vp, C.c_int64]),
+    "mlmc_chebyshev_connection_table": (C.c_int, [C.c_int32, _vp, C.c_int64]),
     "mlmc_percentiles": (C.c_int, [_vp, C.c_int64, _vp, C.c_int32, _vp, _ip, C.c_int]),
     "mlmc_percentiles_rows": (C.c_int, [_vp, C.c_int64, C.c_int64, C.c_int64, _vp, C.c_int32, _vp, _vp, C.c_int]),
     "mlmc_maxent_solve": (C.c_int, [_vp, _vp, _vp, C.c_int32, C.c_double, C.c_double, C.POINTER(MaxentOpts), _vp,
diff --git a/mlmc_amd/csrc/api.hip b/mlmc_amd/csrc/api.hip
--- a/mlmc_amd/csrc/api.hip
+++ b/mlmc_amd/csrc/api.hip
@@ -263,6 +263,22 @@
         }
 }
 
+static void chebyshev_connection(int M, std::vector<double> &out) {
+    std::vector<ld> g(M > 1 ? M : 1);
+    g[0] = 1.0L;
+    for (int j = 1; j < M; ++j) g[j] = g[j - 1] * (ld)(2 * j - 1) / (ld)(2 * j);
+    out.assign((size_t)M * M, 0.0);
+    out[0] = 1.0;
+    for (int m = 1; m < M; ++m) {
+        out[(size_t)m * M + m] = (double)(1.0L / (2.0L * g[m]));
+        for (int k = m - 2; k >= 0; k -= 2) {
+            const int n = (m + k) / 2;
+            const ld v = -((ld)m * ((ld)k + 0.5L)) / ((ld)(m + k + 1) * (ld)(m - k)) * g[(m - k - 2) / 2] / ((ld)n * g[n]);
+            out[(size_t)m * M + k] = (double)v;
+        }
+    }
+}
+
 bool product_table_chebyshev(int R, std::vector<double> &out) {
     std::vector<ld> c;
     legendre_products_ld(R, c);
@@ -294,6 +310,11 @@
 
 static bool linearize_chebyshev_enabled() {
     const char *e = std::getenv("MLMC_HIP_LINEARIZE_CHEB");
+    return !(e && e[0] == '0');
+}
+
+static bool linearize_rowsums_enabled() {
+    const char *e = std::getenv("MLMC_HIP_LINEARIZE_ROWSUMS");
     return !(e && e[0] == '0');
 }
 
@@ -518,6 +539,25 @@
     return 0;
 }
 
+static int connection_table_device(double **out) {
+    static double *d_conn = nullptr;
+    if (!d_conn) {
+        std::vector<double> h;
+        chebyshev_connection(64, h);
+        ld c = 1.0L;
+        for (int i = 0; i < 64; ++i) {
+            if (i >= 1) c = c * (ld)(2 * i - 1) / (ld)(2 * i);
+            h.push_back((double)c);
+        }
+        double *d = nullptr;
+        MLMC_HIP_CHECK(hipMalloc(&d, sizeof(double) * h.size()));
+        MLMC_HIP_CHECK(hipMemcpy(d, h.data(), sizeof(double) * h.size(), hipMemcpyHostToDevice));
+        d_conn = d;
+    }
+    *out = d_conn;
+    return 0;
+}
+
 static int inner_basis_create(const mlmc_basis *b, int size, bool cheb, mlmc_basis **out) {
     mlmc_basis_desc d;
     std::memset(&d, 0, sizeof(d));
@@ -559,7 +599,18 @@
             a->d_lin0_prod = t2->d_prod2;
         }
     }
+    if (!rc && a->cov_rows) {
+        rc = connection_table_device(&a->d_conn);
+        if (!rc && hipMalloc(&a->d_rowsums, sizeof(double) * 64 * (size_t)a->n_levels * a->n_comp) != hipSuccess)
+            rc = fail("covariance: device allocation failed (row sums)");
+        if (!rc && hipMemsetAsync(a->d_rowsums, 0, sizeof(double) * 64 * (size_t)a->n_levels * a->n_comp, rt().stream) != hipSuccess)
+            rc = fail("covariance: memset failed (row sums)");
+        if (!rc) a->lin->first_term = 64;
+    }
     if (rc) {
+        if (a->d_rowsums) (void)hipFree(a->d_rowsums);
+        a->d_rowsums = nullptr;
+        a->cov_rows = false;
         if (a->lin) mlmc_accum_destroy(a->lin);
         if (a->lin_basis) mlmc_basis_destroy(a->lin_basis);
         if (a->lin0) mlmc_accum_destroy(a->lin0);
@@ -635,6 +686,8 @@
         const char *lin0_env = std::getenv("MLMC_HIP_LINEARIZE_LEVEL0");
         a->lin0_eligible = a->R <= 64 && !(lin0_env && lin0_env[0] == '0');
         a->lin_cheb = b->p.kind == MLMC_LEGENDRE && linearize_chebyshev_enabled() && std::getenv("MLMC_HIP_NO_SPLIT") == nullptr;
+        a->cov_rows = a->lin_cheb && a->lin0_eligible && a->R >= 49 && a->R <= 64 && a->RP == 64 && linearize_rowsums_enabled() &&
+                      cov_rows_available();
     }
     *out = a;
     return mlmc_accum_reset(a);
@@ -653,6 +706,7 @@
         a->xcov_pushes = 0;
     }
     a->lin_used = a->lin0_used = false;
+    if (a->d_rowsums) MLMC_HIP_CHECK(hipMemsetAsync(a->d_rowsums, 0, sizeof(double) * 64 * (size_t)a->n_levels * a->n_comp, st));
     a->lin_levels.assign(a->n_levels, 0);
     a->lin0_levels.assign(a->n_levels, 0);
     if (a->lin0)
@@ -670,7 +724,7 @@
     if (a->lin0) mlmc_accum_destroy(a->lin0);
     if (a->lin0_basis) mlmc_basis_destroy(a->lin0_basis);
     void *ptrs[] = {a->d_state, a->d_partials, a->d_pcounts, a->d_stage_f, a->d_stage_c, a->d_mask, a->d_out, a->d_vals_f, a->d_vals_c, a->d_vals_tmp,
-                    a->d_shift};
+                    a->d_shift, a->d_rowparts, a->d_rowsums};
     for (void *p : ptrs)
         if (p) (void)hipFree(p);
     if (a->h_out) (void)hipHostFree(a->h_out);
@@ -970,6 +1024,16 @@
     return 0;
 }
 
+int mlmc_chebyshev_connection_table(int32_t M, double *out, int64_t out_len) {
+    if (!out) return fail("mlmc_chebyshev_connection_table: null argument");
+    if (M < 1 || M > 64) return fail("mlmc_chebyshev_connection_table: size out of range (1 .. 64)");
+    if (out_len < (int64_t)M * M) return fail("mlmc_chebyshev_connection_table: output too small");
+    std::vector<double> t;
+    chebyshev_connection(M, t);
+    std::memcpy(out, t.data(), sizeof(double) * t.size());
+    return 0;
+}
+
 int mlmc_xcov_create(int32_t M, int32_t n_levels, int32_t flags, mlmc_accum **out) {
     MLMC_API_GUARD;
     if (need_runtime()) return 1;
diff --git a/mlmc_amd/csrc/common.hpp b/mlmc_amd/csrc/common.hpp
--- a/mlmc_amd/csrc/common.hpp
+++ b/mlmc_amd/csrc/common.hpp
@@ -155,6 +155,11 @@
     bool lin0_used = false;
     int64_t lin_min_n = 0;
     bool lin_used = false;
+    bool cov_rows = false;
+    double *d_rowparts = nullptr; size_t rowparts_cap = 0;
+    double *d_rowsums = nullptr;
+    double *d_conn = nullptr;
+    int first_term = 0;
     std::vector<PendingSeg> pending;
     bool xcov = false;
     double *d_shift = nullptr;
@@ -173,6 +178,7 @@
 int launch_cov_accum(mlmc_accum *a, int level, int comp, const double *d_f, const double *d_c, const uint8_t *d_mask,
                      int64_t n, bool count, int gram_mode, int ncomp = 1);
 int launch_cov_finalize(mlmc_accum *a);
+bool cov_rows_available();
 constexpr int XCOV_MAX_M = 1024;
 constexpr int MODE_XCOV = 2;
 int launch_xcov_push(mlmc_accum *a, int level, const double *d_f, const double *d_c, int64_t n);
diff --git a/mlmc_amd/csrc/cov.hip b/mlmc_amd/csrc/cov.hip
--- a/mlmc_amd/csrc/cov.hip
+++ b/mlmc_amd/csrc/cov.hip
@@ -388,12 +388,20 @@
 __host__ __device__ constexpr int xsym_i(int kind, int w, int t) { return kind == 2 ? bsym_i(w, t) : (kind == 1 ? psym_i(w, t) : sym_i(w, t)); }
 __host__ __device__ constexpr int xsym_j(int kind, int w, int t) { return kind == 2 ? bsym_j(w, t) : (kind == 1 ? psym_j(w, t) : sym_j(w, t)); }
 
-template <int KIND, bool PAIR, int MODE, int BD, int W>
+#ifndef MLMC_COV_ROWS_WAVES
+#define MLMC_COV_ROWS_WAVES 0
+#endif
+__host__ __device__ constexpr int cov_rows_mask(int w) {
+    return MLMC_COV_ROWS_WAVES == 0 ? (w == 0 ? 3 : (w == 3 ? 12 : 0))
+         : MLMC_COV_ROWS_WAVES == 1 ? (w == 1 ? 1 : (w == 2 ? 14 : 0))
+                                    : (w == 2 ? 15 : 0);
+}
+template <int KIND, bool PAIR, int MODE, int BD, int W, bool RS = false>
 __device__ __forceinline__ void cov_t4_body(const BasisParams &bp, 
                                             const double *__restrict__ fine, const double *__restrict__ coarse,
                                             const uint8_t *__restrict__ mask, int64_t n, double *__restrict__ partials,
                                             int64_t *__restrict__ pcounts, double *__restrict__ lds_f,
-                                            double *__restrict__ lds_c, int (*ldc)[2]) {
+                                            double *__restrict__ lds_c, int (*ldc)[2], double *__restrict__ rowparts = nullptr) {
     constexpr int NT = 64;
     constexpr int TA = 64 * BD;
     constexpr int N_EVAL = TA + NT;
@@ -406,7 +414,10 @@
     constexpr int NFULL = (MODE == 0 && PAIR) ? 2 : (((MODE == 2 || MODE == 3) && PAIR) ? 1 : 0);
     constexpr int GV = MODE == 3 ? 0 : 1;
     constexpr int NSYMM = (MODE == 0 && !PAIR) ? 2 : 1;
+    static_assert(!RS || BLK, "row sums: 2 x 2-block body of a pair level");
+    constexpr int RSM = RS ? cov_rows_mask(W) : 0;
     const int lane = threadIdx.x & 63;
+    double rsum[4] = {0.0, 0.0, 0.0, 0.0};
 
     v4f64 accf[NFULL > 0 ? NFULL : 1][4];
     v4f64 accs[NSYMM][3];
@@ -512,6 +523,9 @@
 #pragma unroll
                 for (int J = 0; J < 4; ++J) ds[J] = d[J] * sm[J];
 #pragma unroll
+                for (int J = 0; J < 4; ++J)
+                    if ((RSM >> J) & 1) rsum[J] += d[J];
+#pragma unroll
                 for (int r = 0; r < 2; ++r) {
                     const double dr2 = d[RA + r] * d[RA + r];
 #pragma unroll
@@ -586,6 +600,12 @@
     }
 #endif
 
+#pragma unroll
+    for (int J = 0; J < 4; ++J)
+        if ((RSM >> J) & 1) {
+            const double v1 = __shfl(rsum[J], (lane & 15) + 16, 64), v2 = __shfl(rsum[J], (lane & 15) + 32, 64), v3 = __shfl(rsum[J], (lane & 15) + 48, 64);
+            if (lane < 16) rowparts[(int64_t)blockIdx.x * 64 + 16 * J + lane] = ((rsum[J] + v1) + v2) + v3;
+        }
     constexpr int NGOUT = cov_ng(MODE);
     double *__restrict__ prow = partials + (int64_t)blockIdx.x * (NGOUT * NT * NT);
     const int r0 = lane >> 4, c0 = lane & 15;
@@ -686,13 +706,54 @@
     }
 }
 
+#if MLMC_COV_BLK22 && MLMC_COV_T4_BATCH == 32
+#define MLMC_COV_HAVE_ROWS 1
+template <int KIND>
+__global__ __launch_bounds__(256, COV_T4_WGS) void k_cov_accum_t4_rows(BasisParams bp, const double *__restrict__ fine,
+                                                              const double *__restrict__ coarse, const uint8_t *__restrict__ mask,
+                                                              int64_t n, double *__restrict__ partials,
+                                                              int64_t *__restrict__ pcounts, double *__restrict__ rowparts) {
+    __shared__ __attribute__((aligned(16))) double lds_f[64 * (COV_T4_BATCH + MLMC_COV_B128_PAD)];
+    __shared__ __attribute__((aligned(16))) double lds_c[64 * (COV_T4_BATCH + MLMC_COV_B128_PAD)];
+    __shared__ int ldc[2][2];
+    fine += (int64_t)blockIdx.y * n;
+    coarse += (int64_t)blockIdx.y * n;
+    partials += (int64_t)blockIdx.y * gridDim.x * (cov_ng(3) * 64 * 64);
+    rowparts += (int64_t)blockIdx.y * gridDim.x * 64;
+    if (blockIdx.y) pcounts = nullptr;
+    switch (__builtin_amdgcn_readfirstlane((int)(threadIdx.x >> 6))) {
+        case 0: cov_t4_body<KIND, true, 3, 0, 0, true>(bp, fine, coarse, mask, n, partials, pcounts, lds_f, lds_c, ldc, rowparts); break;
+        case 1: cov_t4_body<KIND, true, 3, 0, 1, true>(bp, fine, coarse, mask, n, partials, pcounts, lds_f, lds_c, ldc, rowparts); break;
+        case 2: cov_t4_body<KIND, true, 3, 0, 2, true>(bp, fine, coarse, mask, n, partials, pcounts, lds_f, lds_c, ldc, rowparts); break;
+        default: cov_t4_body<KIND, true, 3, 0, 3, true>(bp, fine, coarse, mask, n, partials, pcounts, lds_f, lds_c, ldc, rowparts); break;
+    }
+}
+#endif
+
 __global__ __launch_bounds__(1024) void k_reduce_cov(const double *__restrict__ partials, int nrows, int NT, int NG, int RP,
                                                     int roff, int coff, double *__restrict__ totals, int64_t comp_stride,
                                                     int mirror, const int64_t *__restrict__ pcounts, int nblocks,
-                                                    int64_t *__restrict__ counts) {
+                                                    int64_t *__restrict__ counts, const double *__restrict__ rowparts = nullptr,
+                                                    double *__restrict__ rowsums = nullptr) {
     __shared__ double lds[64][17];
     const int c = threadIdx.x & 15, g = threadIdx.x >> 4;
     const int width = NG * NT * NT;
+    const int n_col_groups = (width + 15) / 16;
+    if (rowparts && (int)blockIdx.x >= n_col_groups && (int)blockIdx.x < n_col_groups + 4) {
+        const int col = ((int)blockIdx.x - n_col_groups) * 16 + c;
+        rowparts += (int64_t)blockIdx.y * nrows * 64;
+        double acc = 0.0;
+        for (int b = g; b < nrows; b += 64) acc += rowparts[(int64_t)b * 64 + col];
+        lds[g][c] = acc;
+        __syncthreads();
+        if (g == 0) {
+            double v = 0.0;
+#pragma unroll
+            for (int k = 0; k < 64; ++k) v += lds[k][c];
+            rowsums[(int64_t)blockIdx.y * 64 + col] += v;
+        }
+        return;
+    }
     if (pcounts && blockIdx.x == gridDim.x - 1) {
         if (blockIdx.y == 0 && threadIdx.x < 64) {
             int64_t a = 0, b = 0;
@@ -975,6 +1036,14 @@
     return full;
 }
 
+bool cov_rows_available() {
+#ifdef MLMC_COV_HAVE_ROWS
+    return true;
+#else
+    return false;
+#endif
+}
+
 int launch_cov_accum(mlmc_accum *a, int level, int comp, const double *d_f, const double *d_c, const uint8_t *d_mask,
                      int64_t n, bool count, int gram_mode, int ncomp) {
     const bool diff_gram_only = gram_mode == 1;
@@ -1020,6 +1089,17 @@
                         : launch_cov_kind<KIND, 0>(bp, T, bi, bj, pair, blocks, ncomp, d_f, d_c, d_mask, n, R, a->d_partials, pc)
             if (gram_mode == 3 && bp.kind != MLMC_LEGENDRE && bp.kind != MLMC_MONOMIAL)
                 return fail("covariance: the variance-only pass exists for the polynomial families");
+            const bool rows = a->cov_rows && gram_mode == 3 && pair;
+            if (rows) {
+#ifdef MLMC_COV_HAVE_ROWS
+                if (int rce = ensure((void **)&a->d_rowparts, &a->rowparts_cap, sizeof(double) * (size_t)blocks * 64 * ncomp)) return rce;
+                hipLaunchKernelGGL((k_cov_accum_t4_rows<MLMC_LEGENDRE>), dim3(blocks, ncomp), dim3(256), 0, st, bp, d_f, d_c, d_mask, n, a->d_partials, pc, a->d_rowparts);
+                MLMC_HIP_CHECK(hipGetLastError());
+                rc = 0;
+#else
+                return fail("covariance: this build has no row sums in the matrix kernel");
+#endif
+            } else
             switch (bp.kind) {
                 case MLMC_LEGENDRE: MLMC_COV_DISPATCH(MLMC_LEGENDRE); break;
                 case MLMC_MONOMIAL: MLMC_COV_DISPATCH(MLMC_MONOMIAL); break;
@@ -1036,9 +1116,11 @@
                 a->alg_bytes += (int64_t)n * (pair ? 16 : 8) * ncomp;
                 a->mfma_flops += (int64_t)512 * cov_tiles_per_sample(T, bi == bj, pair, gram_mode) * n * ncomp;
             }
-            hipLaunchKernelGGL(k_reduce_cov, dim3((unsigned)((width + 15) / 16) + (do_count ? 1u : 0u), ncomp), dim3(1024), 0, st, a->d_partials,
+            hipLaunchKernelGGL(k_reduce_cov, dim3((unsigned)((width + 15) / 16) + (rows ? 4u : 0u) + (do_count ? 1u : 0u), ncomp), dim3(1024), 0, st, a->d_partials,
                                blocks * n_slices, NT, NG, a->RP, 64 * bi, 64 * bj, totals, a->int_width, (!pair && bi != bj) ? 1 : 0,
-                               do_count ? a->d_pcounts : (const int64_t *)nullptr, blocks, a->d_counts + 2 * (int64_t)level);
+                               do_count ? a->d_pcounts : (const int64_t *)nullptr, blocks, a->d_counts + 2 * (int64_t)level,
+                               rows ? a->d_rowparts : (const double *)nullptr,
+                               rows ? a->d_rowsums + ((int64_t)level * a->n_comp + comp) * 64 : (double *)nullptr);
             MLMC_HIP_CHECK(hipGetLastError());
         }
     return 0;
@@ -1078,6 +1160,7 @@
     const double *scale;
     int64_t width;
     int K, squares;
+    const double *rowsums, *conn, *pscale;
 };
 struct LinJob {
     double *out;
@@ -1100,7 +1183,16 @@
         __syncthreads();
         for (int q = threadIdx.x; q < LIN_LC * K; q += blockDim.x) {
             const int l = q / K, k = q % K;
-            m_s[q] = l < jb.n_rows ? sr.scale[k] * sr.totals[(int64_t)jb.row[l] * sr.width + k] : 0.0;
+            double v = 0.0;
+            if (l < jb.n_rows) {
+                if (sr.rowsums && k < 64) {
+                    const double *__restrict__ rs = sr.rowsums + (int64_t)jb.row[l] * 64;
+                    for (int j = k & 1; j <= k; j += 2) v = __builtin_fma(sr.conn[k * 64 + j], sr.pscale[j] * rs[j], v);
+                } else {
+                    v = sr.scale[k] * sr.totals[(int64_t)jb.row[l] * sr.width + k];
+                }
+            }
+            m_s[q] = v;
         }
         __syncthreads();
         if (idx < RR) {
@@ -1154,6 +1246,7 @@
     if (lin) {
         src1.prod = a->d_lin_prod; src1.totals = a->lin->d_totals; src1.scale = a->lin_basis->d_scale;
         src1.width = a->lin->int_width; src1.K = a->lin_K; src1.squares = 0;
+        if (a->cov_rows) { src1.rowsums = a->d_rowsums; src1.conn = a->d_conn; src1.pscale = a->d_conn + 64 * 64; }
         if (a->lin_K > max_K) max_K = a->lin_K;
     }
     LinJobs jobs;
diff --git a/mlmc_amd/csrc/device_basis.hpp b/mlmc_amd/csrc/device_basis.hpp
--- a/mlmc_amd/csrc/device_basis.hpp
+++ b/mlmc_amd/csrc/device_basis.hpp
@@ -73,6 +73,19 @@
         double a = t, b = __builtin_fma(x, t, -1.0);
 #pragma unroll
         for (int k = 0; k < 7; ++k) {
+            const double a2 = 2.0 * a;
+            b = __builtin_fma(a2, b, -t);
+            a = __builtin_fma(a2, a, -1.0);
+        }
+        const double c = __builtin_fma(x, a, -b);
+        p2 = __builtin_fma(x, c, -a) * w;
+        p1 = c * w;
+    }
+    __device__ __forceinline__ void jump64() {
+        const double w = p1, t = 0.5 * x;
+        double a = t, b = __builtin_fma(x, t, -1.0);
+#pragma unroll
+        for (int k = 0; k < 6; ++k) {
             const double a2 = 2.0 * a;
             b = __builtin_fma(a2, b, -t);
             a = __builtin_fma(a2, a, -1.0);
diff --git a/mlmc_amd/csrc/moments.hip b/mlmc_amd/csrc/moments.hip
--- a/mlmc_amd/csrc/moments.hip
+++ b/mlmc_amd/csrc/moments.hip
@@ -521,6 +521,12 @@
                 gf[q].jump128();
                 if (PAIR) gc[q].jump128();
             }
+        } else if constexpr (KIND == KIND_CHEBYSHEV && T0 == 64) {
+#pragma unroll
+            for (int q = 0; q < NS; ++q) {
+                gf[q].jump64();
+                if (PAIR) gc[q].jump64();
+            }
         } else if (T0 > 0) {
 #pragma unroll
             for (int i = 0; i < T0; ++i) {
@@ -870,6 +876,10 @@
 constexpr int SPLIT_MEAN_HEAD_96 = 46, SPLIT_MEAN_HEAD_128 = 62;
 constexpr int SPLIT_MEAN_HEAD_W2 = 40;
 constexpr int SPLIT_CHEB_HEAD_96 = 45, SPLIT_CHEB_HEAD_128 = 61, SPLIT_CHEB_HEAD_W2 = 51;
+#ifndef MLMC_SPLIT_CHEB_HEAD_T64
+#define MLMC_SPLIT_CHEB_HEAD_T64 22
+#endif
+constexpr int SPLIT_CHEB_HEAD_T64 = MLMC_SPLIT_CHEB_HEAD_T64;
 static int split_dispatch(int op, bool plain, const BasisParams &bp, int n_split, int t0, const SegTable *tab, int total_blocks, double *partials,
                           int64_t *pcounts, int *out) {
 #define MLMC_SPLIT_GO(KIND, P)                                                                                                          \
@@ -879,10 +889,12 @@
                      : split_go<KIND, P, SPLIT_MEAN_HEAD_128, 128 - SPLIT_MEAN_HEAD_128, 2, false>(op, bp, tab, total_blocks, partials, pcounts, out))
 #define MLMC_SPLIT_GO_CHEB(P)                                                                                                           \
     (t0 == 128 ? split_go<KIND_CHEBYSHEV, P, SPLIT_CHEB_HEAD_W2, 128 - SPLIT_CHEB_HEAD_W2, 2, false, 128>(op, bp, tab, total_blocks, partials, pcounts, out) \
+     : t0 == 64 ? split_go<KIND_CHEBYSHEV, P, SPLIT_CHEB_HEAD_T64, 63 - SPLIT_CHEB_HEAD_T64, 2, false, 64>(op, bp, tab, total_blocks, partials, pcounts, out) \
      : n_split == 96 ? split_go<KIND_CHEBYSHEV, P, SPLIT_CHEB_HEAD_96, 96 - SPLIT_CHEB_HEAD_96, 2, false>(op, bp, tab, total_blocks, partials, pcounts, out) \
                      : split_go<KIND_CHEBYSHEV, P, SPLIT_CHEB_HEAD_128, 128 - SPLIT_CHEB_HEAD_128, 2, false>(op, bp, tab, total_blocks, partials, pcounts, out))
     if (bp.kind == KIND_CHEBYSHEV) {
         if (n_split == 64 && t0 == 0) return fail("moments: Chebyshev sums exist for the mean-only term-split kernels (65..256 terms)");
+        if (t0 == 64 && n_split != 63) return fail("moments: the Chebyshev pass from term 64 on covers 63 terms");
         return plain ? MLMC_SPLIT_GO_CHEB(true) : MLMC_SPLIT_GO_CHEB(false);
     }
     if (bp.kind == MLMC_LEGENDRE) return plain ? MLMC_SPLIT_GO(MLMC_LEGENDRE, true) : MLMC_SPLIT_GO(MLMC_LEGENDRE, false);
@@ -907,17 +919,19 @@
     const bool split = (poly64 && !no_split) || split_mean;
     if (cheb && !split_mean) return fail("moments: Chebyshev sums exist for the mean-only term-split kernels (65..256 terms)");
     const int pass_terms = split_mean ? 128 : ((poly64 && !split) ? 32 : MAX_TERMS_PER_PASS);
-    for (int t0 = 0; t0 < (sparse_spline ? 1 : R); t0 += pass_terms) {
+    if (a->first_term && !(a->first_term == 64 && cheb && split_mean && R > 64 && R <= 127))
+        return fail("moments: a first term of 64 exists for Chebyshev sums of 65..127 terms");
+    for (int t0 = a->first_term; t0 < (sparse_spline ? 1 : R); t0 += pass_terms) {
         const int n_terms = (R - t0 < pass_terms) ? R - t0 : pass_terms;
-        const int n_split = split_mean ? ((t0 == 0 && R <= 96) ? 96 : 128) : 64;
+        const int n_split = split_mean ? (t0 == 64 ? 63 : ((t0 == 0 && R <= 96) ? 96 : 128)) : 64;
         const int rt_sel = sparse_spline ? R : (split ? n_split : pick_rt(bp.kind, n_terms, t0));
         const int width = 2 * rt_sel;
         int per_cu = 4;
         bool plain = bp.kind != MLMC_IDENTITY && !bp.is_log && bp.is_clip;
         for (const PendingSeg &p : a->pending) plain = plain && p.mask == nullptr;
         if (split) {
-            static int occ_split[3][2][4];
-            int &cached = occ_split[bp.kind == MLMC_LEGENDRE ? 0 : (cheb ? 2 : 1)][plain ? 1 : 0][t0 ? 3 : (n_split == 64 ? 0 : (n_split == 96 ? 1 : 2))];
+            static int occ_split[3][2][5];
+            int &cached = occ_split[bp.kind == MLMC_LEGENDRE ? 0 : (cheb ? 2 : 1)][plain ? 1 : 0][t0 == 64 ? 4 : (t0 ? 3 : (n_split == 64 ? 0 : (n_split == 96 ? 1 : 2)))];
             if (cached == 0)
                 if (int rc = split_dispatch(0, plain, bp, n_split, t0, nullptr, 0, nullptr, nullptr, &cached)) return rc;
             per_cu = cached;
```

New measurement: 315.5 billion (median of 6 runs). +2.3%, better.
